# 0215Arthur/Pytorch_News_Recommender

Hardware: AMD Instinct MI355X
Metric: users/sec (train step) NRMS MIND-small hist=50 cand=5 (higher is better)
Workload: dtype f16 (MFMA inputs and saved activations; fp32 accumulate, softmax, loss, master weights and Adam); 1 GPU; configs[1] shapes: NRMS(nrms_v0) train step, 512 users/GPU, hist=50, cand=5, title_len=30, d=300, h=10, q=200, V=45800, dropout=0.2, Adam(lr=1e-3); users_per_gpu=512, global_batch=512, parallelism=dp1, precision=fp16, resident_batches=32

## Files before the change

### include/nrms_hip.h

```cpp
#ifndef NRMS_HIP_H
#define NRMS_HIP_H

#include <stddef.h>
#include <stdint.h>

#ifdef __cplusplus
extern "C" {
#endif

#define NRMS_OK            0
#define NRMS_EINVAL       -1
#define NRMS_ELAUNCH      -2
#define NRMS_EWORKSPACE   -3

#define NRMS_PRECISION_FP32   0
#define NRMS_PRECISION_BF16X3 1
#define NRMS_PRECISION_BF16   2
#define NRMS_FP16_KP 320
#define NRMS_FP16_DP 320
#define NRMS_FP16_QP 224
#define NRMS_PRECISION_FP16   3

#define NRMS_FLAG_PAD_ROW_ZERO 1
#define NRMS_FLAG_DEFER_WQKV 2
#define NRMS_FLAG_FWD_SCRATCH_KEPT 4
#define NRMS_FLAG_FUSED_SEQ64 8

typedef struct nrms_encoder_desc {
    int32_t  n_seq;
    int32_t  seq_len;
    int32_t  d_model;
    int32_t  n_heads;
    int32_t  q_dim;
    int32_t  vocab;
    float    p_drop_embed;
    float    p_drop_ctx;
    int32_t  precision;
    int32_t  use_output_proj;
    int32_t  mask_mode;
    int32_t  flags;
    uint64_t seed;
    float    loss_scale;
    float    p_drop_attn;
    const int32_t* seq_index;
} nrms_encoder_desc;

typedef struct nrms_encoder_weights {
    const float* table;
    const float* w_qkv;
    const float* b_qkv;
    const float* w_o;
    const float* b_o;
    const float* w_add;
    const float* b_add;
    const float* q_vec;
} nrms_encoder_weights;

typedef struct nrms_encoder_grads {
    float* table;
    float* w_qkv;
    float* b_qkv;
    float* w_o;
    float* b_o;
    float* w_add;
    float* b_add;
    float* q_vec;
} nrms_encoder_grads;

typedef struct nrms_encoder_acts {
    float* x;
    float* qkv;
    float* attn;
    float* ctx;
    float* t;
    float* w;
    void*  scratch;
} nrms_encoder_acts;

size_t nrms_encoder_fwd_scratch_bytes(const nrms_encoder_desc* desc);
size_t nrms_encoder_fused_qkv_bytes(const nrms_encoder_desc* desc);
int nrms_encoder_fwd(const nrms_encoder_desc* desc, const nrms_encoder_weights* w,
                     const int64_t* ids, const float* x, const uint8_t* mask ,
                     const nrms_encoder_acts* acts, float* out, void* stream);

size_t nrms_encoder_bwd_workspace_bytes(const nrms_encoder_desc* desc);
int nrms_encoder_bwd(const nrms_encoder_desc* desc, const nrms_encoder_weights* w,
                     const int64_t* ids, const float* x, const uint8_t* mask,
                     const nrms_encoder_acts* acts, const float* dout,
                     const nrms_encoder_grads* grads, float* dx,
                     void* workspace, size_t workspace_bytes, void* stream);
int nrms_encoder_bwd_wqkv(const nrms_encoder_desc* desc, const int64_t* ids, const float* x,
                          const nrms_encoder_acts* acts, const nrms_encoder_grads* grads,
                          void* workspace, size_t workspace_bytes, void* stream);

int nrms_sanitize_ids(const int64_t* src, int64_t* dst, int64_t n, int32_t vocab, int32_t* n_bad, void* stream);
int nrms_sanitize_ids_i32(const int32_t* src, int64_t* dst, int64_t n, int32_t vocab, int32_t* n_bad, void* stream);

int nrms_title_dedup(const int64_t* ids, int64_t n_titles, int32_t seq_len, int32_t* table, int64_t table_size,
                     int32_t* inverse, int32_t* rep_rows, int32_t* n_unique, void* stream);

int nrms_click_score_fwd(int32_t B, int32_t C, int32_t d, const float* cand, const float* user,
                         const uint8_t* mask, float* scores, void* stream);
int nrms_click_score_indexed(int32_t B, int32_t C, int32_t d, const float* news_vec, int64_t n_vec, const int32_t* index,
                             const float* user, const uint8_t* mask, float* scores, void* stream);
int nrms_click_score_bwd(int32_t B, int32_t C, int32_t d, const float* cand, const float* user,
                         const uint8_t* mask, const float* dscores, float* dcand, float* duser,
                         void* stream);

int nrms_ce_loss_fwd_bwd(int32_t B, int32_t C, const float* scores, float* loss_sum,
                         float* dscores, float grad_scale, void* stream);

int nrms_adam_step(size_t n, float* param, const float* grad, float* exp_avg, float* exp_avg_sq,
                   double lr, double beta1, double beta2, double eps, int32_t step, float grad_scale,
                   void* stream);

int nrms_adam_step_guarded(size_t n, float* param, const float* grad, float* exp_avg, float* exp_avg_sq,
                           double lr, double beta1, double beta2, double eps, int32_t step, float grad_scale,
                           int32_t* n_nonfinite, void* stream);
int nrms_grad_guard(size_t n, float* grad, int32_t* n_nonfinite, void* stream);

int nrms_impression_auc(int32_t n_imp, int32_t max_c, const float* scores, const uint8_t* labels,
                        const int32_t* lens, double* auc, void* stream);

int nrms_impression_metrics(int32_t n_imp, int32_t max_c, const float* scores, const uint8_t* labels,
                            const int32_t* lens, int32_t k_a, int32_t k_b, double* auc, double* mrr, double* ndcg_a,
                            double* ndcg_b, int32_t* ranks, void* stream);

size_t nrms_topk_dot_workspace_bytes(int32_t B, int64_t N, int32_t d, int32_t k);
int nrms_topk_dot(int32_t B, int64_t N, int32_t d, int32_t k, const float* user, const float* items, const int64_t* exclude,
                  int32_t n_exclude, float* top_scores, int64_t* top_ids, void* workspace, size_t workspace_bytes, void* stream);

size_t nrms_topk_grouped_dot_workspace_bytes(int32_t B, int64_t N, int32_t d, int32_t k, int32_t G);
int nrms_topk_grouped_dot(int32_t B, int64_t N, int32_t d, int32_t k, int32_t G, const float* query, const float* items,
                          const int32_t* item_ids, const int64_t* group_ptr, const int64_t* exclude, int32_t n_exclude,
                          float* top_scores, int64_t* top_ids, void* workspace, size_t workspace_bytes, void* stream);

size_t nrms_rank_dot_workspace_bytes(int32_t B, int64_t N, int32_t d, int32_t T, int32_t n_exclude);
int nrms_rank_dot(int32_t B, int64_t N, int32_t d, int32_t T, const float* user, const float* items, const int64_t* targets,
                  const int64_t* exclude, int32_t n_exclude, int32_t* ranks, float* target_scores, void* workspace,
                  size_t workspace_bytes, void* stream);

int nrms_layernorm_fwd(int64_t n_rows, int32_t d, const float* x, const float* gamma, const float* beta, float eps,
                       float* y, float* stats, void* stream);
size_t nrms_layernorm_bwd_workspace_bytes(int32_t d);
int nrms_layernorm_bwd(int64_t n_rows, int32_t d, const float* x, const float* gamma, const float* stats, const float* dy,
                       float* dx, float* dgamma_dbeta, void* workspace, size_t workspace_bytes, void* stream);

typedef struct nrms_news_features {
    int64_t n;
    int32_t d_text;
    int32_t d_cat;
    int32_t n_cat, n_sub;
    float   p_drop;
    uint64_t seed;
    const float* title_vec;
    const float* abst_vec;
    const float* cat_table;
    const float* sub_table;
    const int64_t* categ;
    const int64_t* subcateg;
} nrms_news_features;
int nrms_news_features_fwd(const nrms_news_features* f, float* out, void* stream);
int nrms_news_features_bwd(const nrms_news_features* f, const float* dout, float* d_title_vec, float* d_abst_vec,
                           float* d_cat_table, float* d_sub_table, void* stream);

#define NRMS_SEGPOOL_ROWS_UNIQUE 1
// ... 107 lines not shown
```

### pytorch_news_recommender_amd/_lib.py

```python
from __future__ import annotations

import ctypes as C
import os

PKG = os.path.dirname(os.path.abspath(__file__))
LIB_PATH = os.environ.get("NRMS_HIP_LIB") or os.path.join(PKG, "libnrms_hip.so")

NRMS_OK, NRMS_EINVAL, NRMS_ELAUNCH, NRMS_EWORKSPACE = 0, -1, -2, -3
NRMS_FLAG_PAD_ROW_ZERO = 1
NRMS_FLAG_DEFER_WQKV = 2
NRMS_FLAG_FWD_SCRATCH_KEPT = 4
NRMS_FLAG_FUSED_SEQ64 = 8
NRMS_PRECISION_FP32 = 0
NRMS_PRECISION_BF16X3 = 1
NRMS_PRECISION_BF16 = 2
NRMS_PRECISION_FP16 = 3
NRMS_DROPOUT_FIELDS16 = 0x100
NRMS_DROPOUT_SITE_NEWSVEC = 4
NRMS_FP16_KP, NRMS_FP16_DP, NRMS_FP16_QP = 320, 320, 224
PRECISIONS = {"fp32": 0, "bf16x3": 1, "bf16": 2, "fp16": 3}


class NrmsError(RuntimeError):
    pass


class EncoderDesc(C.Structure):
    _fields_ = [("n_seq", C.c_int32), ("seq_len", C.c_int32), ("d_model", C.c_int32),
                ("n_heads", C.c_int32), ("q_dim", C.c_int32), ("vocab", C.c_int32),
                ("p_drop_embed", C.c_float), ("p_drop_ctx", C.c_float), ("precision", C.c_int32),
                ("use_output_proj", C.c_int32), ("mask_mode", C.c_int32), ("flags", C.c_int32),
                ("seed", C.c_uint64), ("loss_scale", C.c_float), ("p_drop_attn", C.c_float), ("seq_index", C.c_void_p)]


class EncoderWeights(C.Structure):
    _fields_ = [("table", C.c_void_p), ("w_qkv", C.c_void_p), ("b_qkv", C.c_void_p), ("w_o", C.c_void_p),
                ("b_o", C.c_void_p), ("w_add", C.c_void_p), ("b_add", C.c_void_p), ("q_vec", C.c_void_p)]


class EncoderGrads(C.Structure):
    _fields_ = [("table", C.c_void_p), ("w_qkv", C.c_void_p), ("b_qkv", C.c_void_p), ("w_o", C.c_void_p),
                ("b_o", C.c_void_p), ("w_add", C.c_void_p), ("b_add", C.c_void_p), ("q_vec", C.c_void_p)]


class EncoderActs(C.Structure):
    _fields_ = [("x", C.c_void_p), ("qkv", C.c_void_p), ("attn", C.c_void_p), ("ctx", C.c_void_p),
                ("t", C.c_void_p), ("w", C.c_void_p), ("scratch", C.c_void_p)]


class SegPoolDesc(C.Structure):
    _fields_ = [("n_rows", C.c_int64), ("n_seg", C.c_int64), ("nnz", C.c_int64), ("d", C.c_int32), ("q", C.c_int32),
                ("precision", C.c_int32), ("flags", C.c_int32)]


NRMS_SEGPOOL_ROWS_UNIQUE = 1


class ClickGraphDesc(C.Structure):
    _fields_ = [("n_users", C.c_int64), ("n_news", C.c_int64), ("n_edges", C.c_int64), ("user_ptr", C.c_void_p),
                ("user_news", C.c_void_p), ("news_ptr", C.c_void_p), ("news_users", C.c_void_p)]


class NewsFeatures(C.Structure):
    _fields_ = [("n", C.c_int64), ("d_text", C.c_int32), ("d_cat", C.c_int32), ("n_cat", C.c_int32), ("n_sub", C.c_int32),
                ("p_drop", C.c_float), ("seed", C.c_uint64), ("title_vec", C.c_void_p), ("abst_vec", C.c_void_p),
                ("cat_table", C.c_void_p), ("sub_table", C.c_void_p), ("categ", C.c_void_p), ("subcateg", C.c_void_p)]


class NewsvecDesc(C.Structure):
    _fields_ = [("n_slots", C.c_int64), ("n_rows", C.c_int32), ("d", C.c_int32), ("precision", C.c_int32),
                ("p_drop", C.c_float), ("seed", C.c_uint64)]


SIGNATURES = {
    "nrms_encoder_fwd": (C.c_int, [C.POINTER(EncoderDesc), C.POINTER(EncoderWeights), C.c_void_p, C.c_void_p,
                                   C.c_void_p, C.POINTER(EncoderActs), C.c_void_p, C.c_void_p]),
    "nrms_encoder_bwd_workspace_bytes": (C.c_size_t, [C.POINTER(EncoderDesc)]),
    "nrms_encoder_fwd_scratch_bytes": (C.c_size_t, [C.POINTER(EncoderDesc)]),
    "nrms_encoder_fused_qkv_bytes": (C.c_size_t, [C.POINTER(EncoderDesc)]),
    "nrms_encoder_bwd": (C.c_int, [C.POINTER(EncoderDesc), C.POINTER(EncoderWeights), C.c_void_p, C.c_void_p,
                                   C.c_void_p, C.POINTER(EncoderActs), C.c_void_p, C.POINTER(EncoderGrads), C.c_void_p,
                                   C.c_void_p, C.c_size_t, C.c_void_p]),
    "nrms_encoder_bwd_wqkv": (C.c_int, [C.POINTER(EncoderDesc), C.c_void_p, C.c_void_p, C.POINTER(EncoderActs),
                                        C.POINTER(EncoderGrads), C.c_void_p, C.c_size_t, C.c_void_p]),
    "nrms_sanitize_ids": (C.c_int, [C.c_void_p, C.c_void_p, C.c_int64, C.c_int32, C.c_void_p, C.c_void_p]),
    "nrms_sanitize_ids_i32": (C.c_int, [C.c_void_p, C.c_void_p, C.c_int64, C.c_int32, C.c_void_p, C.c_void_p]),
    "nrms_title_dedup": (C.c_int, [C.c_void_p, C.c_int64, C.c_int32, C.c_void_p, C.c_int64, C.c_void_p, C.c_void_p,
                                   C.c_void_p, C.c_void_p]),
    "nrms_click_score_indexed": (C.c_int, [C.c_int32, C.c_int32, C.c_int32, C.c_void_p, C.c_int64, C.c_void_p, C.c_void_p,
                                           C.c_void_p, C.c_void_p, C.c_void_p]),
    "nrms_click_score_fwd": (C.c_int, [C.c_int32, C.c_int32, C.c_int32, C.c_void_p, C.c_void_p, C.c_void_p,
                                       C.c_void_p, C.c_void_p]),
    "nrms_click_score_bwd": (C.c_int, [C.c_int32, C.c_int32, C.c_int32, C.c_void_p, C.c_void_p, C.c_void_p,
                                       C.c_void_p, C.c_void_p, C.c_void_p, C.c_void_p]),
    "nrms_ce_loss_fwd_bwd": (C.c_int, [C.c_int32, C.c_int32, C.c_void_p, C.c_void_p, C.c_void_p, C.c_float,
                                       C.c_void_p]),
    "nrms_adam_step": (C.c_int, [C.c_size_t, C.c_void_p, C.c_void_p, C.c_void_p, C.c_void_p, C.c_double,
                                 C.c_double, C.c_double, C.c_double, C.c_int32, C.c_float, C.c_void_p]),
    "nrms_adam_step_guarded": (C.c_int, [C.c_size_t, C.c_void_p, C.c_void_p, C.c_void_p, C.c_void_p, C.c_double,
                                         C.c_double, C.c_double, C.c_double, C.c_int32, C.c_float, C.c_void_p, C.c_void_p]),
    "nrms_grad_guard": (C.c_int, [C.c_size_t, C.c_void_p, C.c_void_p, C.c_void_p]),
    "nrms_segment_pool_workspace_bytes": (C.c_size_t, [C.POINTER(SegPoolDesc)]),
    "nrms_segment_pool_fwd": (C.c_int, [C.POINTER(SegPoolDesc)] + [C.c_void_p] * 10 + [C.c_void_p, C.c_size_t, C.c_void_p]),
    "nrms_segment_pool_bwd": (C.c_int, [C.POINTER(SegPoolDesc)] + [C.c_void_p] * 12 + [C.c_void_p, C.c_size_t, C.c_void_p]),
    "nrms_hier_tree_scratch_bytes": (C.c_size_t, [C.c_int32, C.c_int32]),
    "nrms_hier_tree_build": (C.c_int, [C.c_int32, C.c_int32] + [C.c_void_p] * 16 + [C.c_size_t, C.c_void_p]),
    "nrms_hier_add_embedding_fwd": (C.c_int, [C.c_int64, C.c_int32, C.c_int32, C.c_void_p, C.c_void_p, C.c_void_p, C.c_void_p, C.c_void_p]),
    "nrms_sequence_partition_count_ints": (C.c_size_t, [C.c_int32]),
    "nrms_sequence_partition": (C.c_int, [C.c_void_p, C.c_int32, C.c_int32, C.c_void_p, C.c_void_p, C.c_void_p]),
    "nrms_encoder_empty_workspace_bytes": (C.c_size_t, [C.POINTER(EncoderDesc)]),
    "nrms_encoder_empty_saved_bytes": (C.c_size_t, [C.POINTER(EncoderDesc)]),
    "nrms_encoder_empty_fwd": (C.c_int, [C.POINTER(EncoderDesc), C.POINTER(EncoderWeights), C.c_void_p, C.c_void_p, C.c_void_p, C.c_void_p, C.c_size_t,
                                         C.c_void_p]),
    "nrms_encoder_empty_bwd": (C.c_int, [C.POINTER(EncoderDesc), C.POINTER(EncoderWeights), C.c_void_p, C.c_void_p, C.c_void_p, C.POINTER(EncoderGrads),
                                         C.c_void_p, C.c_size_t, C.c_void_p]),
    "nrms_csr_from_padded": (C.c_int, [C.c_int64, C.c_int32, C.c_void_p, C.c_int64, C.c_void_p, C.c_void_p, C.c_void_p]),
    "nrms_graph_sample_workspace_bytes": (C.c_size_t, [C.c_int64, C.c_int32]),
    "nrms_graph_sample_neighbors": (C.c_int, [C.POINTER(ClickGraphDesc), C.c_int64, C.c_int32, C.c_void_p, C.c_uint64, C.c_void_p, C.c_void_p,
                                              C.c_void_p, C.c_size_t, C.c_void_p]),
    "nrms_graph_resolve_workspace_bytes": (C.c_size_t, [C.c_int64]),
    "nrms_graph_resolve_rows": (C.c_int, [C.c_int64, C.c_int32, C.c_int64, C.c_void_p, C.c_void_p, C.c_int32] + [C.c_void_p] * 4
                                + [C.c_void_p, C.c_size_t, C.c_void_p]),
    "nrms_hier_add_embedding_bwd_workspace_bytes": (C.c_size_t, [C.c_int64, C.c_int32, C.c_int32]),
    "nrms_hier_add_embedding_bwd": (C.c_int, [C.c_int64, C.c_int32, C.c_int32, C.c_void_p, C.c_void_p, C.c_void_p, C.c_void_p, C.c_void_p,
                                              C.c_size_t, C.c_void_p]),
    "nrms_hier_match": (C.c_int, [C.c_int32, C.c_int32, C.c_int32] + [C.c_void_p] * 11 + [C.c_void_p]),
    "nrms_hier_score_fwd": (C.c_int, [C.c_int32, C.c_int32, C.c_int32] + [C.c_void_p] * 9 + [C.c_float, C.c_float, C.c_void_p, C.c_void_p]),
    "nrms_hier_score_bwd": (C.c_int, [C.c_int32, C.c_int32, C.c_int32] + [C.c_void_p] * 9 + [C.c_float, C.c_float] + [C.c_void_p] * 5 + [C.c_void_p]),
    "nrms_impression_auc": (C.c_int, [C.c_int32, C.c_int32, C.c_void_p, C.c_void_p, C.c_void_p, C.c_void_p,
                                      C.c_void_p]),
    "nrms_impression_metrics": (C.c_int, [C.c_int32, C.c_int32, C.c_void_p, C.c_void_p, C.c_void_p, C.c_int32, C.c_int32]
                                + [C.c_void_p] * 5 + [C.c_void_p]),
    "nrms_topk_dot_workspace_bytes": (C.c_size_t, [C.c_int32, C.c_int64, C.c_int32, C.c_int32]),
    "nrms_topk_dot": (C.c_int, [C.c_int32, C.c_int64, C.c_int32, C.c_int32, C.c_void_p, C.c_void_p, C.c_void_p, C.c_int32,
                                C.c_void_p, C.c_void_p, C.c_void_p, C.c_size_t, C.c_void_p]),
    "nrms_topk_grouped_dot_workspace_bytes": (C.c_size_t, [C.c_int32, C.c_int64, C.c_int32, C.c_int32, C.c_int32]),
    "nrms_topk_grouped_dot": (C.c_int, [C.c_int32, C.c_int64, C.c_int32, C.c_int32, C.c_int32] + [C.c_void_p] * 5 + [C.c_int32]
                              + [C.c_void_p] * 3 + [C.c_size_t, C.c_void_p]),
    "nrms_rank_dot_workspace_bytes": (C.c_size_t, [C.c_int32, C.c_int64, C.c_int32, C.c_int32, C.c_int32]),
    "nrms_rank_dot": (C.c_int, [C.c_int32, C.c_int64, C.c_int32, C.c_int32] + [C.c_void_p] * 4 + [C.c_int32]
                      + [C.c_void_p] * 3 + [C.c_size_t, C.c_void_p]),
    "nrms_hier_query": (C.c_int, [C.c_int32] * 4 + [C.c_void_p] * 10 + [C.c_float, C.c_float, C.c_void_p, C.c_void_p]),
    "nrms_dropout_keep_mask": (C.c_int, [C.c_uint64, C.c_int32, C.c_int64, C.c_int32, C.c_float, C.c_void_p,
                                         C.c_void_p]),
    "nrms_layernorm_fwd": (C.c_int, [C.c_int64, C.c_int32, C.c_void_p, C.c_void_p, C.c_void_p, C.c_float, C.c_void_p,
                                     C.c_void_p, C.c_void_p]),
    "nrms_layernorm_bwd_workspace_bytes": (C.c_size_t, [C.c_int32]),
    "nrms_layernorm_bwd": (C.c_int, [C.c_int64, C.c_int32, C.c_void_p, C.c_void_p, C.c_void_p, C.c_void_p, C.c_void_p,
                                     C.c_void_p, C.c_void_p, C.c_size_t, C.c_void_p]),
    "nrms_news_features_fwd": (C.c_int, [C.POINTER(NewsFeatures), C.c_void_p, C.c_void_p]),
    "nrms_news_features_bwd": (C.c_int, [C.POINTER(NewsFeatures), C.c_void_p, C.c_void_p, C.c_void_p, C.c_void_p,
                                         C.c_void_p, C.c_void_p]),
    "nrms_newsvec_saved_bytes": (C.c_size_t, [C.POINTER(NewsvecDesc)]),
    "nrms_newsvec_workspace_bytes": (C.c_size_t, [C.POINTER(NewsvecDesc)]),
    "nrms_newsvec_fwd": (C.c_int, [C.POINTER(NewsvecDesc)] + [C.c_void_p] * 6 + [C.c_size_t, C.c_void_p, C.c_void_p, C.c_size_t,
                                                                                C.c_void_p]),
    "nrms_newsvec_bwd": (C.c_int, [C.POINTER(NewsvecDesc)] + [C.c_void_p] * 4 + [C.c_size_t] + [C.c_void_p] * 4
                         + [C.c_size_t, C.c_void_p]),
    "nrms_newsvec_distinct": (C.c_int, [C.POINTER(NewsvecDesc), C.c_void_p, C.c_void_p, C.c_void_p, C.c_void_p]),
    "nrms_newsvec_rows_workspace_bytes": (C.c_size_t, [C.c_int64, C.c_int32, C.c_int32]),
    "nrms_newsvec_rows_fwd": (C.c_int, [C.c_int64, C.c_int32, C.c_int32] + [C.c_void_p] * 5 + [C.c_size_t, C.c_void_p]),
    "nrms_timing_enable": (None, [C.c_int]),
# ... 36 lines not shown
```

### pytorch_news_recommender_amd/csrc/capi.hip

```cpp
#include <stdarg.h>

#include <algorithm>

#include <mutex>
#include <vector>

#include "gemm.h"

namespace nrms {

int launch_attention(bool bwd, int n_seq, int S, int d, int h, const float* qkv, float* ctx, const Dropout& drop,
                     const float* dctx, float* dqkv, const uint8_t* mask, const int64_t* ids, const float* bias_hm,
                     const int* pos, float* padsum, float* dbias, hipStream_t stream, const Dropout* pdrop = nullptr,
                     bool split = false);
size_t attention_padsum_floats();
int launch_addattn_fwd(int n_seq, int S, int d, int q, const float* ctx, const float* w_add, const float* b_add,
                       const float* q_vec, float* T, float* wout, float* out, const uint8_t* mask, int npass,
                       void* wplanes, hipStream_t stream);
int addattn_bwd_rows_waves(int n_seq);
int launch_addattn_bwd_rows(int n_seq, int S, int d, int q, const float* ctx, const float* dout, const float* w,
                            const float* T, float* ds, float* dq_partial, float* dq, const uint8_t* mask,
                            hipStream_t stream);

int launch_attention_wide(bool bwd, int n_seq, int S, int d, int h, const float* qkv, float* ctx, const Dropout& pdrop,
// ... 165 lines not shown
    w.wadd_t = take(q * dm);
    w.wo_t = take(d->use_output_proj ? dm * dm : 0);
    const size_t p1 = gemm_tn_workspace_floats((int)M, (int)(3 * dm), (int)dm, nullptr);
    const size_t p2 = gemm_tn_workspace_floats((int)M, (int)q, (int)dm, nullptr);
    const size_t p3 = d->use_output_proj ? gemm_tn_workspace_floats((int)M, (int)dm, (int)dm, nullptr) : 0;
    w.tn_partial = take(p1 > p2 ? (p1 > p3 ? p1 : p3) : (p2 > p3 ? p2 : p3));
    const bool fused64 = (d->flags & NRMS_FLAG_FUSED_SEQ64) != 0;
    w.dq_partial = take(std::max((size_t)(wide_additive(d) ? d->n_seq : addattn_bwd_rows_waves(d->n_seq)) * q,
                                 fused64 ? user64_dq_partial_floats(d->n_seq) : (size_t)0));
    w.wplanes = take(wplane_bytes(d) / sizeof(float));
    const bool pz = d->vocab > 0 && (d->flags & NRMS_FLAG_PAD_ROW_ZERO) != 0;
    w.live = take(d->vocab > 0 ? M : 0);
    w.pos = take(pz ? M : 0);
    w.n_live = take(d->vocab > 0 ? 64 : 0);
    w.cscr = take(d->vocab > 0 ? compact_scratch_ints((long)M) : 0);
    w.padsum = take(pz ? attention_padsum_floats() : 0);
    w.sscr = take(d->vocab > 0 ? scatter_grouped_scratch_ints((long)M, d->vocab) : 0);
    w.u64planes = take(fused64 ? user64_bwd_planes_bytes(d->n_heads) / sizeof(float) + 1 : 0);
    w.total = off;
    return w;
}

}

using namespace nrms;

struct FwdScratch { size_t wq, bq, planes, live, n_live, cscr, total; };
static bool skip_pad_rows(const nrms_encoder_desc* d) { return d->vocab > 0 && (d->flags & NRMS_FLAG_PAD_ROW_ZERO) != 0; }
static FwdScratch fwd_scratch(const nrms_encoder_desc* d) {
    FwdScratch f;
    const size_t dm = (size_t)d->d_model;
    f.wq = 0;
    f.bq = align_up(3 * dm * dm * sizeof(float), 256);
    f.planes = f.bq + align_up(3 * dm * sizeof(float), 256);
    f.live = f.planes + wplane_bytes(d);
    f.n_live = f.live + (skip_pad_rows(d) ? align_up((size_t)d->n_seq * d->seq_len * sizeof(int), 256) : 0);
    f.cscr = f.n_live + (skip_pad_rows(d) ? 256 : 0);
    f.total = f.cscr + (skip_pad_rows(d) ? align_up(compact_scratch_ints((long)d->n_seq * d->seq_len) * sizeof(int), 256) : 0);
    if (d->flags & NRMS_FLAG_FUSED_SEQ64) f.total = std::max(f.total, align_up(user64_fwd_planes_bytes(d->n_heads), 256));
    return f;
}

struct Fwd16Scratch { size_t planes, live, pos, n_live, cscr, order, order_cnt, total; };
static Fwd16Scratch fwd16_scratch(const nrms_encoder_desc* d) {
    Fwd16Scratch f;
    const size_t M = (size_t)d->n_seq * d->seq_len;
    const bool gather = d->vocab > 0;
    f.planes = 0;
    f.live = align_up(d->use_output_proj ? fused16v1_planes_bytes(d->d_model, d->n_heads, d->q_dim)
                                         : fused16_layout(d->d_model, d->n_heads, d->q_dim).total, 256);
    f.pos = f.live + (gather ? align_up(M * sizeof(int), 256) : 0);
    f.n_live = f.pos + (gather ? align_up(M * sizeof(int), 256) : 0);
    f.cscr = f.n_live + (gather ? 256 : 0);
    f.order = f.cscr + (gather ? align_up(compact_scratch_ints((long)M) * sizeof(int), 256) : 0);
    f.order_cnt = f.order + (gather ? align_up((size_t)3 * d->n_seq * sizeof(int), 256) : 0);
    f.total = f.order_cnt + (gather ? align_up(title_order_cnt_ints(d->n_seq) * sizeof(int), 256) : 0);
    return f;
}

struct KeptRec { const void* scratch; const void* ids; int n_seq, seq_len, vocab, d_model, n_heads, use_wo; };
static std::mutex g_kept_mu;
static std::vector<KeptRec> g_kept;
static void kept_forget(const void* scratch) {
    if (scratch == nullptr) return;
    std::lock_guard<std::mutex> lk(g_kept_mu);
    for (size_t i = 0; i < g_kept.size(); ++i)
        if (g_kept[i].scratch == scratch) { g_kept[i] = g_kept.back(); g_kept.pop_back(); break; }
}
static void kept_record(const nrms_encoder_desc* d, const void* scratch, const void* ids) {
    std::lock_guard<std::mutex> lk(g_kept_mu);
    if (g_kept.size() >= 64) g_kept.erase(g_kept.begin());
    g_kept.push_back(KeptRec{scratch, ids, d->n_seq, d->seq_len, d->vocab, d->d_model, d->n_heads, d->use_output_proj});
}
static bool kept_matches(const nrms_encoder_desc* d, const void* scratch, const void* ids) {
    std::lock_guard<std::mutex> lk(g_kept_mu);
    for (const KeptRec& r : g_kept)
        if (r.scratch == scratch)
            return r.ids == ids && r.n_seq == d->n_seq && r.seq_len == d->seq_len && r.vocab == d->vocab && r.d_model == d->d_model &&
                   r.n_heads == d->n_heads && r.use_wo == d->use_output_proj;
    return false;
}

static int encoder_fwd16(const nrms_encoder_desc* desc, const nrms_encoder_weights* w, const int64_t* ids, const float* x,
                         const nrms_encoder_acts* acts, float* out, hipStream_t s) {
    const bool gather = desc->vocab > 0;
    NRMS_REQUIRE(acts->x && acts->ctx && acts->scratch, "encoder_fwd(fp16): acts.x, acts.ctx and acts.scratch are required");
    const int S = desc->seq_len, d = desc->d_model, h = desc->n_heads, q = desc->q_dim;
    const long M = (long)desc->n_seq * S;
    const Fwd16Scratch fs = fwd16_scratch(desc);
    const Fused16Layout L = fused16_layout(d, h, q);
    char* base = (char*)acts->scratch;
    const bool v1 = desc->use_output_proj != 0;
    NRMS_REQUIRE(!v1 || (w->w_o && w->b_o && acts->attn), "encoder_fwd(fp16): use_output_proj needs w_o, b_o and acts.attn");
    SideSet* ss = (gather && skip_pad_rows(desc)) ? side_streams_for(s) : nullptr;
    hipStream_t s_prep = ss != nullptr ? ss->s[1] : s;
    int rc = fused_bwd16_join(s);
    if (rc) return rc;
    if (ss != nullptr) {
        rc = side_order(ss, 5, s, s_prep, "encoder_fwd(fp16)");
        if (rc) return rc;
    }
    bool forked = ss != nullptr;
    auto join_prep = [&]() -> int {
        if (!forked) return NRMS_OK;
        forked = false;
        if (hipEventRecord(ss->ev[4], s_prep) != hipSuccess || hipStreamWaitEvent(s, ss->ev[4], 0) != hipSuccess) {
            set_error("encoder_fwd(fp16): joining the helper stream failed");
            return NRMS_ELAUNCH;
        }
        return NRMS_OK;
    };
    rc = v1 ? launch_prep16v1(d, h, q, w->w_qkv, w->b_qkv, w->w_o, w->b_o, w->w_add, w->b_add, w->q_vec, base + fs.planes, s_prep)
            : launch_prep16(d, h, q, w->w_qkv, w->b_qkv, w->w_add, w->b_add, w->q_vec, base + fs.planes, s_prep);
    if (rc) { (void)join_prep(); return rc; }
    Fused16Fwd f{};
    f.n_seq = desc->n_seq; f.S = S; f.d = d; f.h = h; f.q = q;
    f.planes = base + fs.planes; f.x16 = acts->x; f.ctx16 = acts->ctx; f.t16 = acts->t; f.w = acts->w; f.out = out;
    f.drop = make_dropout(desc->seed, desc->p_drop_ctx);
    if (gather) {
        const Dropout drop_e = make_dropout(desc->seed, desc->p_drop_embed);
        if (skip_pad_rows(desc)) {
            int* live = (int*)(base + fs.live);
            int* pos = (int*)(base + fs.pos);
            int* n_live = (int*)(base + fs.n_live);
            int* order = (int*)(base + fs.order);
            int* order_cnt = (int*)(base + fs.order_cnt);
            rc = S <= 32 ? launch_title_order(desc->n_seq, S, ids, order, order_cnt, s_prep, 3) : NRMS_OK;
            if (rc) { (void)join_prep(); return rc; }
            rc = launch_compact_live_rows(M, ids, live, pos, n_live, (int*)(base + fs.cscr), s);
            if (rc == NRMS_OK) rc = launch_gather16(M, d, L.KP, ids, live, n_live, w->table, drop_e, acts->x, s);
            const int rj = join_prep();
            if (rc) return rc;
            if (rj) return rj;
            f.pos = pos;
            f.n_rows = n_live;
            f.ids = ids;
            if (S <= 32) { f.order = order; f.order_cnt = order_cnt; }
        } else {
            rc = launch_gather16(M, d, L.KP, ids, nullptr, nullptr, w->table, drop_e, acts->x, s);
            if (rc) return rc;
        }
    } else {
        rc = launch_cast16(M, d, L.KP, x, acts->x, s);
        if (rc) return rc;
    }
    rc = v1 ? launch_fused_fwd16v1(f, h, acts->attn, s) : launch_fused_fwd16(f, s);
    if (rc == NRMS_OK && gather && skip_pad_rows(desc)) kept_record(desc, acts->scratch, ids);
    return rc;
}

struct Bwd16Layout { size_t fused, live, pos, n_live, cscr, order, order_cnt, dxc, sscr, total; };
static Bwd16Layout bwd16_layout(const nrms_encoder_desc* d) {
    Bwd16Layout L;
    const size_t M = (size_t)d->n_seq * d->seq_len;
    const bool gather = d->vocab > 0;
    size_t off = 0;
    auto take = [&](size_t bytes) { size_t o = off; off = align_up(off + bytes, 256); return o; };
    L.fused = take(d->use_output_proj ? fused16v1_bwd_bytes((long)M, d->n_seq, d->n_heads) : fused16_bwd_layout((long)M, d->n_seq).total);
    L.live = take(gather ? M * sizeof(int) : 0);
    L.pos = take(gather ? M * sizeof(int) : 0);
    L.n_live = take(gather ? 256 : 0);
    L.cscr = take(gather ? compact_scratch_ints((long)M) * sizeof(int) : 0);
    L.order = take(gather ? (size_t)3 * d->n_seq * sizeof(int) : 0);
    L.order_cnt = take(gather ? title_order_cnt_ints(d->n_seq) * sizeof(int) : 0);
    L.dxc = take(gather ? M * std::max((size_t)d->d_model * sizeof(float), (size_t)NRMS_FP16_KP * 2) : 0);
    L.sscr = take(gather ? scatter_grouped_scratch_ints((long)M, d->vocab) * sizeof(int) : 0);
    L.total = off;
    return L;
}

static int encoder_bwd16(const nrms_encoder_desc* desc, const nrms_encoder_weights* w, const int64_t* ids, const float* x,
                         const nrms_encoder_acts* acts, const float* dout, const nrms_encoder_grads* grads, float* dx,
                         void* workspace, size_t workspace_bytes, hipStream_t s) {
    NRMS_REQUIRE(w && acts && dout && grads && workspace, "encoder_bwd(fp16): null argument");
    const bool v1 = desc->use_output_proj != 0;
    NRMS_REQUIRE(!v1 || (w->w_o && acts->attn && grads->w_o && grads->b_o),
                 "encoder_bwd(fp16): use_output_proj needs w_o, acts.attn, grads.w_o, grads.b_o");
    NRMS_REQUIRE(acts->x && acts->ctx && acts->t && acts->w, "encoder_bwd(fp16): acts.x, ctx, t, w are required");
    NRMS_REQUIRE(grads->w_qkv && grads->b_qkv && grads->w_add && grads->b_add && grads->q_vec, "encoder_bwd(fp16): null gradient buffer");
    const bool gather = desc->vocab > 0;
    NRMS_REQUIRE(gather ? (ids != nullptr && grads->table != nullptr) : (dx != nullptr), "encoder_bwd(fp16): %s missing",
                 gather ? "ids / grads.table" : "dx");
    const Bwd16Layout L = bwd16_layout(desc);
    if (workspace_bytes < L.total) { set_error("encoder_bwd(fp16): workspace %zu < required %zu bytes", workspace_bytes, L.total); return NRMS_EWORKSPACE; }
    NRMS_REQUIRE(((uintptr_t)workspace & 255) == 0, "encoder_bwd(fp16): workspace must be 256-byte aligned");
    if (desc->n_seq == 0) return NRMS_OK;
    const int S = desc->seq_len, d = desc->d_model;
    const long M = (long)desc->n_seq * S;
    char* base = (char*)workspace;
    Fused16Bwd f{};
    f.n_seq = desc->n_seq; f.S = S; f.d = d; f.h = desc->n_heads; f.q = desc->q_dim;
    f.workspace = base + L.fused;
    f.w_qkv = w->w_qkv; f.b_qkv = w->b_qkv; f.w_add = w->w_add; f.q_vec = w->q_vec;
    f.x16 = acts->x; f.ctx16 = acts->ctx; f.t16 = acts->t; f.w = acts->w; f.dout = dout;
    f.loss_scale = desc->loss_scale;
    f.drop = make_dropout(desc->seed, desc->p_drop_ctx);
    f.dw_qkv = grads->w_qkv; f.db_qkv = grads->b_qkv; f.dw_add = grads->w_add; f.db_add = grads->b_add; f.dq_vec = grads->q_vec;
    if (v1) { f.w_o = w->w_o; f.attn16 = acts->attn; f.dw_o = grads->w_o; f.db_o = grads->b_o; }
    int rc;
    int* live = (int*)(base + L.live);
    int* n_live = (int*)(base + L.n_live);
    if (gather) {
        const bool kept = (desc->flags & NRMS_FLAG_FWD_SCRATCH_KEPT) != 0 && skip_pad_rows(desc) && acts->scratch != nullptr &&
                          kept_matches(desc, acts->scratch, ids);
        if (kept) {
            const Fwd16Scratch fs = fwd16_scratch(desc);
            char* fb = (char*)acts->scratch;
            live = (int*)(fb + fs.live);
            n_live = (int*)(fb + fs.n_live);
            f.pos = (int*)(fb + fs.pos); f.n_rows_dev = n_live; f.ids = ids;
            if (S <= 32) { f.order = (int*)(fb + fs.order); f.order_cnt = (int*)(fb + fs.order_cnt); }
        } else {
            int* pos = (int*)(base + L.pos);
            rc = launch_compact_live_rows(M, ids, live, pos, n_live, (int*)(base + L.cscr), s);
            if (rc) return rc;
            if (skip_pad_rows(desc)) {
                int* order = (int*)(base + L.order);
                int* order_cnt = (int*)(base + L.order_cnt);
                f.pos = pos; f.n_rows_dev = n_live; f.ids = ids;
                if (S <= 32) {
                    rc = launch_title_order(desc->n_seq, S, ids, order, order_cnt, s, 3);
                    if (rc) return rc;
                    f.order = order; f.order_cnt = order_cnt;
                }
            }
        }
        f.dx = (float*)(base + L.dxc);
        f.dx_fp16 = skip_pad_rows(desc);
    } else {
        f.dx = dx;
    }
    SideSet* ss_prep = (gather && skip_pad_rows(desc)) ? side_streams_for(s) : nullptr;
    bool prepared = false;
    if (ss_prep != nullptr) {
        rc = side_order(ss_prep, 5, s, ss_prep->s[1], "encoder_bwd(fp16)");
        if (rc) return rc;
        rc = launch_scatter_prepare(M, desc->vocab, ids, live, n_live, (int*)(base + L.sscr), ss_prep->s[1]);
        if (hipEventRecord(ss_prep->ev[4], ss_prep->s[1]) != hipSuccess) { set_error("encoder_bwd(fp16): hipEventRecord failed"); return NRMS_ELAUNCH; }
        if (rc) { (void)hipStreamWaitEvent(s, ss_prep->ev[4], 0); return rc; }
        prepared = true;
    }
    auto join_prepare = [&]() -> int {
        if (!prepared) return NRMS_OK;
        if (hipStreamWaitEvent(s, ss_prep->ev[4], 0) != hipSuccess) { set_error("encoder_bwd(fp16): hipStreamWaitEvent failed"); return NRMS_ELAUNCH; }
        return NRMS_OK;
    };
    const float* sc_dev = nullptr;
    f.sc_out = &sc_dev;
    f.defer_join = (desc->flags & NRMS_FLAG_DEFER_WQKV) != 0;
    rc = v1 ? launch_fused_bwd16v1(f, s) : launch_fused_bwd16(f, s);
    {
        const int rj = join_prepare();
        if (rc) return rc;
        if (rj) return rj;
    }
    if (gather) {
        const Dropout drop_e = make_dropout(desc->seed, desc->p_drop_embed);
        if (skip_pad_rows(desc))
            rc = launch_scatter_grouped(M, desc->vocab, d, ids, live, n_live, f.dx, drop_e, grads->table, (int*)(base + L.sscr), s,
                                        f.dx_fp16, NRMS_FP16_KP, sc_dev, prepared);
        else
            rc = launch_scatter_dense_rows(M, d, ids, live, n_live, f.dx, drop_e, grads->table, s);
    }
    return rc;
}

extern "C" int nrms_encoder_fwd(const nrms_encoder_desc* desc, const nrms_encoder_weights* w, const int64_t* ids,
                                const float* x, const uint8_t* mask, const nrms_encoder_acts* acts, float* out,
                                void* stream) {
    int rc = validate_desc(desc, "encoder_fwd");
    if (rc) return rc;
    if (acts != nullptr) kept_forget(acts->scratch);
    if (desc->precision == NRMS_PRECISION_FP16) {
        NRMS_REQUIRE(w && acts && out, "encoder_fwd: null argument");
        NRMS_REQUIRE(w->w_qkv && w->b_qkv && w->w_add && w->b_add && w->q_vec, "encoder_fwd: null weight");
        NRMS_REQUIRE(desc->vocab > 0 ? (ids != nullptr && w->table != nullptr) : (x != nullptr), "encoder_fwd: input missing");
        if (desc->n_seq == 0) return NRMS_OK;
        return encoder_fwd16(desc, w, ids, x, acts, out, (hipStream_t)stream);
    }
    NRMS_REQUIRE(w && acts && out, "encoder_fwd: null argument");
    NRMS_REQUIRE(w->w_qkv && w->b_qkv && w->w_add && w->b_add && w->q_vec, "encoder_fwd: null weight");
    if (desc->flags & NRMS_FLAG_FUSED_SEQ64) {
        NRMS_REQUIRE(x != nullptr && acts->qkv != nullptr && acts->scratch != nullptr, "encoder_fwd(fused): x, acts.qkv and acts.scratch are required");
        const bool train = acts->ctx != nullptr && acts->t != nullptr && acts->w != nullptr;
        if (desc->n_seq == 0) return NRMS_OK;
        rc = fused_bwd16_join((hipStream_t)stream);
        if (rc) return rc;
        return launch_user64_fwd(desc->n_seq, desc->seq_len, desc->d_model, desc->n_heads, desc->q_dim, x, w->w_qkv, w->b_qkv, w->w_add,
                                 w->b_add, w->q_vec, acts->scratch, acts->ctx, acts->t, acts->w, acts->qkv, out, train, (hipStream_t)stream);
    }
    NRMS_REQUIRE(acts->qkv && acts->ctx, "encoder_fwd: acts.qkv / acts.ctx are required");
    const bool gather = desc->vocab > 0, wo = desc->use_output_proj != 0;
    NRMS_REQUIRE(gather ? (ids != nullptr && w->table != nullptr) : (x != nullptr),
                 "encoder_fwd: %s input missing", gather ? "ids/table" : "x");
    NRMS_REQUIRE(!wo || (w->w_o && w->b_o && acts->attn), "encoder_fwd: use_output_proj needs w_o, b_o and acts.attn");
    NRMS_REQUIRE(desc->mask_mode == 0 || mask != nullptr, "encoder_fwd: mask_mode=%d but mask is null", desc->mask_mode);
    if (desc->n_seq == 0) return NRMS_OK;
    hipStream_t s = (hipStream_t)stream;
    const int S = desc->seq_len, d = desc->d_model, q = desc->q_dim, M = desc->n_seq * S;
    const Dropout drop_e = make_dropout(desc->seed, desc->p_drop_embed);
    const Dropout drop_c = make_dropout(desc->seed, desc->p_drop_ctx);
    const Dropout no_drop = make_dropout(0, 0.f);
    const uint8_t* amask = (desc->mask_mode & 1) ? mask : nullptr;
    const uint8_t* pmask = (desc->mask_mode & 2) ? mask : nullptr;

    NRMS_REQUIRE(acts->scratch != nullptr, "encoder_fwd: acts.scratch (nrms_encoder_fwd_scratch_bytes) is required");
    const FwdScratch fs = fwd_scratch(desc);
    float* wq_hm = (float*)((char*)acts->scratch + fs.wq);
    float* bq_hm = (float*)((char*)acts->scratch + fs.bq);
    void* wplanes = (char*)acts->scratch + fs.planes;
    const HeadPerm perm{d / desc->n_heads, desc->n_heads};
    rc = launch_permute_rows(w->w_qkv, w->b_qkv, wq_hm, bq_hm, 3 * d, d, perm, s);
    if (rc) return rc;

    NTArgs g{};
    g.M = M; g.N = 3 * d; g.K = d; g.rows_per_tile = NT_BM;
    g.W = wq_hm; g.bias = bq_hm; g.C = acts->qkv; g.ldc = 3 * d;
    const float* xin = x;
    if (gather) {
        NRMS_REQUIRE(acts->x != nullptr, "encoder_fwd: acts.x (gathered embeddings) is required for the news encoder");
        if (skip_pad_rows(desc)) {
            int* live = (int*)((char*)acts->scratch + fs.live);
            int* n_live = (int*)((char*)acts->scratch + fs.n_live);
            int* cscr = (int*)((char*)acts->scratch + fs.cscr);
            rc = launch_compact_live_rows((long)M, ids, live, nullptr, n_live, cscr, s);
            if (rc) return rc;
            rc = launch_gather_dropout_compact((long)M, d, ids, live, n_live, w->table, drop_e, acts->x, s);
            if (rc) return rc;
            rc = launch_fill_pad_rows((long)desc->n_seq, S, 3 * d, ids, bq_hm, acts->qkv, amask == nullptr, s);
            if (rc) return rc;
            g.c_rows = live; g.m_dev = n_live;
        } else {
            rc = launch_gather_dropout((long)M, d, ids, w->table, drop_e, acts->x, s);
            if (rc) return rc;
        }
        xin = acts->x;
    }
    g.A = xin; g.lda = d;
    rc = nt_gemm(desc, A_PLAIN, E_STORE, g, wplanes, s, "qkv_proj_fwd");
    if (rc) return rc;
    Dropout pdrop_attn = make_dropout(desc->seed, desc->p_drop_attn);
    pdrop_attn.seq_index = desc->seq_index; pdrop_attn.seq_h = desc->n_heads;
    if (wide_attention(desc))
        rc = launch_attention_wide(false, desc->n_seq, S, d, desc->n_heads, acts->qkv, wo ? acts->attn : acts->ctx,
                                   pdrop_attn, nullptr, nullptr, amask, s);
    else
        rc = launch_attention(false, desc->n_seq, S, d, desc->n_heads, acts->qkv, wo ? acts->attn : acts->ctx,
                              wo ? no_drop : drop_c, nullptr, nullptr, amask,
                              (gather && skip_pad_rows(desc)) ? ids : nullptr, (gather && skip_pad_rows(desc)) ? bq_hm : nullptr,
                              nullptr, nullptr, nullptr, s, &pdrop_attn, desc->precision != NRMS_PRECISION_FP32);
    if (rc) return rc;
    if (wo) {
        NTArgs o{};
        o.M = M; o.N = d; o.K = d; o.rows_per_tile = NT_BM;
        o.A = acts->attn; o.lda = d; o.W = w->w_o; o.bias = w->b_o; o.C = acts->ctx; o.ldc = d; o.drop = drop_c;
        rc = nt_gemm(desc, A_PLAIN, E_STORE, o, wplanes, s, "out_proj_fwd");
        if (rc) return rc;
    }
    if (wide_additive(desc)) {
        NRMS_REQUIRE(acts->t != nullptr, "encoder_fwd: acts.t is required for q_dim > 256 or d_model > 512 (also for inference)");
        NTArgs z{};
        z.M = M; z.N = q; z.K = d; z.rows_per_tile = NT_BM;
        z.A = acts->ctx; z.lda = d; z.W = w->w_add; z.bias = w->b_add; z.C = acts->t; z.ldc = q;
        rc = nt_gemm(desc, A_PLAIN, E_STORE, z, wplanes, s, "addattn_proj_fwd");
        if (rc) return rc;
        return launch_addattn_rows_fwd_wide(desc->n_seq, S, d, q, acts->t, w->q_vec, acts->ctx, pmask, acts->w, out, s);
    }
    const int npass = desc->precision == NRMS_PRECISION_FP32 ? 0 : (desc->precision == NRMS_PRECISION_BF16X3 ? 3 : 1);
    return launch_addattn_fwd(desc->n_seq, S, d, q, acts->ctx, w->w_add, w->b_add, w->q_vec, acts->t, acts->w, out,
                              pmask, npass, wplanes, s);
}

extern "C" size_t nrms_encoder_fwd_scratch_bytes(const nrms_encoder_desc* desc) {
    if (validate_desc(desc, "encoder_fwd_scratch_bytes")) return 0;
    if (desc->precision == NRMS_PRECISION_FP16) return fwd16_scratch(desc).total;
    return fwd_scratch(desc).total;
}

extern "C" size_t nrms_encoder_fused_qkv_bytes(const nrms_encoder_desc* desc) {
    if (desc == nullptr || !(desc->flags & NRMS_FLAG_FUSED_SEQ64) || validate_desc(desc, "encoder_fused_qkv_bytes")) return 0;
    return user64_qkv_bytes(desc->n_seq, desc->n_heads);
}

extern "C" size_t nrms_encoder_bwd_workspace_bytes(const nrms_encoder_desc* desc) {
    if (validate_desc(desc, "encoder_bwd_workspace_bytes")) return 0;
    if (desc->precision == NRMS_PRECISION_FP16) return bwd16_layout(desc).total;
    return bwd_layout(desc).total;
}

namespace nrms {
struct SideEntry { int device; hipStream_t caller; SideSet* set; };
static std::mutex g_side_mu;
static std::vector<SideEntry> g_side_sets;

SideSet* side_streams_for(hipStream_t caller) {
    if (getenv("NRMS_NO_SIDE_STREAMS") != nullptr) return nullptr;
    int dev = 0;
    if (hipGetDevice(&dev) != hipSuccess) return nullptr;
    std::lock_guard<std::mutex> lk(g_side_mu);
    for (const SideEntry& e : g_side_sets)
        if (e.device == dev && e.caller == caller) return e.set;
    if (g_side_sets.size() >= 32) return nullptr;
    SideSet* ss = new SideSet();
    bool ok = true;
    for (int i = 0; i < 2 && ok; ++i) ok = hipStreamCreateWithFlags(&ss->s[i], hipStreamNonBlocking) == hipSuccess;
    for (int i = 0; i < 8 && ok; ++i) ok = hipEventCreateWithFlags(&ss->ev[i], hipEventDisableTiming) == hipSuccess;
    if (!ok) {
        for (int i = 0; i < 2; ++i) if (ss->s[i]) (void)hipStreamDestroy(ss->s[i]);
        for (int i = 0; i < 8; ++i) if (ss->ev[i]) (void)hipEventDestroy(ss->ev[i]);
        delete ss;
        ss = nullptr;
        (void)hipGetLastError();
    }
    g_side_sets.push_back(SideEntry{dev, caller, ss});
    return ss;
}

int side_order(SideSet* ss, int e, hipStream_t from, hipStream_t to, const char* what) {
    if (hipEventRecord(ss->ev[e], from) != hipSuccess || hipStreamWaitEvent(to, ss->ev[e], 0) != hipSuccess) {
        set_error("%s: ordering the helper stream failed: %s", what, hipGetErrorString(hipGetLastError()));
        return NRMS_ELAUNCH;
    }
    return NRMS_OK;
}

SideJoinGuard::~SideJoinGuard() {
    if (!armed) return;
    for (int i = 0; i < 2; ++i)
        if (hipEventRecord(ss->ev[6 + i], ss->s[i]) == hipSuccess) (void)hipStreamWaitEvent(caller, ss->ev[6 + i], 0);
}
}

static int bwd_wqkv(const nrms_encoder_desc* desc, const float* xin, const float* dqkv, const int* n_live,
                    const nrms_encoder_grads* grads, float* tn_partial, hipStream_t s) {
    const int d = desc->d_model, M = desc->n_seq * desc->seq_len;
    TNArgs t{};
    t.M = M; t.N = 3 * d; t.K = d; t.amode = A_PLAIN;
    t.A = dqkv; t.lda = 3 * d; t.B = xin; t.ldb = d;
    t.dW = grads->w_qkv; t.dbias = grads->b_qkv; t.partial = tn_partial;
    t.perm = HeadPerm{d / desc->n_heads, desc->n_heads};
    if (skip_pad_rows(desc)) t.m_dev = n_live;
    return tn_gemm(desc, t, s, "dwqkv_bwd");
}

extern "C" int nrms_encoder_bwd_wqkv(const nrms_encoder_desc* desc, const int64_t* ids, const float* x,
                                     const nrms_encoder_acts* acts, const nrms_encoder_grads* grads, void* workspace,
                                     size_t workspace_bytes, void* stream) {
    int rc = validate_desc(desc, "encoder_bwd_wqkv");
    if (rc) return rc;
    if (desc->precision == NRMS_PRECISION_FP16) return fused_bwd16_join((hipStream_t)stream);
    NRMS_REQUIRE(acts && grads && workspace, "encoder_bwd_wqkv: null argument");
    NRMS_REQUIRE(grads->w_qkv && grads->b_qkv, "encoder_bwd_wqkv: null gradient buffer");
    const bool gather = desc->vocab > 0;
    NRMS_REQUIRE(gather ? (ids != nullptr && acts->x != nullptr) : (x != nullptr), "encoder_bwd_wqkv: input missing");
    if (desc->n_seq == 0) return NRMS_OK;
    const BwdWorkspace L = bwd_layout(desc);
    if (workspace_bytes < L.total) {
        set_error("encoder_bwd_wqkv: workspace %zu < required %zu bytes", workspace_bytes, L.total);
        return NRMS_EWORKSPACE;
    }
    char* base = (char*)workspace;
    return bwd_wqkv(desc, gather ? acts->x : x, (const float*)(base + L.dqkv), (const int*)(base + L.n_live), grads,
                    (float*)(base + L.tn_partial), (hipStream_t)stream);
}

extern "C" int nrms_encoder_bwd(const nrms_encoder_desc* desc, const nrms_encoder_weights* w, const int64_t* ids,
                                const float* x, const uint8_t* mask, const nrms_encoder_acts* acts, const float* dout,
                                const nrms_encoder_grads* grads, float* dx, void* workspace, size_t workspace_bytes,
                                void* stream) {
    int rc = validate_desc(desc, "encoder_bwd");
    if (rc) return rc;
    if (desc->precision == NRMS_PRECISION_FP16)
        return encoder_bwd16(desc, w, ids, x, acts, dout, grads, dx, workspace, workspace_bytes, (hipStream_t)stream);
    NRMS_REQUIRE(w && acts && dout && grads && workspace, "encoder_bwd: null argument");
    NRMS_REQUIRE(acts->qkv && acts->ctx && acts->t && acts->w, "encoder_bwd: all saved activations are required");
    NRMS_REQUIRE(grads->w_qkv && grads->b_qkv && grads->w_add && grads->b_add && grads->q_vec,
                 "encoder_bwd: null gradient buffer");
    const bool gather = desc->vocab > 0, wo = desc->use_output_proj != 0;
    NRMS_REQUIRE(gather ? (ids != nullptr && acts->x != nullptr && grads->table != nullptr) : (x != nullptr && dx != nullptr),
                 "encoder_bwd: %s missing", gather ? "ids/acts.x/grads.table" : "x/dx");
    NRMS_REQUIRE(!wo || (w->w_o && acts->attn && grads->w_o && grads->b_o),
                 "encoder_bwd: use_output_proj needs w_o, acts.attn, grads.w_o, grads.b_o");
    NRMS_REQUIRE(desc->mask_mode == 0 || mask != nullptr, "encoder_bwd: mask_mode=%d but mask is null", desc->mask_mode);
    const BwdWorkspace L = bwd_layout(desc);
    if (workspace_bytes < L.total) {
        set_error("encoder_bwd: workspace %zu < required %zu bytes", workspace_bytes, L.total);
        return NRMS_EWORKSPACE;
    }
    NRMS_REQUIRE(((uintptr_t)workspace & 255) == 0, "encoder_bwd: workspace must be 256-byte aligned");
    if (desc->n_seq == 0) return NRMS_OK;
    hipStream_t s = (hipStream_t)stream;
    const int S = desc->seq_len, d = desc->d_model, q = desc->q_dim, M = desc->n_seq * S;
    const Dropout drop_e = make_dropout(desc->seed, desc->p_drop_embed);
    const Dropout drop_c = make_dropout(desc->seed, desc->p_drop_ctx);
    const Dropout no_drop = make_dropout(0, 0.f);
    const uint8_t* amask = (desc->mask_mode & 1) ? mask : nullptr;
    const uint8_t* pmask = (desc->mask_mode & 2) ? mask : nullptr;
    char* base = (char*)workspace;
    float* dctx = (float*)(base + L.dctx);
    float* dqkv = (float*)(base + L.dqkv);
    float* dattn = (float*)(base + L.dattn);
    float* ds = (float*)(base + L.ds);
    float* wqkv_t = (float*)(base + L.wqkv_t);
    float* wadd_t = (float*)(base + L.wadd_t);
    float* wo_t = (float*)(base + L.wo_t);
    float* tn_partial = (float*)(base + L.tn_partial);
    float* dq_partial = (float*)(base + L.dq_partial);
    void* wplanes = (void*)(base + L.wplanes);

    rc = fused_bwd16_join(s);
    if (rc) return rc;
    SideSet* ss = side_streams_for(s);
    const bool side = ss != nullptr;
    hipStream_t s2 = side ? ss->s[0] : s;
    SideJoinGuard join_guard(ss, s);
    auto fork = [&](int i) -> int {
        return side ? side_order(ss, i, s, s2, "encoder_bwd") : NRMS_OK;
    };

    const bool fused64 = (desc->flags & NRMS_FLAG_FUSED_SEQ64) != 0;
    if (fused64) {
        rc = launch_user64_bwd(desc->n_seq, S, d, desc->n_heads, q, w->w_add, w->q_vec, base + L.u64planes, dout, acts->t, acts->w,
                               acts->qkv, ds, dq_partial, grads->q_vec, dqkv, s);
        if (rc) return rc;
    } else {
        if (wide_additive(desc))
            rc = launch_addattn_rows_bwd_wide(desc->n_seq, S, d, q, acts->ctx, dout, acts->w, acts->t, ds, dq_partial, grads->q_vec,
                                              pmask, s);
        else
            rc = launch_addattn_bwd_rows(desc->n_seq, S, d, q, acts->ctx, dout, acts->w, acts->t, ds, dq_partial, grads->q_vec,
                                         pmask, s);
        if (rc) return rc;
    }
    rc = fork(0);
    if (rc) return rc;
    {
        TNArgs t{};
        t.M = M; t.N = q; t.K = d; t.amode = A_DZ;
        t.ds = ds; t.qv = w->q_vec; t.T = acts->t; t.B = acts->ctx; t.ldb = d;
        t.dW = grads->w_add; t.dbias = grads->b_add; t.partial = tn_partial;
        rc = tn_gemm(desc, t, s2, "dwadd_bwd");
        if (rc) return rc;
    }
    if (!fused64) {
        rc = launch_transpose(w->w_add, wadd_t, q, d, s);
        if (rc) return rc;
        {
            NTArgs g{};
            g.M = M; g.N = d; g.K = q; g.rows_per_tile = NT_BM;
            g.ds = ds; g.qv = w->q_vec; g.T = acts->t;
            g.W = wadd_t; g.C = dctx; g.ldc = d;
            g.wrow = acts->w; g.dout = dout; g.seq_of_row = make_row_div((uint32_t)S);
            g.drop = drop_c;
            rc = nt_gemm(desc, A_DZ, E_DCTX, g, wplanes, s, "dctx_bwd");
            if (rc) return rc;
        }
// ... 195 lines not shown
```

### pytorch_news_recommender_amd/csrc/common.h

```cpp
#pragma once
#include <hip/hip_runtime.h>
#include <stdint.h>
#include <stdio.h>
#include <string>

#include "../../include/nrms_hip.h"

namespace nrms {

typedef float f32x4 __attribute__((ext_vector_type(4)));
typedef float f32x16 __attribute__((ext_vector_type(16)));

constexpr int WAVE = 64;

__device__ __forceinline__ f32x4 mfma16(float a, float b, f32x4 c) {
    return __builtin_amdgcn_mfma_f32_16x16x4f32(a, b, c, 0, 0, 0);
}
__device__ __forceinline__ f32x16 mfma32(float a, float b, f32x16 c) {
    return __builtin_amdgcn_mfma_f32_32x32x2f32(a, b, c, 0, 0, 0);
}
__device__ __forceinline__ int crow32(int r, int hh) { return (r & 3) + 8 * (r >> 2) + 4 * hh; }

struct Keep4 { bool k[4]; };

constexpr uint32_t PHILOX_SITE_GRAPH_SAMPLE = 5u;

__host__ __device__ __forceinline__ void philox_round(uint32_t& c0, uint32_t& c1, uint32_t& c2,
                                                      uint32_t& c3, uint32_t k0, uint32_t k1) {
    const uint64_t p0 = (uint64_t)0xD2511F53u * c0;
    const uint64_t p1 = (uint64_t)0xCD9E8D57u * c2;
    const uint32_t n0 = (uint32_t)(p1 >> 32) ^ c1 ^ k0;
    const uint32_t n1 = (uint32_t)p1;
    const uint32_t n2 = (uint32_t)(p0 >> 32) ^ c3 ^ k1;
    const uint32_t n3 = (uint32_t)p0;
    c0 = n0; c1 = n1; c2 = n2; c3 = n3;
}

__host__ __device__ __forceinline__ void philox4x32_7(uint64_t seed, uint64_t group, uint32_t site,
                                                      uint32_t out[4]) {
    uint32_t c0 = (uint32_t)group, c1 = (uint32_t)(group >> 32), c2 = site, c3 = 0x9E3779B9u;
    uint32_t k0 = (uint32_t)seed, k1 = (uint32_t)(seed >> 32);
#pragma unroll
    for (int i = 0; i < 7; ++i) {
        philox_round(c0, c1, c2, c3, k0, k1);
        k0 += 0x9E3779B9u;
        k1 += 0xBB67AE85u;
    }
    out[0] = c0; out[1] = c1; out[2] = c2; out[3] = c3;
}

__host__ __device__ __forceinline__ uint32_t drop_threshold(float p) {
    double t = (double)p * 4294967296.0;
    if (t <= 0.0) return 0u;
    if (t >= 4294967295.0) return 4294967295u;
    return (uint32_t)t;
}

__device__ __forceinline__ f32x4 dropout_scale4(uint64_t seed, uint32_t site, uint64_t group,
                                                uint32_t thresh, float inv_keep) {
    uint32_t r[4];
    philox4x32_7(seed, group, site, r);
    f32x4 s;
    s[0] = r[0] >= thresh ? inv_keep : 0.f;
    s[1] = r[1] >= thresh ? inv_keep : 0.f;
    s[2] = r[2] >= thresh ? inv_keep : 0.f;
    s[3] = r[3] >= thresh ? inv_keep : 0.f;
    return s;
}
__host__ __device__ __forceinline__ uint32_t drop_threshold16(float p) {
    const double t = (double)p * 65536.0;
    return t <= 0.0 ? 0u : (t >= 65535.0 ? 65535u : (uint32_t)t);
}
__device__ __forceinline__ void dropout_scale8(uint64_t seed, uint32_t site, uint64_t group8, uint32_t thresh16, float inv_keep,
                                               float (&s)[8]) {
    uint32_t r[4];
    philox4x32_7(seed, group8, site, r);
#pragma unroll
    for (int w = 0; w < 4; ++w) {
        s[2 * w] = (r[w] & 0xFFFFu) >= thresh16 ? inv_keep : 0.f;
        s[2 * w + 1] = (r[w] >> 16) >= thresh16 ? inv_keep : 0.f;
    }
}
__device__ __forceinline__ float dropout_scale1(uint64_t seed, uint32_t site, uint64_t elem,
                                                uint32_t thresh, float inv_keep) {
    uint32_t r[4];
    philox4x32_7(seed, elem >> 2, site, r);
    return r[elem & 3] >= thresh ? inv_keep : 0.f;
}

__device__ __forceinline__ float fast_tanh(float x) {
    const float e = __expf(2.0f * x);
    const float r = 1.0f - 2.0f * __builtin_amdgcn_rcpf(e + 1.0f);
    const float x2 = x * x;
    const float p = x * (1.0f + x2 * (-0.33333333f + x2 * (0.13333333f + x2 * -0.053968254f)));
    return fabsf(x) < 0.12f ? p : r;
}

struct HeadPerm {
    int dk, h;
    __host__ __device__ __forceinline__ int src(int np) const {
        if (dk == 0) return np;
        const int head = np / (3 * dk), r = np - head * 3 * dk;
        const int which = r / dk, j = r - which * dk;
        return which * h * dk + head * dk + j;
    }
};

struct Dropout {
    uint64_t seed;
    uint32_t thresh;
    float inv_keep;
    uint32_t thresh16;
    const int* seq_index;
    int seq_h;
    __device__ __forceinline__ long unit_of(long unit) const {
        if (seq_index == nullptr) return unit;
        const long seq = unit / seq_h;
        return (long)seq_index[seq] * seq_h + (unit - seq * seq_h);
    }
};

inline Dropout make_dropout(uint64_t seed, float p) {
    Dropout d;
    d.seed = seed;
    d.thresh = drop_threshold(p);
    d.thresh16 = drop_threshold16(p);
    d.inv_keep = p > 0.f ? 1.0f / (1.0f - p) : 1.0f;
    d.seq_index = nullptr;
    d.seq_h = 1;
    return d;
}

__device__ __forceinline__ float wave_sum(float v) {
#pragma unroll
    for (int o = 32; o > 0; o >>= 1) v += __shfl_xor(v, o, 64);
    return v;
}
__device__ __forceinline__ float wave_max(float v) {
#pragma unroll
    for (int o = 32; o > 0; o >>= 1) v = fmaxf(v, __shfl_xor(v, o, 64));
    return v;
}

void set_error(const char* fmt, ...);
int check_launch(const char* what);

struct SideSet {
    hipStream_t s[2] = {nullptr, nullptr};
    hipEvent_t ev[8] = {nullptr, nullptr, nullptr, nullptr, nullptr, nullptr, nullptr, nullptr};
    bool pending = false;
};
SideSet* side_streams_for(hipStream_t caller);
int side_order(SideSet* ss, int e, hipStream_t from, hipStream_t to, const char* what);
struct SideJoinGuard {
    SideSet* ss; hipStream_t caller; bool armed;
    SideJoinGuard(SideSet* set, hipStream_t c) : ss(set), caller(c), armed(set != nullptr) {}
    void disarm() { armed = false; }
    ~SideJoinGuard();
};

struct TimingScope {
    TimingScope(const char* name, hipStream_t s);
    ~TimingScope();
    bool active;
// ... 16 lines not shown
```

### pytorch_news_recommender_amd/csrc/fused16.hip

```cpp
#include <stdlib.h>

#include "fused16.h"

namespace nrms {

struct Fwd16Args {
    int n_seq, S, d, h, dk, q;
    const _Float16* x16;
    const int* pos;
    const int* n_rows;
    const int64_t* ids;
    const int* order;
    const int* order_cnt;
    const _Float16* wtiles;
    const float* bqkv32;
    const float* badd32;
    const float* qv32;
    _Float16* ctx16;
    _Float16* t16;
    float* w;
    float* out;
    Dropout drop;
    int dbg;
};

#ifndef F16_FWD_SLOTS
#define F16_FWD_SLOTS 3
#endif
constexpr int F16_FWD_WGS = F16_FWD_SLOTS == 2 ? 3 : 2;
template <bool TRAIN, int SB>
__global__ __launch_bounds__(F16_THREADS, SB == 1 ? F16_FWD_WGS : 1) void fused_fwd16_kernel(Fwd16Args a) {
    extern __shared__ __attribute__((aligned(16))) char smem[];
    const int tid = threadIdx.x, lane = tid & 63;
    const int wave = __builtin_amdgcn_readfirstlane(tid >> 6);
    const int l32 = lane & 31, hh = lane >> 5;
    const int S = a.S;
    constexpr int KP = F16_KP, DP = F16_DP;
    const int n_head_tiles = 3 * a.h;

    int slot_id = blockIdx.x * F16_WAVES + wave;
    bool valid = slot_id < a.n_seq;
    int seq = slot_id;
    if (a.order != nullptr) {
        const int n_ne = a.order_cnt[0], n_e = a.order_cnt[1];
        const int g_ne = (n_ne + F16_WAVES - 1) / F16_WAVES;
        if ((int)blockIdx.x < g_ne) { valid = slot_id < n_ne; seq = valid ? a.order[slot_id] : 0; }
        else {
            slot_id -= g_ne * F16_WAVES;
            valid = slot_id < n_e;
            seq = valid ? a.order[a.n_seq + slot_id] : 0;
        }
    }
    if (!valid) seq = 0;
    const long tok0 = (long)seq * S;
    bool tok_ok[SB];
#pragma unroll
    for (int b = 0; b < SB; ++b) tok_ok[b] = valid && 32 * b + l32 < S;
    bool empty = false;
    if (SB == 1 && a.ids != nullptr && valid) {
        const bool is_pad = lane < S ? a.ids[tok0 + lane] == 0 : true;
        empty = __ballot(is_pad) == ~0ull;
    }
    const bool live = valid && !empty;
    const bool skip_heads = __syncthreads_and(live ? 0 : 1) != 0;
    const int n_begin = skip_heads ? n_head_tiles : 0;

    using Ring = TileRingDMA<SB == 1 ? F16_FWD_SLOTS : 3>;
    constexpr int AH = Ring::AHEAD;
    Ring ring;
    ring.smem = smem; ring.src = a.wtiles; ring.n_tiles = n_head_tiles + F16_QT; ring.wave = wave; ring.lane = lane; ring.l32 = l32; ring.hh = hh;
#pragma unroll
    for (int i = 0; i < AH; ++i) ring.load(n_begin + i);
    float* addv = reinterpret_cast<float*>(smem + (SB == 1 ? F16_FWD_SLOTS : 3) * F16_SLOT_DMA);
    for (int i = tid; i < 2 * F16_QP; i += F16_THREADS) addv[i] = i < F16_QP ? a.badd32[i] : a.qv32[i - F16_QP];

    h8 xf[SB][F16_KS];
#pragma unroll
    for (int b = 0; b < SB; ++b) {
        long row = -1;
        if (tok_ok[b] && !empty) {
            row = a.pos != nullptr ? (long)a.pos[tok0 + 32 * b + l32] : tok0 + 32 * b + l32;
            if (row < 0) row = *a.n_rows;
        }
        const _Float16* xr = a.x16 + (row < 0 ? 0 : row) * KP + 8 * hh;
#pragma unroll
        for (int s = 0; s < F16_KS; ++s) xf[b][s] = *reinterpret_cast<const h8*>(xr + 16 * s);
        if (row < 0) {
#pragma unroll
            for (int s = 0; s < F16_KS; ++s) xf[b][s] = h8{0, 0, 0, 0, 0, 0, 0, 0};
        }
    }
    __builtin_amdgcn_s_waitcnt(0x0F70);
    __asm__ volatile("s_waitcnt lgkmcnt(0)\n\ts_barrier" ::: "memory");

    int n = n_begin;
#pragma unroll 1
    for (int head = 0; head < a.h; ++head) {
        f32x16 ct[SB];
        if (!skip_heads) {
            f32x16 qt[SB], kt[SB], vv[SB];
            auto pre = [&](int g) { ring.load_group(n + AH, g); };
            if (!live) ring.load(n + AH);
#pragma unroll
            for (int b = 0; b < SB; ++b) {
                qt[b] = zero16();
                if (live) { if (b == 0) tile_mma<true>(qt[b], ring, n, xf[b], pre); else tile_mma<true>(qt[b], ring, n, xf[b]); }
            }
            ring.step_barrier(n);
            ++n;
            if (!live) ring.load(n + AH);
#pragma unroll
            for (int b = 0; b < SB; ++b) {
                kt[b] = zero16();
                if (live) { if (b == 0) tile_mma<true>(kt[b], ring, n, xf[b], pre); else tile_mma<true>(kt[b], ring, n, xf[b]); }
            }
            ring.step_barrier(n);
            ++n;
            if (!live) ring.load(n + AH);
#pragma unroll
            for (int b = 0; b < SB; ++b) {
                vv[b] = zero16();
                if (live) { if (b == 0) tile_mma<false>(vv[b], ring, n, xf[b], pre); else tile_mma<false>(vv[b], ring, n, xf[b]); }
            }
            if (live) {
#pragma unroll
                for (int ib = 0; ib < SB; ++ib) {
                    f32x16 st[SB];
                    float m = -3.0e38f;
#pragma unroll
                    for (int jb = 0; jb < SB; ++jb) {
                        st[jb] = mfma32h(acc_frag(kt[jb], 0), acc_frag(qt[ib], 0), zero16());
                        st[jb] = mfma32h(acc_frag(kt[jb], 1), acc_frag(qt[ib], 1), st[jb]);
#pragma unroll
                        for (int r = 0; r < 16; ++r) {
                            st[jb][r] = 32 * jb + crow32(r, hh) < S ? st[jb][r] : -3.0e38f;
                            m = fmaxf(m, st[jb][r]);
                        }
                    }
                    m = fmaxf(m, __shfl_xor(m, 32, 64));
                    float sum = 0.f;
#pragma unroll
                    for (int jb = 0; jb < SB; ++jb)
#pragma unroll
                        for (int r = 0; r < 16; ++r) {
                            const float p = 32 * jb + crow32(r, hh) < S ? __expf(st[jb][r] - m) : 0.f;
                            st[jb][r] = p;
                            sum += p;
                        }
                    sum += __shfl_xor(sum, 32, 64);
                    const float inv = 1.0f / sum;
                    ct[ib] = zero16();
#pragma unroll
                    for (int jb = 0; jb < SB; ++jb) {
#pragma unroll
                        for (int r = 0; r < 16; ++r) st[jb][r] *= inv;
                        ct[ib] = mfma32h(acc_frag(vv[jb], 0), acc_frag(st[jb], 0), ct[ib]);
                        ct[ib] = mfma32h(acc_frag(vv[jb], 1), acc_frag(st[jb], 1), ct[ib]);
                    }
                }
            }
        }
        if (!live) {
#pragma unroll
            for (int b = 0; b < SB; ++b) ct[b] = rows_of(a.bqkv32 + (3 * head + 2) * 32, hh);
        }
#pragma unroll
        for (int b = 0; b < SB; ++b) {
            if (a.drop.thresh != 0u) {
#pragma unroll
                for (int c = 0; c < 2; ++c) {
                    const uint64_t e0 = (uint64_t)(tok0 + 32 * b + l32) * (uint64_t)DP + (uint64_t)(head * 32 + 16 * c + 8 * hh);
                    float sc[8];
                    dropout_scale8(a.drop.seed, 1u, e0 >> 3, a.drop.thresh16, a.drop.inv_keep, sc);
#pragma unroll
                    for (int e = 0; e < 8; ++e) ct[b][8 * c + e] *= sc[e];
                }
            }
            if (valid && !F16_DBG(a.dbg, 8)) {
                const h8 z = {0, 0, 0, 0, 0, 0, 0, 0};
                _Float16* dst = a.ctx16 + frag_off((long)seq * SB + b, F16_CS, 2 * head, l32, hh);
                *reinterpret_cast<h8*>(dst) = tok_ok[b] ? acc_frag(ct[b], 0) : z;
                *reinterpret_cast<h8*>(dst + 512) = tok_ok[b] ? acc_frag(ct[b], 1) : z;
            }
        }
        if (!skip_heads) {
            ring.step_barrier(n);
            ++n;
        }
    }
#pragma unroll
    for (int b = 0; b < SB; ++b) {
        if (valid) {
            for (int head = a.h; head < F16_CS / 2; ++head) {
                _Float16* dst = a.ctx16 + frag_off((long)seq * SB + b, F16_CS, 2 * head, l32, hh);
                *reinterpret_cast<h8*>(dst) = h8{0, 0, 0, 0, 0, 0, 0, 0};
                *reinterpret_cast<h8*>(dst + 512) = h8{0, 0, 0, 0, 0, 0, 0, 0};
            }
        }
    }

    __asm__ volatile("s_waitcnt vmcnt(0)" ::: "memory");
    h8 cf[SB][F16_CS];
#pragma unroll
    for (int b = 0; b < SB; ++b) {
        const _Float16* src = a.ctx16 + frag_off((long)seq * SB + b, F16_CS, 0, l32, hh);
#pragma unroll
        for (int s = 0; s < F16_CS; ++s) cf[b][s] = *reinterpret_cast<const h8*>(src + (F16_DBG(a.dbg, 16) ? 0 : 512 * s));
    }
    float score[SB];
#pragma unroll
    for (int b = 0; b < SB; ++b) score[b] = 0.f;
#pragma unroll 1
    for (int t = 0; t < F16_QT; ++t) {
        const f32x16 ba = rows_of(addv + 32 * t, hh), qq = rows_of(addv + F16_QP + 32 * t, hh);
        __builtin_amdgcn_sched_barrier(0);
        auto pre2 = [&](int g) { ring.load_group(n + AH, g); };
        if (!valid) ring.load(n + AH);
#pragma unroll
        for (int b = 0; b < SB; ++b) {
            f32x16 tt = zero16();
            if (valid) { if (b == 0) tile_mma<true>(tt, ring, n, cf[b], pre2); else tile_mma<true>(tt, ring, n, cf[b]); }
#pragma unroll
            for (int g = 0; g < 4; ++g) {
                h4 th;
#pragma unroll
                for (int e = 0; e < 4; ++e) {
                    const float ex = __builtin_amdgcn_exp2f(fmaf(tt[4 * g + e], 2.885390082f, ba[4 * g + e]));
                    const float v = fmaf(-2.0f, __builtin_amdgcn_rcpf(ex + 1.0f), 1.0f);
                    score[b] += qq[4 * g + e] * v;
                    th[e] = (_Float16)v;
                }
                if (TRAIN && valid && !F16_DBG(a.dbg, 4)) {
                    if (!tok_ok[b]) th = h4{0, 0, 0, 0};
                    *reinterpret_cast<h4*>(a.t16 + ((((long)seq * SB + b) * (F16_QP / 16) + 2 * t + (g >> 1)) * 32 + l32) * 16 +
                                           8 * (g & 1) + 4 * hh) = th;
                }
            }
        }
        ring.step_barrier(n);
        ++n;
    }
    float mx = -3.0e38f;
#pragma unroll
    for (int b = 0; b < SB; ++b) {
        score[b] += __shfl_xor(score[b], 32, 64);
        score[b] = 32 * b + l32 < S ? score[b] : -3.0e38f;
        mx = fmaxf(mx, score[b]);
    }
#pragma unroll
    for (int o = 16; o > 0; o >>= 1) mx = fmaxf(mx, __shfl_xor(mx, o, 64));
    float es = 0.f, wgt[SB];
#pragma unroll
    for (int b = 0; b < SB; ++b) {
        wgt[b] = 32 * b + l32 < S ? __expf(score[b] - mx) : 0.f;
        es += wgt[b];
    }
#pragma unroll
    for (int o = 16; o > 0; o >>= 1) es += __shfl_xor(es, o, 64);
#pragma unroll
// ... 41 lines not shown
    for (int t = 0; t < F16_QT; ++t) {
        const f32x16 ba = rows_of(addv + 32 * t, hh), qq = rows_of(addv + F16_QP + 32 * t, hh);
        __builtin_amdgcn_sched_barrier(0);
        auto pre2 = [&](int g) { if (n + AH < n_steps) ring.load_piece_at(n + AH, tile_at(n + AH), g); };
        if (!valid && n + AH < n_steps) ring.load_at(n + AH, tile_at(n + AH));
        f32x16 tt = zero16();
        if (valid) tile_mma<true>(tt, ring, n, cf, pre2);
#pragma unroll
        for (int g = 0; g < 4; ++g) {
            h4 th;
#pragma unroll
            for (int e = 0; e < 4; ++e) {
                const float ex = __builtin_amdgcn_exp2f(fmaf(tt[4 * g + e], 2.885390082f, ba[4 * g + e]));
                const float v = fmaf(-2.0f, __builtin_amdgcn_rcpf(ex + 1.0f), 1.0f);
                score += qq[4 * g + e] * v;
                th[e] = (_Float16)v;
            }
            if (TRAIN && valid) {
                if (!tok) th = h4{0, 0, 0, 0};
                *reinterpret_cast<h4*>(a.t16 + (((long)sq * (F16_QP / 16) + 2 * t + (g >> 1)) * 32 + l32) * 16 + 8 * (g & 1) + 4 * hh) = th;
            }
        }
        ring.step_barrier(n);
        ++n;
    }
    score += __shfl_xor(score, 32, 64);
    score = l32 < S ? score : NEG;
    float mx = score;
#pragma unroll
    for (int o = 16; o > 0; o >>= 1) mx = fmaxf(mx, __shfl_xor(mx, o, 64));
    float wgt = l32 < S ? __expf(score - mx) : 0.f;
    float es = wgt;
#pragma unroll
    for (int o = 16; o > 0; o >>= 1) es += __shfl_xor(es, o, 64);
    wgt /= es;
    if (TRAIN && a.w != nullptr && tok && hh == 0) a.w[t0 + l32] = wgt;
    if (valid) {
        h8 sel[2];
#pragma unroll
        for (int s2 = 0; s2 < 2; ++s2)
#pragma unroll
            for (int j = 0; j < 8; ++j) sel[s2][j] = (_Float16)(l32 == 16 * s2 + 8 * hh + j ? 1.0f : 0.0f);
        float wrow[16];
#pragma unroll
        for (int r = 0; r < 16; ++r) wrow[r] = __shfl(wgt, crow32(r, hh), 64);
#pragma unroll
        for (int p = 0; p < F16_CS / 2; ++p) {
            f32x16 dd = mfma32h(cf[2 * p], sel[0], zero16());
            dd = mfma32h(cf[2 * p + 1], sel[1], dd);
            float acc = 0.f;
#pragma unroll
            for (int r = 0; r < 16; ++r) acc += wrow[r] * dd[r];
            acc += __shfl_xor(acc, 32, 64);
            const int nn = l32, f = 16 * (nn >> 4) + 8 * ((nn & 7) >> 2) + 4 * ((nn >> 3) & 1) + (nn & 3);
            if (hh == 0 && f < a.dk && p < a.h) a.out[(long)sq * a.d + p * a.dk + f] = acc;
        }
    }
}

template <bool TRAIN>
__device__ __forceinline__ void fwd16p_closed(const Fwd16Args& a, char* smem, int first_slot, int n_e) {
    const int tid = threadIdx.x, lane = tid & 63;
    const int wave = __builtin_amdgcn_readfirstlane(tid >> 6);
    const int l32 = lane & 31, hh = lane >> 5;
    constexpr int DP = F16_DP;
    const int sl = first_slot + wave;
    const bool valid = sl < n_e;
    const int sq = valid ? a.order[(long)a.n_seq + sl] : 0;
    const long t0 = (long)sq * a.S;
    const bool tok = valid && l32 < a.S;

    const int first_tile = 3 * a.h;
    auto tile_at = [&](int step) { return first_tile + step; };
    using Ring = TileRingDMA<F16_FWD_SLOTS>;
    constexpr int AH = Ring::AHEAD;
    Ring ring;
    ring.smem = smem; ring.src = a.wtiles; ring.n_tiles = F16_QT; ring.wave = wave; ring.lane = lane; ring.l32 = l32; ring.hh = hh;
#pragma unroll
    for (int i = 0; i < AH; ++i) ring.load_at(i, tile_at(i));
    float* addv = reinterpret_cast<float*>(smem + F16_FWD_SLOTS * F16_SLOT_DMA);
    for (int i = tid; i < 2 * F16_QP; i += F16_THREADS) addv[i] = i < F16_QP ? a.badd32[i] : a.qv32[i - F16_QP];

    h8 cf[F16_CS];
#pragma unroll
    for (int head = 0; head < F16_CS / 2; ++head) {
#pragma unroll
        for (int c = 0; c < 2; ++c) {
            h8 fr = {0, 0, 0, 0, 0, 0, 0, 0};
            if (head < a.h && tok) {
                const float* bv = a.bqkv32 + (3 * head + 2) * 32 + 16 * c + 4 * hh;
                const f32x4 b0 = *reinterpret_cast<const f32x4*>(bv), b1 = *reinterpret_cast<const f32x4*>(bv + 8);
                float sc[8];
#pragma unroll
                for (int e = 0; e < 8; ++e) sc[e] = 1.0f;
                if (a.drop.thresh != 0u) {
                    const uint64_t e0 = (uint64_t)(t0 + l32) * (uint64_t)DP + (uint64_t)(head * 32 + 16 * c + 8 * hh);
                    dropout_scale8(a.drop.seed, 1u, e0 >> 3, a.drop.thresh16, a.drop.inv_keep, sc);
                }
#pragma unroll
                for (int e = 0; e < 8; ++e) fr[e] = closed_ctx16(e < 4 ? b0[e & 3] : b1[e & 3], sc[e]);
            }
            cf[2 * head + c] = fr;
        }
    }
    __builtin_amdgcn_s_waitcnt(0x0F70);
    __asm__ volatile("s_waitcnt lgkmcnt(0)\n\ts_barrier" ::: "memory");
    int n = 0;
    fwd16p_additive_pool<TRAIN>(a, ring, n, F16_QT, tile_at, addv, cf, valid, tok, sq, t0, l32, hh);
    if (valid) {
        _Float16* dst = a.ctx16 + frag_off((long)sq, F16_CS, 0, l32, hh);
#pragma unroll
        for (int s = 0; s < F16_CS; ++s) *reinterpret_cast<h8*>(dst + 512 * s) = cf[s];
    }
}

template <bool TRAIN>
__global__ __launch_bounds__(F16_THREADS, F16_FWD_WGS) void fused_fwd16p_kernel(Fwd16Args a) {
    extern __shared__ __attribute__((aligned(16))) char smem[];
    const int tid = threadIdx.x, lane = tid & 63;
    const int wave = __builtin_amdgcn_readfirstlane(tid >> 6);
    const int l32 = lane & 31, hh = lane >> 5;
    const int S = a.S;
    constexpr int KP = F16_KP, DP = F16_DP;
    const int n_head_tiles = 3 * a.h;
    constexpr float NEG = -3.0e38f;

    const int n_long = a.order_cnt[0], n_e = a.order_cnt[1], n_short = a.order_cnt[2];
    const int g_pair = (n_short + 2 * F16_WAVES - 1) / (2 * F16_WAVES);
    const int g_long = (n_long + F16_WAVES - 1) / F16_WAVES, g_e = (n_e + F16_WAVES - 1) / F16_WAVES;
    const int blk = blockIdx.x;
    if (blk >= g_pair + g_long + g_e) return;
    if (blk >= g_pair + g_long) {
        fwd16p_closed<TRAIN>(a, smem, (blk - g_pair - g_long) * F16_WAVES, n_e);
        return;
    }
    const bool pair = blk < g_pair;
    const int NT = pair ? 2 : 1;
    int seq[2] = {0, 0};
    bool val[2] = {false, false};
    if (pair) {
        const int p0 = 2 * (blk * F16_WAVES + wave);
#pragma unroll
        for (int i = 0; i < 2; ++i) { val[i] = p0 + i < n_short; seq[i] = val[i] ? a.order[2 * (long)a.n_seq + p0 + i] : 0; }
    } else {
        const int sl = (blk - g_pair) * F16_WAVES + wave;
        val[0] = sl < n_long; seq[0] = val[0] ? a.order[sl] : 0;
    }
    long tok0[2];
    int nlive[2];
#pragma unroll
    for (int i = 0; i < 2; ++i) {
        tok0[i] = (long)seq[i] * S;
        nlive[i] = 0;
        if (pair && val[i]) nlive[i] = __popcll(__ballot(lane < S && a.ids[tok0[i] + lane] != 0));
    }

    const int myp = pair ? (l32 >> 4) : 0, myr = pair ? (l32 & 15) : l32;
    const int myn = myp ? nlive[1] : nlive[0];
    const bool myval = myp ? val[1] : val[0];
    long xrow = -1;
    if (myval) {
        const long t0 = myp ? tok0[1] : tok0[0];
        if (pair) {
            if (myr < myn) xrow = a.pos[t0 + myr];
            else if (myr == myn && myn < S) xrow = *a.n_rows;
        } else if (myr < S) {
            xrow = a.pos[t0 + myr];
            if (xrow < 0) xrow = *a.n_rows;
        }
    }
    f32x16 kbias;
#pragma unroll
    for (int r = 0; r < 16; ++r) {
        const int j = crow32(r, hh);
        float bsv;
        if (pair) {
            const int jr = j & 15;
            const float lm = __logf((float)max(S - myn, 1));
            bsv = (j >> 4) != myp ? NEG : (jr < myn ? 0.f : ((jr == myn && myn < S) ? lm : NEG));
        } else {
            bsv = j < S ? 0.f : NEG;
        }
        kbias[r] = bsv;
    }
    int src_lane[2];
#pragma unroll
    for (int i = 0; i < 2; ++i) src_lane[i] = 4 * (16 * i + min(l32, nlive[i]) + 32 * hh);
    bool tok_ok[2];
#pragma unroll
    for (int i = 0; i < 2; ++i) tok_ok[i] = val[i] && l32 < S;

    const int n_steps = n_head_tiles + F16_QT * NT;
    auto tile_at = [&](int step) { return step < n_head_tiles ? step : n_head_tiles + (step - n_head_tiles) % F16_QT; };
    using Ring = TileRingDMA<F16_FWD_SLOTS>;
    constexpr int AH = Ring::AHEAD;
    Ring ring;
    ring.smem = smem; ring.src = a.wtiles; ring.n_tiles = n_steps; ring.wave = wave; ring.lane = lane; ring.l32 = l32; ring.hh = hh;
#pragma unroll
    for (int i = 0; i < AH; ++i) ring.load_at(i, tile_at(i));
    float* addv = reinterpret_cast<float*>(smem + F16_FWD_SLOTS * F16_SLOT_DMA);
    for (int i = tid; i < 2 * F16_QP; i += F16_THREADS) addv[i] = i < F16_QP ? a.badd32[i] : a.qv32[i - F16_QP];

    h8 xf[F16_KS];
    {
        const _Float16* xr = a.x16 + (xrow < 0 ? 0 : xrow) * KP + 8 * hh;
#pragma unroll
        for (int s = 0; s < F16_KS; ++s) xf[s] = *reinterpret_cast<const h8*>(xr + 16 * s);
        if (xrow < 0) {
#pragma unroll
            for (int s = 0; s < F16_KS; ++s) xf[s] = h8{0, 0, 0, 0, 0, 0, 0, 0};
        }
    }
    __builtin_amdgcn_s_waitcnt(0x0F70);
    __asm__ volatile("s_waitcnt lgkmcnt(0)\n\ts_barrier" ::: "memory");

    const bool any_live = val[0] || val[1];
    int n = 0;
#pragma unroll 1
    for (int head = 0; head < a.h; ++head) {
        f32x16 ct;
        f32x16 qt = zero16(), kt = zero16(), vv = zero16();
        auto pre = [&](int g) { if (n + AH < n_steps) ring.load_piece_at(n + AH, tile_at(n + AH), g); };
        if (!any_live && n + AH < n_steps) ring.load_at(n + AH, tile_at(n + AH));
        if (any_live) tile_mma<true>(qt, ring, n, xf, pre);
        ring.step_barrier(n);
        ++n;
        if (!any_live && n + AH < n_steps) ring.load_at(n + AH, tile_at(n + AH));
        if (any_live) tile_mma<true>(kt, ring, n, xf, pre);
        ring.step_barrier(n);
        ++n;
        if (!any_live && n + AH < n_steps) ring.load_at(n + AH, tile_at(n + AH));
        if (any_live) tile_mma<false>(vv, ring, n, xf, pre);
        if (any_live) {
            f32x16 st = mfma32h(acc_frag(kt, 0), acc_frag(qt, 0), zero16());
            st = mfma32h(acc_frag(kt, 1), acc_frag(qt, 1), st);
            float m = NEG;
#pragma unroll
            for (int r = 0; r < 16; ++r) { st[r] += kbias[r]; m = fmaxf(m, st[r]); }
            m = fmaxf(m, __shfl_xor(m, 32, 64));
            float sum = 0.f;
#pragma unroll
            for (int r = 0; r < 16; ++r) { st[r] = __expf(st[r] - m); sum += st[r]; }
            sum += __shfl_xor(sum, 32, 64);
            const float inv = 1.0f / sum;
#pragma unroll
            for (int r = 0; r < 16; ++r) st[r] *= inv;
            ct = mfma32h(acc_frag(vv, 0), acc_frag(st, 0), zero16());
            ct = mfma32h(acc_frag(vv, 1), acc_frag(st, 1), ct);
        } else {
            ct = zero16();
        }
#pragma unroll
        for (int i = 0; i < 2; ++i) {
            if (i < NT) {
                f32x16 cx = ct;
                if (pair) {
#pragma unroll
                    for (int r = 0; r < 16; ++r)
                        cx[r] = __int_as_float(__builtin_amdgcn_ds_bpermute(src_lane[i], __float_as_int(ct[r])));
                }
                if (a.drop.thresh != 0u) {
#pragma unroll
                    for (int c = 0; c < 2; ++c) {
                        const uint64_t e0 = (uint64_t)(tok0[i] + l32) * (uint64_t)DP + (uint64_t)(head * 32 + 16 * c + 8 * hh);
                        float sc[8];
                        dropout_scale8(a.drop.seed, 1u, e0 >> 3, a.drop.thresh16, a.drop.inv_keep, sc);
#pragma unroll
                        for (int e = 0; e < 8; ++e) cx[8 * c + e] *= sc[e];
                    }
                }
                if (val[i]) {
                    const h8 z = {0, 0, 0, 0, 0, 0, 0, 0};
                    _Float16* dst = a.ctx16 + frag_off((long)seq[i], F16_CS, 2 * head, l32, hh);
                    *reinterpret_cast<h8*>(dst) = tok_ok[i] ? acc_frag(cx, 0) : z;
                    *reinterpret_cast<h8*>(dst + 512) = tok_ok[i] ? acc_frag(cx, 1) : z;
                }
            }
        }
        ring.step_barrier(n);
        ++n;
    }
#pragma unroll
    for (int i = 0; i < 2; ++i) {
        if (i < NT && val[i]) {
            for (int head = a.h; head < F16_CS / 2; ++head) {
                _Float16* dst = a.ctx16 + frag_off((long)seq[i], F16_CS, 2 * head, l32, hh);
                *reinterpret_cast<h8*>(dst) = h8{0, 0, 0, 0, 0, 0, 0, 0};
                *reinterpret_cast<h8*>(dst + 512) = h8{0, 0, 0, 0, 0, 0, 0, 0};
            }
        }
    }

#pragma unroll 1
    for (int i = 0; i < NT; ++i) {
        const bool valid = i ? val[1] : val[0];
        const bool tok = i ? tok_ok[1] : tok_ok[0];
        const int sq = i ? seq[1] : seq[0];
        const long t0 = i ? tok0[1] : tok0[0];
        __asm__ volatile("s_waitcnt vmcnt(0)" ::: "memory");
        h8 cf[F16_CS];
        {
            const _Float16* src = a.ctx16 + frag_off((long)sq, F16_CS, 0, l32, hh);
#pragma unroll
            for (int s = 0; s < F16_CS; ++s) cf[s] = *reinterpret_cast<const h8*>(src + 512 * s);
        }
        fwd16p_additive_pool<TRAIN>(a, ring, n, n_steps, tile_at, addv, cf, valid, tok, sq, t0, l32, hh);
    }
}

struct Prep16Args {
    int d, h, dk, q, KP, DP, QP;
    const float* w_qkv;
    const float* b_qkv;
    const float* w_add;
    const float* b_add;
    const float* q_vec;
    _Float16* wqkv16;
    float* bqkv32;
    _Float16* wadd16;
    float* badd32;
    float* qv32;
};

__global__ __launch_bounds__(256) void prep16_kernel(Prep16Args a) {
    const float qscale = 1.0f / sqrtf((float)a.dk);
    const long n1 = (long)3 * a.h * 32 * a.KP, n2 = (long)a.QP * a.DP, n3 = (long)3 * a.h * 32, n4 = a.QP;
    const long total = n1 + n2 + n3 + 2 * n4;
    for (long i = (long)blockIdx.x * blockDim.x + threadIdx.x; i < total; i += (long)gridDim.x * blockDim.x) {
        if (i < n1) {
            const int k = (int)(i % a.KP);
            const long r = i / a.KP;
            const int f = (int)(r & 31), tile = (int)(r >> 5), head = tile / 3, which = tile - 3 * head;
            float v = 0.f;
            if (f < a.dk && k < a.d) v = a.w_qkv[((long)which * a.d + head * a.dk + f) * a.d + k] * (which == 0 ? qscale : 1.0f);
            if (f < a.dk && k == a.d) v = a.b_qkv[which * a.d + head * a.dk + f] * (which == 0 ? qscale : 1.0f);
            a.wqkv16[(long)tile * 32 * a.KP + dma_tile_pos(f, k)] = (_Float16)v;
        } else if (i < n1 + n2) {
            const long j = i - n1;
            const int p = (int)(j % a.DP), qq = (int)(j / a.DP);
            const int b16 = p >> 4, t = p & 15, hh = t >> 3, jj = t & 7;
            const int fpad = 16 * b16 + 8 * (jj >> 2) + 4 * hh + (jj & 3);
            const int head = fpad >> 5, f = fpad & 31;
            float v = 0.f;
            if (qq < a.q && f < a.dk) v = a.w_add[(long)qq * a.d + head * a.dk + f];
            a.wadd16[(long)(qq >> 5) * 32 * a.DP + dma_tile_pos(qq & 31, p)] = (_Float16)v;
        } else if (i < n1 + n2 + n3) {
            const long j = i - n1 - n2;
            const int f = (int)(j & 31), tile = (int)(j >> 5), head = tile / 3, which = tile - 3 * head;
            float v = 0.f;
            if (f < a.dk) v = a.b_qkv[which * a.d + head * a.dk + f] * (which == 0 ? qscale : 1.0f);
            a.bqkv32[j] = v;
        } else if (i < n1 + n2 + n3 + n4) {
// ... 122 lines not shown
#pragma unroll
            for (int e = 0; e < 4; ++e) o[e] = (_Float16)v[e];
        }
        *reinterpret_cast<h4*>(x16 + (long)i * 4) = o;
    }
}

bool fused16_supported(int S, int d, int h, int q, const char** why) {
    const int dk = d / h;
    const char* w = nullptr;
    if (S > 64) w = "seq_len <= 64";
    else if (d > F16_KP - 4) w = "d_model <= 316";
    else if (dk > 32) w = "d_k <= 32";
    else if (32 * h > F16_DP) w = "n_heads <= 10";
    else if (q > F16_QP) w = "q_dim <= 224";
    if (why) *why = w;
    return w == nullptr;
}

Fused16Layout fused16_layout(int d, int h, int q) {
    Fused16Layout L;
    L.KP = F16_KP;
    L.DP = F16_DP;
    L.QP = F16_QP;
    size_t off = 0;
    auto take = [&](size_t bytes) { size_t o = off; off = (off + bytes + 255) / 256 * 256; return o; };
    L.wqkv16 = take((size_t)3 * h * 32 * L.KP * 2 + (size_t)L.QP * L.DP * 2);
    L.wadd16 = L.wqkv16 + (size_t)3 * h * 32 * L.KP * 2;
    L.bqkv32 = take((size_t)3 * h * 32 * 4);
    L.badd32 = take((size_t)L.QP * 4);
    L.qv32 = take((size_t)L.QP * 4);
    L.total = off;
    return L;
}

int launch_prep16(int d, int h, int q, const float* w_qkv, const float* b_qkv, const float* w_add, const float* b_add,
                  const float* q_vec, void* planes, hipStream_t stream) {
    const Fused16Layout L = fused16_layout(d, h, q);
    char* base = (char*)planes;
    Prep16Args a{};
    a.d = d; a.h = h; a.dk = d / h; a.q = q; a.KP = L.KP; a.DP = L.DP; a.QP = L.QP;
    a.w_qkv = w_qkv; a.b_qkv = b_qkv; a.w_add = w_add; a.b_add = b_add; a.q_vec = q_vec;
    a.wqkv16 = (_Float16*)(base + L.wqkv16); a.wadd16 = (_Float16*)(base + L.wadd16);
    a.bqkv32 = (float*)(base + L.bqkv32); a.badd32 = (float*)(base + L.badd32); a.qv32 = (float*)(base + L.qv32);
    const long total = (long)3 * h * 32 * L.KP + (long)L.QP * L.DP + 3 * h * 32 + 2 * L.QP;
    TimingScope ts("prep16", stream);
    hipLaunchKernelGGL(prep16_kernel, dim3(cdiv(total, 256)), dim3(256), 0, stream, a);
    return check_launch("prep16");
}

int launch_gather16(long M, int d, int KP, const int64_t* ids, const int* live, const int* n_live, const float* table,
                    const Dropout& drop, void* x16, hipStream_t stream) {
    if (M <= 0) return NRMS_OK;
    if ((M + 1) * (KP / 4) >= (1L << 32)) { set_error("gather16: index overflow"); return NRMS_EINVAL; }
    int blocks = cdiv((M + 1) * (KP / 4), 256);
    if (blocks > 256 * 16) blocks = 256 * 16;
    TimingScope ts("gather_dropout", stream);
    hipLaunchKernelGGL(gather16_kernel, dim3(blocks), dim3(256), 0, stream, (unsigned)(d / 4), (unsigned)(KP / 4), M, ids, live,
                       n_live, table, drop, (_Float16*)x16);
    return check_launch("gather16");
}

int launch_cast16(long M, int d, int KP, const float* x, void* x16, hipStream_t stream) {
    if (M <= 0) return NRMS_OK;
    if (M * (KP / 4) >= (1L << 32)) { set_error("cast16: index overflow"); return NRMS_EINVAL; }
    int blocks = cdiv(M * (KP / 4), 256);
    if (blocks > 256 * 16) blocks = 256 * 16;
    TimingScope ts("cast16", stream);
    hipLaunchKernelGGL(cast16_kernel, dim3(blocks), dim3(256), 0, stream, (unsigned)(d / 4), (unsigned)(KP / 4), M, x, (_Float16*)x16);
    return check_launch("cast16");
}

int launch_fused_fwd16(const Fused16Fwd& f, hipStream_t stream) {
    if (f.n_seq <= 0) return NRMS_OK;
    const Fused16Layout L = fused16_layout(f.d, f.h, f.q);
    const char* base = (const char*)f.planes;
    Fwd16Args a{};
    a.n_seq = f.n_seq; a.S = f.S; a.d = f.d; a.h = f.h; a.dk = f.d / f.h; a.q = f.q;
    a.x16 = (const _Float16*)f.x16; a.pos = f.pos; a.n_rows = f.n_rows; a.ids = f.ids; a.order = f.order; a.order_cnt = f.order_cnt;
    a.wtiles = (const _Float16*)(base + L.wqkv16); a.bqkv32 = (const float*)(base + L.bqkv32);
    a.badd32 = (const float*)(base + L.badd32); a.qv32 = (const float*)(base + L.qv32);
    a.ctx16 = (_Float16*)f.ctx16; a.t16 = (_Float16*)f.t16; a.w = f.w; a.out = f.out; a.drop = f.drop;
    const bool train = f.t16 != nullptr, two = f.S > 32;
    const size_t lds = (size_t)(two ? 3 : F16_FWD_SLOTS) * F16_SLOT_DMA + (size_t)2 * F16_QP * 4;
    a.dbg = 0;
#ifdef NRMS_F16_EXPERIMENTS
    { const char* e = getenv("NRMS_F16_DBG"); a.dbg = e ? atoi(e) : 0; }
#endif
    const bool paired = !two && f.order != nullptr && f.pos != nullptr && f.ids != nullptr;
    if (!paired) { a.order = nullptr; a.order_cnt = nullptr; }
    const void* fn = paired ? (train ? (const void*)fused_fwd16p_kernel<true> : (const void*)fused_fwd16p_kernel<false>)
                   : two ? (train ? (const void*)fused_fwd16_kernel<true, 2> : (const void*)fused_fwd16_kernel<false, 2>)
                         : (train ? (const void*)fused_fwd16_kernel<true, 1> : (const void*)fused_fwd16_kernel<false, 1>);
    const hipError_t e = hipFuncSetAttribute(fn, hipFuncAttributeMaxDynamicSharedMemorySize, (int)lds);
    if (e != hipSuccess) { set_error("fused_fwd16: hipFuncSetAttribute: %s", hipGetErrorString(e)); return NRMS_ELAUNCH; }
    TimingScope ts(two ? "fused64_fwd16" : "fused_fwd16", stream);
    const dim3 grid(cdiv(f.n_seq, F16_WAVES) + (f.order != nullptr ? 3 : 0));
    if (paired) {
        if (train) hipLaunchKernelGGL((fused_fwd16p_kernel<true>), grid, dim3(F16_THREADS), lds, stream, a);
        else hipLaunchKernelGGL((fused_fwd16p_kernel<false>), grid, dim3(F16_THREADS), lds, stream, a);
    } else if (two) {
        if (train) hipLaunchKernelGGL((fused_fwd16_kernel<true, 2>), grid, dim3(F16_THREADS), lds, stream, a);
        else hipLaunchKernelGGL((fused_fwd16_kernel<false, 2>), grid, dim3(F16_THREADS), lds, stream, a);
    } else {
        if (train) hipLaunchKernelGGL((fused_fwd16_kernel<true, 1>), grid, dim3(F16_THREADS), lds, stream, a);
        else hipLaunchKernelGGL((fused_fwd16_kernel<false, 1>), grid, dim3(F16_THREADS), lds, stream, a);
    }
    return check_launch("fused_fwd16");
}

}
```

### pytorch_news_recommender_amd/csrc/fused16_bwd.h

```cpp
#pragma once
#include "fused16.h"

namespace nrms {

constexpr int B16_RED_QKV = 3 * 10 * 32;
constexpr int B16_RED = B16_RED_QKV + 2 * F16_QP;
constexpr int B16_DQ = 96 * 10;

struct Bwd16Args {
    int n_seq, S, d, h, dk, q;
    int n_groups;
    const _Float16* x16;
    const int* pos;
    const int* n_rows;
    const int64_t* ids;
    const int* order;
    const int* order_cnt;
    int n_cls;
    const _Float16* btiles;
    const float* bqkv32;
    const _Float16* qv16;
    const _Float16* ctx16;
    const _Float16* t16;
    const float* w;
    const _Float16* dout16;
    _Float16* dz16;
    _Float16* dctx16;
    _Float16* dqkv16;
    float* red;
    Dropout drop;
    int v1;
    int dbg;
};

__device__ __forceinline__ f32x16 transpose32(const f32x16& x, const h8 (&idf)[2]) {
    f32x16 z = mfma32h(acc_frag(x, 0), idf[0], zero16());
    return mfma32h(acc_frag(x, 1), idf[1], z);
}

__device__ __forceinline__ float regsum(const f32x16& x) {
    float s0 = 0.f, s1 = 0.f, s2 = 0.f, s3 = 0.f;
#pragma unroll
    for (int g = 0; g < 4; ++g) { s0 += x[4 * g]; s1 += x[4 * g + 1]; s2 += x[4 * g + 2]; s3 += x[4 * g + 3]; }
    return (s0 + s1) + (s2 + s3);
}

__device__ __forceinline__ f32x16 transpose_frags(const h8& x0, const h8& x1, const h8 (&idf)[2]) {
    f32x16 z = mfma32h(x0, idf[0], zero16());
    return mfma32h(x1, idf[1], z);
}

constexpr int DX_BM = 256, DX_BK = 64, DX_THREADS = 512;
constexpr int DX_SLABS = B16_DQ / DX_BK;
constexpr int DX_A_BYTES = DX_BM * DX_BK * 2;
constexpr int DX_B_BYTES = DX_BK * F16_KP * 2;
constexpr int DX_SLOT = DX_A_BYTES + DX_B_BYTES;
static_assert(B16_DQ % DX_BK == 0 && F16_KP == 320, "15 slabs of 64; 10 column tiles of 32");
struct Dx16Args {
    int M;
    const int* m_dev;
    const _Float16* a16;
    const _Float16* xtiles;
    int lda, n_slabs;
    float* c;
    int ldc, d;
    const float* sc;
};


size_t bwd16_fused_lds(bool two_blocks);
int launch_bwd16_pool(const Bwd16Args& a, int n_wg, bool two_blocks, hipStream_t stream);
int launch_dx16(const Dx16Args& g, bool out16, hipStream_t stream);
int launch_dout16(long n_seq, int d, int h, int dk, float fixed_scale, float* sc, const float* dout, _Float16* dout16, hipStream_t stream);
int launch_tn16(int geom, const _Float16* A, int lda, int N, const _Float16* B, int ldb, int K, int M, const int* m_dev,
                float* partial, int splits, const int* nmap, const int* kmap, const float* nscale, int ldw, float* dW,
                hipStream_t stream, const char* name, float* dbias = nullptr, const int* blk_list = nullptr, const int* blk_cnt = nullptr,
                int blk_stride = 0);

}
```

### pytorch_news_recommender_amd/csrc/fused16_bwd.hip

```cpp
#include <stdlib.h>

#include "fused16_bwd.h"

namespace nrms {

template <int SB>
__global__ __launch_bounds__(F16_THREADS, SB == 1 ? 8 / F16_WAVES : 1) void fused_bwd16_pool_kernel(Bwd16Args a) {
    extern __shared__ __attribute__((aligned(16))) char smem[];
    float* red = reinterpret_cast<float*>(smem + 3 * F16_SLOT);
    float* stg_t = red + B16_RED;
    float* stg_h = stg_t + F16_WAVES * SB * 2 * F16_QT * 32;
    const int tid = threadIdx.x, lane = tid & 63;
    const int wave = __builtin_amdgcn_readfirstlane(tid >> 6);
    const int l32 = lane & 31, hh = lane >> 5;
    const int S = a.S;
    constexpr int DP = F16_DP, QP = F16_QP;

    for (int i = tid; i < B16_RED; i += F16_THREADS) red[i] = 0.f;

    h8 idf[2], sel[2];
#pragma unroll
    for (int s = 0; s < 2; ++s)
#pragma unroll
        for (int j = 0; j < 8; ++j) {
            idf[s][j] = (_Float16)(l32 == 16 * s + 8 * (j >> 2) + 4 * hh + (j & 3) ? 1.0f : 0.0f);
            sel[s][j] = (_Float16)(l32 == 16 * s + 8 * hh + j ? 1.0f : 0.0f);
        }

    int n_ne = a.n_seq, n_e = 0, n_sh = 0, g_ne = a.n_groups, g_sh = 0;
    if (a.order != nullptr) {
        n_ne = a.order_cnt[0];
        n_e = a.order_cnt[1];
        g_ne = (n_ne + F16_WAVES - 1) / F16_WAVES;
        if (a.n_cls == 3) { n_sh = a.order_cnt[2]; g_sh = (n_sh + F16_WAVES - 1) / F16_WAVES; }
    }
    TileRing ring;
    ring.smem = smem; ring.src = a.btiles; ring.n_tiles = a.h; ring.tid = tid; ring.l32 = l32; ring.hh = hh; ring.dbg = 0;

#pragma unroll 1
    for (int grp = blockIdx.x; grp < a.n_groups; grp += gridDim.x) {
        int slot_id = grp * F16_WAVES + wave;
        bool valid;
        int seq;
        if (grp < g_ne) { valid = slot_id < n_ne; seq = valid ? (a.order != nullptr ? a.order[slot_id] : slot_id) : 0; }
        else if (grp < g_ne + g_sh) {
            slot_id -= g_ne * F16_WAVES;
            valid = slot_id < n_sh;
            seq = valid ? a.order[2 * (long)a.n_seq + slot_id] : 0;
        } else {
            slot_id -= (g_ne + g_sh) * F16_WAVES;
            valid = slot_id < n_e;
            seq = valid ? a.order[a.n_seq + slot_id] : 0;
        }
        const long tok0 = (long)seq * S;
        bool empty = false;
        if (SB == 1 && a.ids != nullptr && valid) {
            const bool is_pad = lane < S ? a.ids[tok0 + lane] == 0 : true;
            empty = __ballot(is_pad) == ~0ull;
        }
        const bool live = valid && !empty;
        int nshort = -1;
        h8 selT[2] = {h8{0, 0, 0, 0, 0, 0, 0, 0}, h8{0, 0, 0, 0, 0, 0, 0, 0}};
        if (SB == 1 && a.n_cls == 3 && live && grp >= g_ne) {
            nshort = __popcll(__ballot(lane < S && a.ids[tok0 + lane] != 0));
#pragma unroll
            for (int s = 0; s < 2; ++s)
#pragma unroll
                for (int j = 0; j < 8; ++j) {
                    const int tok = crow32(8 * s + j, hh);
                    const int src = tok < nshort ? tok : (tok < S ? nshort : -1);
                    selT[s][j] = (_Float16)(src == l32 ? 1.0f : 0.0f);
                }
        }
        ring.load(0);

        bool tok_ok[SB];
        float wgt[SB], dw[SB];
#pragma unroll
        for (int b = 0; b < SB; ++b) {
            tok_ok[b] = valid && 32 * b + l32 < S;
            wgt[b] = tok_ok[b] ? a.w[tok0 + 32 * b + l32] : 0.f;
        }

        float aw = 0.f;
#pragma unroll
        for (int b = 0; b < SB; ++b) {
            f32x16 acc = zero16();
            const _Float16* dsrc = a.dout16 + (long)seq * DP + 8 * hh;
            const _Float16* csrc = a.ctx16 + frag_off((long)seq * SB + b, F16_CS, 0, l32, hh);
#pragma unroll
            for (int g = 0; g < F16_CS / 4; ++g) {
                h8 da[4], cb[4];
#pragma unroll
                for (int i = 0; i < 4; ++i) {
                    da[i] = *reinterpret_cast<const h8*>(dsrc + 16 * (4 * g + i));
                    cb[i] = *reinterpret_cast<const h8*>(csrc + 512 * (4 * g + i));
                }
#pragma unroll
                for (int i = 0; i < 4; ++i) acc = mfma32h(da[i], cb[i], acc);
            }
            dw[b] = acc[0];
            aw += wgt[b] * dw[b];
        }
#pragma unroll
        for (int o = 16; o > 0; o >>= 1) aw += __shfl_xor(aw, o, 64);

        h8 zf[SB][16];
#pragma unroll
        for (int b = 0; b < SB; ++b) {
            const float ds = wgt[b] * (dw[b] - aw);
            const _Float16* tsrc = a.t16 + frag_off((long)seq * SB + b, QP / 16, 0, l32, hh);
#pragma unroll
            for (int s = 0; s < 14; ++s) zf[b][s] = *reinterpret_cast<const h8*>(tsrc + 512 * s);
#pragma unroll
            for (int t = 0; t < F16_QT; ++t) {
                f32x16 accz = zero16(), accu = zero16();
#pragma unroll
                for (int s2 = 0; s2 < 2; ++s2) {
                    const int s = 2 * t + s2;
                    const h8 qf = *reinterpret_cast<const h8*>(a.qv16 + 16 * s + 8 * hh);
                    h8 dz, u;
#pragma unroll
                    for (int j = 0; j < 8; ++j) {
                        const float tv = (float)zf[b][s][j];
                        dz[j] = (_Float16)(ds * (float)qf[j] * (1.0f - tv * tv));
                        u[j] = (_Float16)(ds * tv);
                    }
                    zf[b][s] = dz;
                    if (valid && !F16_DBG(a.dbg, 4)) *reinterpret_cast<h8*>(a.dz16 + frag_off((long)seq * SB + b, QP / 16, s, l32, hh)) = dz;
                    accz = mfma32h(dz, sel[s2], accz);
                    accu = mfma32h(u, sel[s2], accu);
                }
                float cz = valid ? regsum(accz) : 0.f, cu = valid ? regsum(accu) : 0.f;
                cz += __shfl_xor(cz, 32, 64);
                cu += __shfl_xor(cu, 32, 64);
                if (hh == 0) {
                    float* row = stg_t + ((wave * SB + b) * 2 * F16_QT + 2 * t) * 32 + l32;
                    row[0] = cz;
                    row[32] = cu;
                }
            }
            zf[b][14] = h8{0, 0, 0, 0, 0, 0, 0, 0};
            zf[b][15] = h8{0, 0, 0, 0, 0, 0, 0, 0};
        }
        ring.store(0);
        ring.load(1);
        ring.store(1);
        const bool any_closed = __syncthreads_or((!live && valid) ? 1 : 0) != 0;
        for (int i = tid; i < 2 * F16_QT * 32; i += F16_THREADS) {
            float sum = 0.f;
#pragma unroll
            for (int w = 0; w < F16_WAVES; ++w)
#pragma unroll
                for (int b = 0; b < SB; ++b) sum += stg_t[((w * SB + b) * 2 * F16_QT) * 32 + i];
            const int r = i >> 5, c = i & 31;
            red[B16_RED_QKV + (r & 1) * QP + 32 * (r >> 1) + c] += sum;
        }

        int n = 0;
#pragma unroll 1
        for (int head = 0; head < a.h; ++head) {
            ring.load(n + 2);
            const h8 d0 = *reinterpret_cast<const h8*>(a.dout16 + (long)seq * DP + head * 32 + 8 * hh);
            const h8 d1 = *reinterpret_cast<const h8*>(a.dout16 + (long)seq * DP + head * 32 + 16 + 8 * hh);
            float closed = 0.f;
#pragma unroll
            for (int b = 0; b < SB; ++b) {
                f32x16 dct = zero16();
                if (!F16_DBG(a.dbg, 8)) tile_mma<true>(dct, ring, n, zf[b]);
#pragma unroll
                for (int r = 0; r < 8; ++r) {
                    dct[r] += wgt[b] * (float)d0[r];
                    dct[8 + r] += wgt[b] * (float)d1[r];
                }
                if (a.drop.thresh != 0u) {
#pragma unroll
                    for (int c = 0; c < 2; ++c) {
                        const uint64_t e0 = (uint64_t)(tok0 + 32 * b + l32) * (uint64_t)DP + (uint64_t)(head * 32 + 16 * c + 8 * hh);
                        float sc[8];
                        dropout_scale8(a.drop.seed, 1u, e0 >> 3, a.drop.thresh16, a.drop.inv_keep, sc);
#pragma unroll
                        for (int e = 0; e < 8; ++e) dct[8 * c + e] *= sc[e];
                    }
                }
                if (a.v1 && live && nshort >= 0 && l32 >= 16) {
                    _Float16* dcrow = a.dctx16 + frag_off((long)seq * SB + b, F16_CS, 2 * head, l32, hh);
                    *reinterpret_cast<h8*>(dcrow) = h8{0, 0, 0, 0, 0, 0, 0, 0};
                    *reinterpret_cast<h8*>(dcrow + 512) = h8{0, 0, 0, 0, 0, 0, 0, 0};
                }
                if (live && !F16_DBG(a.dbg, 4)) {
                    _Float16* dcrow = a.dctx16 + frag_off((long)seq * SB + b, F16_CS, 2 * head, l32, hh);
                    if (SB == 1 && nshort >= 0) {
                        const f32x16 xt = transpose32(dct, idf);
                        f32x16 dcp = mfma32h(acc_frag(xt, 0), selT[0], zero16());
                        dcp = mfma32h(acc_frag(xt, 1), selT[1], dcp);
                        if (l32 < 16) {
                            *reinterpret_cast<h8*>(dcrow) = acc_frag(dcp, 0);
                            *reinterpret_cast<h8*>(dcrow + 512) = acc_frag(dcp, 1);
                        }
                    } else {
                        *reinterpret_cast<h8*>(dcrow) = acc_frag(dct, 0);
                        *reinterpret_cast<h8*>(dcrow + 512) = acc_frag(dct, 1);
                    }
                }
                if (!live && valid) {
                    closed += regsum(transpose32(dct, idf));
                }
            }
            if (any_closed) {
                closed += __shfl_xor(closed, 32, 64);
                if (hh == 0) stg_h[((head & 1) * F16_WAVES + wave) * 32 + l32] = closed;
            }
            ring.store(n + 2);
            __syncthreads();
            if (any_closed && tid < 32) {
                float sum = 0.f;
#pragma unroll
                for (int w = 0; w < F16_WAVES; ++w) sum += stg_h[((head & 1) * F16_WAVES + w) * 32 + tid];
                red[(3 * head + 2) * 32 + tid] += sum;
            }
            ++n;
        }
        __syncthreads();
    }
    __syncthreads();
    float* out = a.red + (long)blockIdx.x * B16_RED;
    for (int i = tid; i < B16_RED; i += F16_THREADS) out[i] = red[i];
}

template <int SB>
__global__ __launch_bounds__(F16_THREADS, SB == 1 ? 8 / F16_WAVES : 1) void fused_bwd16_attn_kernel(Bwd16Args a) {
    extern __shared__ __attribute__((aligned(16))) char smem[];
    float* red = reinterpret_cast<float*>(smem + 3 * F16_SLOT);
    float* stg = red + B16_RED;
    const int tid = threadIdx.x, lane = tid & 63;
    const int wave = __builtin_amdgcn_readfirstlane(tid >> 6);
    const int l32 = lane & 31, hh = lane >> 5;
    const int S = a.S;
    constexpr int KP = F16_KP;
    constexpr float NEG = -3.0e38f;
    for (int i = tid; i < B16_RED; i += F16_THREADS) red[i] = 0.f;
    h8 idf[2];
#pragma unroll
    for (int s = 0; s < 2; ++s)
#pragma unroll
        for (int j = 0; j < 8; ++j) idf[s][j] = (_Float16)(l32 == 16 * s + 8 * (j >> 2) + 4 * hh + (j & 3) ? 1.0f : 0.0f);
    int n_ne = a.n_seq, g_ne = a.n_groups, n_sh = 0, g_pair = 0;
    if (a.order != nullptr) {
        n_ne = a.order_cnt[0];
        g_ne = (n_ne + F16_WAVES - 1) / F16_WAVES;
        if (SB == 1 && a.n_cls == 3) { n_sh = a.order_cnt[2]; g_pair = (n_sh + 2 * F16_WAVES - 1) / (2 * F16_WAVES); }
    }
    TileRing ring;
    ring.smem = smem; ring.src = a.btiles + (long)a.h * 32 * KP; ring.n_tiles = 3 * a.h; ring.tid = tid; ring.l32 = l32; ring.hh = hh; ring.dbg = 0;
    const h8 z8 = {0, 0, 0, 0, 0, 0, 0, 0};
    __syncthreads();
#pragma unroll 1
    for (int grp = blockIdx.x; grp < g_pair + g_ne; grp += gridDim.x) {
// ... 681 lines not shown
                              int* kmap_x, int* nmap_add, float* nscale_add, int* kmap_ctx) {
    const float inv_scale = sc[1];
    const int i = blockIdx.x * blockDim.x + threadIdx.x;
    if (i < B16_DQ) {
        const int head = i / 96, rem = i - head * 96, which = rem >> 5, p = rem & 31;
        const int s = p >> 4, t = p & 15, hh = t >> 3, jj = t & 7;
        const int f = 16 * s + 8 * (jj >> 2) + 4 * hh + (jj & 3);
        nmap_qkv[i] = (head < h && f < dk) ? which * d + head * dk + f : -1;
        nscale_qkv[i] = inv_scale * (which == 0 ? qscale : 1.0f);
    }
    if (i < F16_KP) kmap_x[i] = i < d ? i : -1;
    if (i < F16_QP) { nmap_add[i] = i < q ? i : -1; nscale_add[i] = inv_scale; }
    if (i < F16_DP) {
        const int b16 = i >> 4, t = i & 15, hh = t >> 3, jj = t & 7;
        const int fpad = 16 * b16 + 8 * (jj >> 2) + 4 * hh + (jj & 3);
        const int head = fpad >> 5, f = fpad & 31;
        kmap_ctx[i] = (head < h && f < dk) ? head * dk + f : -1;
    }
}

static size_t up256(size_t x) { return (x + 255) / 256 * 256; }


Fused16BwdLayout fused16_bwd_layout(long M, int n_seq) {
    Fused16BwdLayout L;
    const long Mp = (long)n_seq * (M > (long)n_seq * 32 ? 64 : 32);
    size_t off = 0;
    auto take = [&](size_t bytes) { size_t o = off; off = up256(off + bytes); return o; };
    L.n_wg = 512;
    L.btiles = take((size_t)40 * 32 * F16_KP * 2);
    L.xtiles = take((size_t)DX_SLABS * DX_B_BYTES);
    L.qv16 = take((size_t)F16_QP * 2);
    L.bqkv32 = take((size_t)30 * 32 * 4);
    L.dout16 = take((size_t)n_seq * F16_DP * 2);
    L.dz16 = take((size_t)Mp * F16_QP * 2);
    L.dctx16 = take((size_t)Mp * F16_DP * 2);
    L.dqkv16 = take((size_t)(M + 32) * B16_DQ * 2);
    L.red = take((size_t)2 * L.n_wg * B16_RED * 4);
    L.maps = take((size_t)(B16_DQ * 2 + F16_KP + F16_QP * 2 + F16_DP) * 4);
    L.scale = take(256);
    L.tn_splits_qkv = 40;
    L.tn_splits_add = 192;
    if (const char* e = getenv("NRMS_TN_SPLITS_QKV")) L.tn_splits_qkv = atoi(e);
    if (const char* e = getenv("NRMS_TN_SPLITS_ADD")) L.tn_splits_add = atoi(e);
    const size_t p1 = (size_t)L.tn_splits_qkv * B16_DQ * F16_KP * 4, p2 = (size_t)L.tn_splits_add * F16_QP * F16_DP * 4;
    L.partial = take(up256(p1) + p2);
    L.total = off;
    return L;
}

int launch_tn16(int geom, const _Float16* A, int lda, int N, const _Float16* B, int ldb, int K, int M, const int* m_dev,
                float* partial, int splits, const int* nmap, const int* kmap, const float* nscale, int ldw, float* dW,
                hipStream_t stream, const char* name, float* dbias, const int* blk_list, const int* blk_cnt, int blk_stride) {
    Tn16Args t{};
    t.M = M; t.m_dev = m_dev; t.A = A; t.lda = lda; t.N = N; t.B = B; t.ldb = ldb; t.K = K; t.partial = partial;
    t.blk_list = geom != 0 ? blk_list : nullptr; t.blk_cnt = blk_cnt; t.blk_stride = blk_stride;
    typedef void (*Kern)(Tn16Args);
    const Kern fn = geom == 1 ? (Kern)gemm16_tn_kernel<true, 2, 7, 4, 5> : geom == 2 ? (Kern)gemm16_tn_kernel<true, 4, 5, 2, 5>
                                                                                     : (Kern)gemm16_tn_kernel<false, 4, 5, 2, 5>;
    const int aw = geom == 1 ? Tn16Add::AW : Tn16Qkv::AW, bw = geom == 1 ? Tn16Add::BW : Tn16Qkv::BW;
    t.splits = splits; t.n_blk = cdiv(N, aw); t.k_blk = cdiv(K, bw);
    const size_t lds = 2 * (size_t)(geom == 1 ? Tn16Add::STAGE : Tn16Qkv::STAGE);
    const hipError_t e = hipFuncSetAttribute((const void*)fn, hipFuncAttributeMaxDynamicSharedMemorySize, (int)lds);
    if (e != hipSuccess) { set_error("%s: hipFuncSetAttribute: %s", name, hipGetErrorString(e)); return NRMS_ELAUNCH; }
    {
        TimingScope ts(name, stream);
        hipLaunchKernelGGL(fn, dim3(splits * t.n_blk * t.k_blk), dim3(T16_THREADS), lds, stream, t);
    }
    int rc = check_launch(name);
    if (rc) return rc;
    TimingScope ts("tn_reduce", stream);
    hipLaunchKernelGGL(tn16_reduce_kernel, dim3(cdiv((long)N * K, 256)), dim3(256), 0, stream, partial, splits, N, K, nmap, kmap,
                       nscale, ldw, dW, dbias);
    return check_launch("tn16_reduce");
}

size_t bwd16_fused_lds(bool two) {
    static_assert(F16_WAVES * 2 * F16_QT * 32 + 2 * F16_WAVES * 32 >= 2 * F16_WAVES * 3 * 32, "the attention kernel's staging fits the same size");
    return (size_t)3 * F16_SLOT + (size_t)B16_RED * 4 + (size_t)(F16_WAVES * (two ? 2 : 1) * 2 * F16_QT * 32 + 2 * F16_WAVES * 32) * 4;
}

int launch_bwd16_pool(const Bwd16Args& a, int n_wg, bool two, hipStream_t stream) {
    const size_t lds = bwd16_fused_lds(two);
    const void* fp = two ? (const void*)fused_bwd16_pool_kernel<2> : (const void*)fused_bwd16_pool_kernel<1>;
    const hipError_t e = hipFuncSetAttribute(fp, hipFuncAttributeMaxDynamicSharedMemorySize, (int)lds);
    if (e != hipSuccess) { set_error("fused_bwd16: hipFuncSetAttribute: %s", hipGetErrorString(e)); return NRMS_ELAUNCH; }
    TimingScope ts(two ? "fused64_bwd16_pool" : "fused_bwd16_pool", stream);
    if (two) hipLaunchKernelGGL(fused_bwd16_pool_kernel<2>, dim3(n_wg), dim3(F16_THREADS), lds, stream, a);
    else hipLaunchKernelGGL(fused_bwd16_pool_kernel<1>, dim3(n_wg), dim3(F16_THREADS), lds, stream, a);
    return check_launch("fused_bwd16_pool");
}

int launch_dx16(const Dx16Args& g, bool out16, hipStream_t stream) {
    if ((g.d & 3) != 0 || ((uintptr_t)g.c & 15) != 0) { set_error("gemm16_dx: dx must be 16-byte aligned, d %% 4 == 0"); return NRMS_EINVAL; }
    const size_t lds = (size_t)2 * DX_SLOT;
    const void* fn = out16 ? (const void*)gemm16_dx_kernel<true> : (const void*)gemm16_dx_kernel<false>;
    const hipError_t e = hipFuncSetAttribute(fn, hipFuncAttributeMaxDynamicSharedMemorySize, (int)lds);
    if (e != hipSuccess) { set_error("gemm16_dx: hipFuncSetAttribute: %s", hipGetErrorString(e)); return NRMS_ELAUNCH; }
    TimingScope ts("dx_bwd", stream);
    if (out16) hipLaunchKernelGGL(gemm16_dx_kernel<true>, dim3(cdiv(g.M, DX_BM)), dim3(DX_THREADS), lds, stream, g);
    else hipLaunchKernelGGL(gemm16_dx_kernel<false>, dim3(cdiv(g.M, DX_BM)), dim3(DX_THREADS), lds, stream, g);
    return check_launch("gemm16_dx");
}

int launch_dout16(long n_seq, int d, int h, int dk, float fixed_scale, float* sc, const float* dout, _Float16* dout16, hipStream_t stream) {
    unsigned* max_bits = (unsigned*)(sc + 2);
    if (hipMemsetAsync(max_bits, 0, sizeof(unsigned), stream) != hipSuccess) { set_error("fused_bwd16: memset failed"); return NRMS_ELAUNCH; }
    const long nd = n_seq * d;
    if (!(fixed_scale > 0.f))
        hipLaunchKernelGGL(absmax_kernel, dim3(nd > 512L * 1024 ? 512 : (int)cdiv(nd, 1024)), dim3(256), 0, stream, nd, dout, max_bits);
    hipLaunchKernelGGL(dout16_kernel, dim3(cdiv(n_seq * F16_DP, 256) > 4096 ? 4096 : cdiv(n_seq * F16_DP, 256)),
                       dim3(256), 0, stream, n_seq, d, h, dk, fixed_scale, max_bits, sc, dout, dout16);
    return check_launch("dout16");
}

int launch_fused_bwd16(const Fused16Bwd& f, hipStream_t stream) {
    if (f.n_seq <= 0) return NRMS_OK;
    const long M = (long)f.n_seq * f.S;
    const Fused16BwdLayout L = fused16_bwd_layout(M, f.n_seq);
    char* base = (char*)f.workspace;
    const int dk = f.d / f.h;
    const float qscale = 1.0f / sqrtf((float)dk);
    _Float16* btiles = (_Float16*)(base + L.btiles);
    _Float16* xtiles = (_Float16*)(base + L.xtiles);
    _Float16* qv16 = (_Float16*)(base + L.qv16);
    float* bqkv32 = (float*)(base + L.bqkv32);
    _Float16* dout16 = (_Float16*)(base + L.dout16);
    _Float16* dz16 = (_Float16*)(base + L.dz16);
    _Float16* dctx16 = (_Float16*)(base + L.dctx16);
    _Float16* dqkv16 = (_Float16*)(base + L.dqkv16);
    float* red = (float*)(base + L.red);
    int* nmap_qkv = (int*)(base + L.maps);
    float* nscale_qkv = (float*)(nmap_qkv + B16_DQ);
    int* kmap_x = (int*)(nscale_qkv + B16_DQ);
    int* nmap_add = kmap_x + F16_KP;
    float* nscale_add = (float*)(nmap_add + F16_QP);
    int* kmap_ctx = (int*)(nscale_add + F16_QP);
    float* sc = (float*)(base + L.scale);
    if (f.sc_out != nullptr) *f.sc_out = sc;
    float* partial_qkv = (float*)(base + L.partial);
    float* partial_add = (float*)(base + L.partial + up256((size_t)L.tn_splits_qkv * B16_DQ * F16_KP * 4));
    { const int jr = fused_bwd16_join(stream); if (jr) return jr; }
    SideSet* ss = side_streams_for(stream);
    const bool side = ss != nullptr;
    hipStream_t s_add = side ? ss->s[0] : stream, s_qkv = side ? ss->s[1] : stream;
    SideJoinGuard join_guard(ss, stream);
    const int Mp = f.n_seq * 32 * (f.S > 32 ? 2 : 1);
    {
        Prep16bArgs p{};
        p.d = f.d; p.h = f.h; p.dk = dk; p.q = f.q; p.w_qkv = f.w_qkv; p.b_qkv = f.b_qkv; p.w_add = f.w_add; p.q_vec = f.q_vec;
        p.btiles = btiles; p.xtiles = xtiles; p.qv16 = qv16; p.bqkv32 = bqkv32;
        TimingScope ts("prep16", stream);
        hipLaunchKernelGGL(prep16b_kernel, dim3(2048), dim3(256), 0, stream, p);
        int rc0 = launch_dout16((long)f.n_seq, f.d, f.h, dk, f.loss_scale, sc, f.dout, dout16, stream);
        if (rc0) return rc0;
        hipLaunchKernelGGL(maps16_kernel, dim3(cdiv(B16_DQ, 256)), dim3(256), 0, stream, f.d, f.h, dk, f.q, sc, qscale,
                           nmap_qkv, nscale_qkv, kmap_x, nmap_add, nscale_add, kmap_ctx);
        int rc = check_launch("prep16b");
        if (rc) return rc;
    }
    Bwd16Args a{};
    a.n_seq = f.n_seq; a.S = f.S; a.d = f.d; a.h = f.h; a.dk = dk; a.q = f.q;
    const bool lists = f.order != nullptr && f.S <= 32;
    a.n_groups = cdiv(f.n_seq, F16_WAVES) + (lists ? 2 : 0);
    a.n_cls = lists ? 3 : 2;
    a.x16 = (const _Float16*)f.x16; a.pos = f.pos; a.n_rows = f.n_rows_dev; a.ids = f.ids;
    a.order = lists ? f.order : nullptr; a.order_cnt = lists ? f.order_cnt : nullptr;
    a.btiles = btiles; a.bqkv32 = bqkv32; a.qv16 = qv16;
    a.ctx16 = (const _Float16*)f.ctx16; a.t16 = (const _Float16*)f.t16; a.w = f.w; a.dout16 = dout16;
    a.dz16 = dz16; a.dctx16 = dctx16; a.dqkv16 = dqkv16; a.red = red; a.drop = f.drop;
    a.dbg = 0;
#ifdef NRMS_F16_EXPERIMENTS
    { const char* e = getenv("NRMS_F16_DBG"); a.dbg = e ? atoi(e) : 0; }
#endif
    const int n_wg = a.n_groups < L.n_wg ? a.n_groups : L.n_wg;
    {
        const bool two = f.S > 32;
        const size_t lds = bwd16_fused_lds(two);
        const void* fa = two ? (const void*)fused_bwd16_attn_kernel<2> : (const void*)fused_bwd16_attn_kernel<1>;
        const hipError_t e = hipFuncSetAttribute(fa, hipFuncAttributeMaxDynamicSharedMemorySize, (int)lds);
        if (e != hipSuccess) { set_error("fused_bwd16: hipFuncSetAttribute: %s", hipGetErrorString(e)); return NRMS_ELAUNCH; }
        {
            const int rcp = launch_bwd16_pool(a, n_wg, two, stream);
            if (rcp) return rcp;
        }
        if (side) {
            int rc = side_order(ss, 0, stream, s_add, "fused_bwd16");
            if (rc) return rc;
            rc = launch_tn16(1, dz16, F16_QP, F16_QP, (const _Float16*)f.ctx16, F16_DP, F16_DP, Mp, nullptr, partial_add,
                             L.tn_splits_add, nmap_add, kmap_ctx, nscale_add, f.d, f.dw_add, s_add, "dwadd_bwd");
            if (rc) return rc;
            if (hipEventRecord(ss->ev[2], s_add) != hipSuccess) { set_error("fused_bwd16: hipEventRecord failed"); return NRMS_ELAUNCH; }
        }
        Bwd16Args b = a;
        b.red = red + (long)n_wg * B16_RED;
        {
            TimingScope ts(two ? "fused64_bwd16_attn" : "fused_bwd16_attn", stream);
            if (two) hipLaunchKernelGGL(fused_bwd16_attn_kernel<2>, dim3(n_wg), dim3(F16_THREADS), lds, stream, b);
            else hipLaunchKernelGGL(fused_bwd16_attn_kernel<1>, dim3(n_wg), dim3(F16_THREADS), lds, stream, b);
        }
        int rc = check_launch("fused_bwd16");
        if (rc) return rc;
    }
    {
        TimingScope ts("red16", stream);
        hipLaunchKernelGGL(red16_kernel, dim3(cdiv(B16_RED, 32)), dim3(1024), 0, stream, red, 2 * n_wg, f.h, dk, f.d, f.q, sc,
                           qscale, f.db_qkv, f.db_add, f.dq_vec);
        int rc = check_launch("red16");
        if (rc) return rc;
    }
    int rc = NRMS_OK;
    if (!side) {
        rc = launch_tn16(1, dz16, F16_QP, F16_QP, (const _Float16*)f.ctx16, F16_DP, F16_DP, Mp, nullptr, partial_add,
                         L.tn_splits_add, nmap_add, kmap_ctx, nscale_add, f.d, f.dw_add, stream, "dwadd_bwd");
        if (rc) return rc;
    }
    if (side) {
        rc = side_order(ss, 1, stream, s_qkv, "fused_bwd16");
        if (rc) return rc;
    }
    rc = launch_tn16(0, dqkv16, B16_DQ, B16_DQ, (const _Float16*)f.x16, F16_KP, F16_KP, (int)M, f.n_rows_dev, partial_qkv,
                     L.tn_splits_qkv, nmap_qkv, kmap_x, nscale_qkv, f.d, f.dw_qkv, s_qkv, "dwqkv_bwd");
    if (rc) return rc;
    if (side && hipEventRecord(ss->ev[3], s_qkv) != hipSuccess) { set_error("fused_bwd16: hipEventRecord failed"); return NRMS_ELAUNCH; }
    {
        Dx16Args g{};
        g.M = (int)M; g.m_dev = f.n_rows_dev; g.a16 = dqkv16; g.xtiles = xtiles; g.c = f.dx; g.ldc = f.d; g.d = f.d;
        g.sc = sc; g.lda = B16_DQ; g.n_slabs = DX_SLABS;
        rc = launch_dx16(g, f.dx_fp16, stream);
    }
    if (side && rc == NRMS_OK) {
        if (f.defer_join) ss->pending = true;
        else if (hipStreamWaitEvent(stream, ss->ev[2], 0) != hipSuccess || hipStreamWaitEvent(stream, ss->ev[3], 0) != hipSuccess) {
            set_error("fused_bwd16: hipStreamWaitEvent failed");
            return NRMS_ELAUNCH;
        }
        join_guard.disarm();
    }
    return rc;
}

int fused_bwd16_join(hipStream_t stream) {
    SideSet* ss = side_streams_for(stream);
    if (ss == nullptr || !ss->pending) return NRMS_OK;
    ss->pending = false;
    if (hipStreamWaitEvent(stream, ss->ev[2], 0) != hipSuccess || hipStreamWaitEvent(stream, ss->ev[3], 0) != hipSuccess) {
        set_error("fused_bwd16_join: hipStreamWaitEvent failed");
        return NRMS_ELAUNCH;
    }
    return NRMS_OK;
}

}
// ... 1 lines not shown
```

### pytorch_news_recommender_amd/csrc/gemm.h

```cpp
#pragma once
#include "common.h"
#include "rowdiv.h"

namespace nrms {

constexpr int NT_BM = 128;
constexpr int NT_BK = 16;
constexpr int NT_STAGE_A = NT_BM * NT_BK;

enum { A_PLAIN = 0, A_DZ = 2 };
enum { E_STORE = 0, E_DCTX = 1 };

struct NTArgs {
    int M, N, K;
    int rows_per_tile;
    const float* A; int lda;
    const float* ds;
    const float* qv;
    const float* T;
    const float* W;
    const float* bias;
    float* C; int ldc;
    const float* wrow;
    const float* dout;
// ... 181 lines not shown
                    int sr, c4, rl, n;
                    if (!rem_pos(idx, rbase, sr, c4, rl, n)) continue;
                    const long gr = (long)row0 + rl;
                    f32x4 v = *reinterpret_cast<const f32x4*>(wave_lds + sr * S + 4 * c4);
                    if (!dropped) {
                        f32x4 b4 = {0.f, 0.f, 0.f, 0.f};
                        if (EMODE == E_STORE && g.bias != nullptr) b4 = *reinterpret_cast<const f32x4*>(g.bias + n);
                        v = fix(v, gr, n, b4);
                    }
                    *reinterpret_cast<f32x4*>(g.C + (g.c_rows != nullptr ? (long)g.c_rows[gr] : gr) * g.ldc + n) = v;
                }
            }
            __builtin_amdgcn_fence(__ATOMIC_RELEASE, "wavefront");
            __builtin_amdgcn_wave_barrier();
            __builtin_amdgcn_fence(__ATOMIC_ACQUIRE, "wavefront");
        }
    }
}

int launch_gemm_nt(int amode, int emode, const NTArgs& a, hipStream_t stream, const char* name);

struct TNArgs {
    int M, N, K;
    int amode;
    const float* A; int lda;
    const float* ds;
    const float* qv;
    const float* T;
    const float* B; int ldb;
    float* dW;
    float* dbias;
    float* partial;
    int splits;
    int rows_per_split;
    HeadPerm perm;
    const int* m_dev;
};
size_t gemm_tn_workspace_floats(int M, int N, int K, int* splits_out);
int launch_gemm_tn(const TNArgs& a, hipStream_t stream, const char* name);

int launch_transpose(const float* in, float* out, int rows, int cols, hipStream_t stream, HeadPerm perm = HeadPerm{0, 0});
int launch_permute_rows(const float* w, const float* b, float* w2, float* b2, int rows, int cols, HeadPerm perm,
                        hipStream_t stream);

int launch_gemm_nt_bf16(int amode, int emode, int npass, const NTArgs& a, void* wplanes, hipStream_t stream,
                        const char* name);
size_t gemm_nt_bf16_wplane_bytes(int N, int K);
int launch_gemm_tn_bf16(int npass, const TNArgs& a, hipStream_t stream, const char* name);

struct AddFwdArgs {
    NTArgs g;
    const float* qv;
    float* T;
    float* wout;
    float* out;
    int S, d;
    const uint8_t* mask;
};
int launch_addattn_fwd_bf16(int npass, const AddFwdArgs& a, void* wplanes, hipStream_t stream);
int launch_colsum_add(const float* partial, int rows, int cols, float* out, hipStream_t stream);

struct Fused16Layout { int KP, DP, QP; size_t wqkv16, wadd16, bqkv32, badd32, qv32, total; };
Fused16Layout fused16_layout(int d, int h, int q);
bool fused16_supported(int S, int d, int h, int q, const char** why);
int launch_prep16(int d, int h, int q, const float* w_qkv, const float* b_qkv, const float* w_add, const float* b_add,
                  const float* q_vec, void* planes, hipStream_t stream);
int launch_gather16(long M, int d, int KP, const int64_t* ids, const int* live, const int* n_live, const float* table,
                    const Dropout& drop, void* x16, hipStream_t stream);
int launch_cast16(long M, int d, int KP, const float* x, void* x16, hipStream_t stream);
struct Fused16Fwd {
    int n_seq, S, d, h, q;
    const void* planes;
    const void* x16;
    const int* pos;
    const int* n_rows;
    const int64_t* ids;
    const int* order;
    const int* order_cnt;
    void* ctx16;
    void* t16;
    float* w;
    float* out;
    Dropout drop;
};
int launch_fused_fwd16(const Fused16Fwd& f, hipStream_t stream);
bool fused16v1_supported(int S, int d, int h, int q, const char** why);
size_t fused16v1_planes_bytes(int d, int h, int q);
int launch_prep16v1(int d, int h, int q, const float* w_qkv, const float* b_qkv, const float* w_o, const float* b_o,
                    const float* w_add, const float* b_add, const float* q_vec, void* planes, hipStream_t stream);
int launch_fused_fwd16v1(const Fused16Fwd& f, int h, void* attn16, hipStream_t stream);
size_t title_order_cnt_ints(int n_seq);
int launch_title_order(int n_seq, int S, const int64_t* ids, int* order, int* cnt, hipStream_t stream, int n_classes = 2);

struct Fused16BwdLayout { int n_wg, tn_splits_qkv, tn_splits_add; size_t btiles, xtiles, qv16, bqkv32, dout16, dz16, dctx16, dqkv16, red, maps, scale, partial, total; };
Fused16BwdLayout fused16_bwd_layout(long M, int n_seq);
struct Fused16Bwd {
    int n_seq, S, d, h, q;
    void* workspace;
    const float* w_qkv; const float* b_qkv; const float* w_add; const float* q_vec;
    const void* x16;
    const int* pos;
    const int* n_rows_dev;
    const int64_t* ids;
    const int* order; const int* order_cnt;
    const void* ctx16; const void* t16; const float* w;
    const float* dout;
    float loss_scale;
    Dropout drop;
    float* dw_qkv; float* db_qkv; float* dw_add; float* db_add; float* dq_vec;
    float* dx;
    bool dx_fp16;
    const float** sc_out;
    bool defer_join;
    const float* w_o; const void* attn16; float* dw_o; float* db_o;
};
int launch_fused_bwd16(const Fused16Bwd& f, hipStream_t stream);
size_t fused16v1_bwd_bytes(long M, int n_seq, int h);
int launch_fused_bwd16v1(const Fused16Bwd& f, hipStream_t stream);
int fused_bwd16_join(hipStream_t stream);

bool user64_supported(int S, int d, int h, int q, const char** why);
size_t user64_qkv_bytes(int n_seq, int h);
size_t user64_fwd_planes_bytes(int h);
size_t user64_bwd_planes_bytes(int h);
size_t user64_dq_partial_floats(int n_seq);
int launch_user64_fwd(int n_seq, int S, int d, int h, int q, const float* x, const float* w_qkv, const float* b_qkv,
                      const float* w_add, const float* b_add, const float* q_vec, void* planes, float* ctx, float* t, float* w,
                      void* qkv, float* out, bool train, hipStream_t stream);
int launch_user64_bwd(int n_seq, int S, int d, int h, int q, const float* w_add, const float* q_vec, void* planes, const float* dout,
                      const float* t, const float* w, const void* qkv, float* ds, float* dq_partial, float* dq_vec, float* dqkv,
                      hipStream_t stream);

int launch_sanitize_ids(long n, const void* src, bool src_is_int32, int64_t* dst, int vocab, int* n_bad, hipStream_t stream);
int launch_title_dedup(long n, int L, const int64_t* ids, int* table, long table_size, int* inverse, int* rep_rows,
                       int* n_unique, hipStream_t stream);
int launch_gather_dropout(long M, int d, const int64_t* ids, const float* table, const Dropout& drop, float* x,
                          hipStream_t stream);
int launch_gather_dropout_compact(long M, int d, const int64_t* ids, const int* live, const int* n_live,
                                  const float* table, const Dropout& drop, float* x, hipStream_t stream);
int launch_fill_pad_rows(long n_seq, int S, int n, const int64_t* ids, const float* row, float* out, bool skip_all_pad,
                         hipStream_t stream);
size_t compact_scratch_ints(long M);
int launch_compact_live_rows(long M, const int64_t* ids, int* live, int* pos, int* n_live, int* scratch,
                             hipStream_t stream);
size_t scatter_grouped_scratch_ints(long M, int V);
int launch_scatter_grouped(long M, int V, int d, const int64_t* ids, const int* live, const int* n_live, const void* dx,
                           const Dropout& drop, float* dtable, int* scratch, hipStream_t stream, bool dx_fp16 = false, int ldx = 0,
                           const float* sc = nullptr, bool prepared = false);
int launch_scatter_prepare(long M, int V, const int64_t* ids, const int* live, const int* n_live, int* scratch, hipStream_t stream);
int launch_scatter_dense_rows(long M, int d, const int64_t* ids, const int* live, const int* n_live, const float* dx,
                              const Dropout& drop, float* dtable, hipStream_t stream);
int launch_scatter_dropout_compact(long M, int d, const int64_t* ids, const int* live, const int* n_live, const float* dx,
                                   const Dropout& drop, float* dtable, hipStream_t stream);

}
```

### pytorch_news_recommender_amd/engine.py

```python
from __future__ import annotations

import ctypes as C
import math
from dataclasses import dataclass

import torch

from . import _lib
from .synth import ENCODERS


@dataclass(frozen=True)
class ModelDims:
    n_words: int
    word_embed_size: int
    num_attention_heads: int
    query_vector_dim: int
    news_heads: int = 0
    output_proj: bool = False
    style: str = "v0"

    def heads(self, enc):
        return self.news_heads if (enc == "news_encoder" and self.news_heads) else self.num_attention_heads

# ... 137 lines not shown
                and d.word_embed_size // h <= L["d_k"] and d.query_vector_dim <= L["q_dim"]
                and not d.output_proj and not mask_mode and (not training or self.fp16_backward))

    def set_precision(self, precision):
        if precision not in _lib.PRECISIONS:
            raise ValueError("precision must be one of %s" % sorted(_lib.PRECISIONS))
        self.precision = precision
        self.pad_row_zero = False

    def _buf(self, key, numel, dtype=torch.float32):
        t = self._bufs.get(key)
        if t is None or t.numel() < numel or t.dtype != dtype:
            t = torch.empty(max(int(numel), 1), dtype=dtype, device=self.device)
            self._bufs[key] = t
        return t

    def _desc(self, enc, n_seq, seq_len, p_embed=0.0, p_ctx=0.0, seed=0, mask_mode=0, training=False):
        d = self.dims
        prec = self.precision
        if prec == "fp16" and not self._fp16_ok(enc, seq_len, mask_mode, training):
            prec = "bf16x3"
        flags = _lib.NRMS_FLAG_PAD_ROW_ZERO if (self.pad_row_zero and enc == "news_encoder") else 0
        h = d.heads(enc)
        if (enc == "user_encoder" and self.fused_user_encoder and prec == "bf16x3" and not d.output_proj and not mask_mode
                and 32 < seq_len <= 64 and d.word_embed_size <= 300 and d.word_embed_size % h == 0
                and (d.word_embed_size // h) <= 32 and (d.word_embed_size // h) % 2 == 0 and h <= 10 and d.query_vector_dim <= 224):
            flags |= _lib.NRMS_FLAG_FUSED_SEQ64
        return _lib.EncoderDesc(n_seq=n_seq, seq_len=seq_len, d_model=d.word_embed_size, n_heads=h,
                                q_dim=d.query_vector_dim, vocab=d.n_words if enc == "news_encoder" else 0,
                                p_drop_embed=float(p_embed), p_drop_ctx=float(p_ctx),
                                precision=_lib.PRECISIONS[prec], use_output_proj=int(d.output_proj),
                                mask_mode=int(mask_mode),
                                flags=flags,
                                seed=int(seed), loss_scale=float(self.loss_scale), p_drop_attn=0.0)

    def _ptrs(self, cls, flat, enc):
        b = self.layout.blocks[enc]
        base = flat.data_ptr()
        p = lambda role: (base + 4 * b[role]) if role in b else None
        return cls(table=p("table"), w_qkv=p("wq"), b_qkv=p("bq"), w_o=p("wo"), b_o=p("bo"), w_add=p("wa"),
                   b_add=p("ba"), q_vec=p("qv"))

    def _weights(self, flat, enc):
        return self._ptrs(_lib.EncoderWeights, flat, enc)

    def _grads(self, gflat, enc):
        return self._ptrs(_lib.EncoderGrads, gflat, enc)

    def _acts(self, tag, M, need_bwd, gather=False, desc=None):
        d, q = self.dims.word_embed_size, self.dims.query_vector_dim
        if desc is not None and desc.precision == _lib.NRMS_PRECISION_FP16:
            KP, DP, QP = _lib.NRMS_FP16_KP, _lib.NRMS_FP16_DP, _lib.NRMS_FP16_QP
            h = torch.float16
            x = self._buf(tag + ".x16", (M + 1) * KP, h)
            Mp = desc.n_seq * (32 if desc.seq_len <= 32 else 64)
            ctx = self._buf(tag + ".ctx16", Mp * DP, h)
            t = self._buf(tag + ".t16", Mp * QP, h) if need_bwd else None
            w = self._buf(tag + ".w", M) if need_bwd else None
            nbytes = int(self.lib.nrms_encoder_fwd_scratch_bytes(C.byref(desc)))
            scratch = self._buf(tag + ".scratch16", (nbytes + 3) // 4)
            attn = self._buf(tag + ".attn16", Mp * DP, h) if desc.use_output_proj else None
            dp = lambda z: None if z is None else z.data_ptr()
            return _lib.EncoderActs(x=dp(x), qkv=None, attn=dp(attn), ctx=dp(ctx), t=dp(t), w=dp(w), scratch=dp(scratch))
        x = self._buf(tag + ".x", M * d) if gather else None
        if desc is not None and desc.flags & _lib.NRMS_FLAG_FUSED_SEQ64:
            nb = int(self.lib.nrms_encoder_fused_qkv_bytes(C.byref(desc)))
            qkv = self._buf(tag + ".qkvf", (nb + 3) // 4)
            ctx = self._buf(tag + ".ctx", M * d) if need_bwd else None
            t = self._buf(tag + ".t", M * q) if need_bwd else None
            w = self._buf(tag + ".w", M) if need_bwd else None
            ns = int(self.lib.nrms_encoder_fwd_scratch_bytes(C.byref(desc)))
            scratch = self._buf("fwd_scratch64", (ns + 3) // 4)
            dp = lambda z: None if z is None else z.data_ptr()
            return _lib.EncoderActs(x=None, qkv=dp(qkv), attn=None, ctx=dp(ctx), t=dp(t), w=dp(w), scratch=dp(scratch))
        qkv = self._buf(tag + ".qkv", M * 3 * d)
        attn = self._buf(tag + ".attn", M * d) if self.dims.output_proj else None
        ctx = self._buf(tag + ".ctx", M * d)
        t = self._buf(tag + ".t", M * q) if need_bwd else None
        w = self._buf(tag + ".w", M) if need_bwd else None
        scratch = self._buf("fwd_scratch", 3 * d * d + 3 * d + 256 + (3 * d + 32) * (d + 32) + (M + M // 1024 + 512 if gather else 0))
        dp = lambda z: None if z is None else z.data_ptr()
        return _lib.EncoderActs(x=dp(x), qkv=dp(qkv), attn=dp(attn), ctx=dp(ctx), t=dp(t), w=dp(w), scratch=dp(scratch))

    def sanitize_ids(self, src, dst):
        n = src.numel()
        if n == 0:
            return dst
        fn = self.lib.nrms_sanitize_ids_i32 if src.dtype == torch.int32 else self.lib.nrms_sanitize_ids
        rc = fn(_lib.ptr(src), _lib.ptr(dst), C.c_int64(n), int(self.dims.n_words), _lib.ptr(self._bad_ids), _stream())
        _lib.check(rc, "nrms_sanitize_ids")
        self._bad_host.copy_(self._bad_ids, non_blocking=True)
        ev = torch.cuda.Event()
        ev.record()
        self._bad_event = ev
        return dst

    def note_bad_ids(self):
        self._bad_host.copy_(self._bad_ids, non_blocking=True)
        ev = torch.cuda.Event()
        ev.record()
        self._bad_event = ev

    def _raise_bad_ids(self):
        n = int(self._bad_host.item())
        if n:
            self._bad_ids.zero_()
            self._bad_host.zero_()
            raise _lib.NrmsError("%d word id(s) outside [0, %d) reached the embedding gather (treated as the padding "
                                 "id on the device; the vocabulary and the embedding table disagree)" % (n, self.dims.n_words))

    def poll_ids(self):
        if self._bad_event is not None and self._bad_event.query():
            self._bad_event = None
            self._raise_bad_ids()

    def check_ids(self):
        if self._bad_event is not None:
            self._bad_event.synchronize()
            self._bad_event = None
        self._raise_bad_ids()

    def encode_titles(self, flat, ids, out=None, p_embed=0.0, p_ctx=0.0, seed=0, save=False, tag=None,
                      chunk_titles=32768, mask=None, mask_mode=0, trusted_ids=False):
        N, L = ids.shape
        d = self.dims.word_embed_size
        if tag is None:
            tag = "news" if save else "news_eval"
        if out is None:
            out = torch.empty(N, d, dtype=torch.float32, device=self.device)
        if trusted_ids:
            ids = ids.contiguous()
        else:
            self.poll_ids()
            ids = self.sanitize_ids(ids.contiguous(), self._buf(tag + ".ids", N * L, torch.int64)[:N * L].view(N, L))
        if mask is not None:
            mask = mask.contiguous()
        w = self._weights(flat, "news_encoder")
        step = N if save else min(N, chunk_titles)
        for s0 in range(0, N, max(step, 1)):
            n = min(step, N - s0)
            desc = self._desc("news_encoder", n, L, p_embed, p_ctx, seed, mask_mode if mask is not None else 0, training=save)
            acts = self._acts(tag, n * L, save, gather=True, desc=desc)
            mp = None if mask is None else C.c_void_p(mask[s0:].data_ptr())
            rc = self.lib.nrms_encoder_fwd(C.byref(desc), C.byref(w), C.c_void_p(ids[s0:].data_ptr()), None, mp,
                                           C.byref(acts), C.c_void_p(out[s0:].data_ptr()), _stream())
            _lib.check(rc, "nrms_encoder_fwd(news)")
        return out

    def encode_users(self, flat, news_vectors, out=None, save=False, tag=None, mask=None, mask_mode=0):
        B, H, d = news_vectors.shape
        if tag is None:
            tag = "user" if save else "user_eval"
        if out is None:
            out = torch.empty(B, d, dtype=torch.float32, device=self.device)
        w = self._weights(flat, "user_encoder")
        desc = self._desc("user_encoder", B, H, mask_mode=mask_mode if mask is not None else 0, training=save)
        acts = self._acts(tag, B * H, save, desc=desc)
        rc = self.lib.nrms_encoder_fwd(C.byref(desc), C.byref(w), None, C.c_void_p(news_vectors.data_ptr()),
                                       _lib.ptr(None if mask is None else mask.contiguous()), C.byref(acts),
                                       C.c_void_p(out.data_ptr()), _stream())
        _lib.check(rc, "nrms_encoder_fwd(user)")
        return out

    def click_scores(self, cand_vec, user_vec, cand_mask=None, out=None):
        B, Cn, d = cand_vec.shape
        if out is None:
            out = torch.empty(B, Cn, dtype=torch.float32, device=self.device)
        rc = self.lib.nrms_click_score_fwd(B, Cn, d, _lib.ptr(cand_vec), _lib.ptr(user_vec), _lib.ptr(cand_mask),
                                           _lib.ptr(out), _stream())
        _lib.check(rc, "nrms_click_score_fwd")
        return out

    def forward(self, flat, hist_ids, cand_ids, cand_mask, training, p_drop=0.0, seed=0, user_mask=None,
                user_mask_mode=0):
        B, H, L = hist_ids.shape
        Cn = cand_ids.shape[1]
        d = self.dims.word_embed_size
        N = B * (H + Cn)
        sfx = "" if training else "_eval"
        self.poll_ids()
        ids = self._buf("ids" + sfx, N * L, torch.int64)[:N * L].view(N, L)
        self.sanitize_ids(hist_ids.reshape(B * H, L).contiguous(), ids[:B * H])
        self.sanitize_ids(cand_ids.reshape(B * Cn, L).contiguous(), ids[B * H:])
        nv = self._buf("news_vec" + sfx, N * d)[:N * d].view(N, d)
        p = float(p_drop)
        p_embed = 0.0 if self.dims.style == "v1" else p
        self.encode_titles(flat, ids, out=nv, p_embed=p_embed, p_ctx=p, seed=seed, save=training, tag="news" + sfx,
                           trusted_ids=True)
        hist = nv[:B * H].view(B, H, d)
        cand = nv[B * H:].view(B, Cn, d)
        user = self._buf("user_vec" + sfx, B * d)[:B * d].view(B, d)
        self.encode_users(flat, hist, out=user, save=training, tag="user" + sfx, mask=user_mask, mask_mode=user_mask_mode)
        if cand_mask is not None:
            cand_mask = cand_mask.contiguous()
        scores = torch.empty(B, Cn, dtype=torch.float32, device=self.device)
        self.click_scores(cand, user, cand_mask, out=scores)
        if training:
            self._gen += 1
            self._saved = dict(B=B, H=H, C=Cn, L=L, ids=ids, nv=nv, user=user, mask=cand_mask, p=p, p_embed=p_embed,
                               seed=seed, user_mask=user_mask, user_mask_mode=user_mask_mode if user_mask is not None else 0,
                               gen=self._gen)
        return scores

    def ce_loss(self, scores, grad_scale=None, want_grad=True):
        B, Cn = scores.shape
        loss_sum = torch.zeros(1, dtype=torch.float32, device=self.device)
        dscores = torch.empty_like(scores) if want_grad else None
        gs = (1.0 / B) if grad_scale is None else grad_scale
        rc = self.lib.nrms_ce_loss_fwd_bwd(B, Cn, _lib.ptr(scores), _lib.ptr(loss_sum), _lib.ptr(dscores),
                                           C.c_float(gs), _stream())
        _lib.check(rc, "nrms_ce_loss_fwd_bwd")
        return loss_sum, dscores

    def _bwd_workspace(self, *descs):
        nbytes = max(self.lib.nrms_encoder_bwd_workspace_bytes(C.byref(d)) for d in descs)
        return self._buf("bwd_ws", (nbytes + 3) // 4)

    def encode_users_backward(self, flat, gflat, news_vectors, dout, dx=None, tag="user", mask=None, mask_mode=0):
        B, H, d = news_vectors.shape
        if dx is None:
            dx = torch.empty(B * H, d, dtype=torch.float32, device=self.device)
        desc = self._desc("user_encoder", B, H, mask_mode=mask_mode if mask is not None else 0, training=True)
        ws = self._bwd_workspace(desc)
        w, g = self._weights(flat, "user_encoder"), self._grads(gflat, "user_encoder")
        acts = self._acts(tag, B * H, True, desc=desc)
        rc = self.lib.nrms_encoder_bwd(C.byref(desc), C.byref(w), None, _lib.ptr(news_vectors),
                                       _lib.ptr(None if mask is None else mask.contiguous()), C.byref(acts),
                                       _lib.ptr(dout.contiguous()), C.byref(g), _lib.ptr(dx), _lib.ptr(ws),
                                       C.c_size_t(ws.numel() * 4), _stream())
        _lib.check(rc, "nrms_encoder_bwd(user)")
        return dx[:B * H].view(B, H, d)

    def backward(self, flat, gflat, dscores, table_grad_ready=None, gen=None):
        sv = self._saved
        if sv is None:
            raise _lib.NrmsError("backward() without a training forward()")
        if gen is not None and gen != sv["gen"]:
            raise _lib.NrmsError("backward() for training forward #%d, but the saved activations belong to forward #%d: "
                                 "a later training forward replaced them (one forward/backward pair at a time)" % (gen, sv["gen"]))
        B, H, Cn, L = sv["B"], sv["H"], sv["C"], sv["L"]
        d = self.dims.word_embed_size
        N = B * (H + Cn)
        self.poll_grad_overflow()
        self.loss_scale = float(getattr(self, "loss_scale_override", None) or -float(self.loss_scale_backoff))
        nv, user = sv["nv"], sv["user"]
        hist = nv[:B * H]
        cand = nv[B * H:]
        dnv = self._buf("d_news_vec", N * d)[:N * d].view(N, d)
        duser = self._buf("d_user_vec", B * d)[:B * d].view(B, d)
        dscores = dscores.contiguous()
        rc = self.lib.nrms_click_score_bwd(B, Cn, d, _lib.ptr(cand), _lib.ptr(user), _lib.ptr(sv["mask"]),
                                           _lib.ptr(dscores), C.c_void_p(dnv[B * H:].data_ptr()), _lib.ptr(duser),
                                           _stream())
        _lib.check(rc, "nrms_click_score_bwd")
        desc_u = self._desc("user_encoder", B, H, mask_mode=sv["user_mask_mode"], training=True)
        desc_n = self._desc("news_encoder", N, L, sv["p_embed"], sv["p"], sv["seed"], training=True)
        ws = self._bwd_workspace(desc_u, desc_n)
        self.encode_users_backward(flat, gflat, hist.view(B, H, d), duser, dx=dnv, tag="user", mask=sv["user_mask"],
                                   mask_mode=sv["user_mask_mode"])
        wn, gn = self._weights(flat, "news_encoder"), self._grads(gflat, "news_encoder")
        acts_n = self._acts("news", N * L, True, gather=True, desc=desc_n)
        if desc_n.precision == _lib.NRMS_PRECISION_FP16:
            desc_n.flags |= _lib.NRMS_FLAG_FWD_SCRATCH_KEPT
        if table_grad_ready is not None:
            desc_n.flags |= _lib.NRMS_FLAG_DEFER_WQKV
        rc = self.lib.nrms_encoder_bwd(C.byref(desc_n), C.byref(wn), _lib.ptr(sv["ids"]), None, None, C.byref(acts_n),
                                       _lib.ptr(dnv), C.byref(gn), None, _lib.ptr(ws),
                                       C.c_size_t(ws.numel() * 4), _stream())
        _lib.check(rc, "nrms_encoder_bwd(news)")
        if table_grad_ready is not None:
            table_grad_ready()
            rc = self.lib.nrms_encoder_bwd_wqkv(C.byref(desc_n), _lib.ptr(sv["ids"]), None, C.byref(acts_n), C.byref(gn),
                                                _lib.ptr(ws), C.c_size_t(ws.numel() * 4), _stream())
            _lib.check(rc, "nrms_encoder_bwd_wqkv(news)")

    def adam_step(self, flat, gflat, exp_avg, exp_avg_sq, step, lr=1e-3, betas=(0.9, 0.999), eps=1e-8,
                  grad_scale=1.0, guard=None):
        if guard is None:
            guard = self.precision == "fp16"
        if guard:
            rc = self.lib.nrms_adam_step_guarded(C.c_size_t(flat.numel()), _lib.ptr(flat), _lib.ptr(gflat), _lib.ptr(exp_avg),
                                                 _lib.ptr(exp_avg_sq), C.c_double(lr), C.c_double(betas[0]), C.c_double(betas[1]),
                                                 C.c_double(eps), int(step), C.c_float(grad_scale), _lib.ptr(self._grad_bad), _stream())
            _lib.check(rc, "nrms_adam_step_guarded")
            return
        rc = self.lib.nrms_adam_step(C.c_size_t(flat.numel()), _lib.ptr(flat), _lib.ptr(gflat), _lib.ptr(exp_avg),
                                     _lib.ptr(exp_avg_sq), C.c_double(lr), C.c_double(betas[0]), C.c_double(betas[1]),
                                     C.c_double(eps), int(step), C.c_float(grad_scale), _stream())
        _lib.check(rc, "nrms_adam_step")

    def grad_guard(self, gflat):
        rc = self.lib.nrms_grad_guard(C.c_size_t(gflat.numel()), _lib.ptr(gflat), _lib.ptr(self._grad_bad), _stream())
        _lib.check(rc, "nrms_grad_guard")

    def note_grad_check(self):
        if self._grad_bad_event is not None and not self._grad_bad_event.query():
            return
        self._grad_bad_host.copy_(self._grad_bad, non_blocking=True)
        ev = torch.cuda.Event()
        ev.record()
        self._grad_bad_event = ev

    def poll_grad_overflow(self, block=False):
        ev = self._grad_bad_event
        if ev is None:
            return self.loss_scale_backoff
        if block:
            ev.synchronize()
        elif not ev.query():
            return self.loss_scale_backoff
        self._grad_bad_event = None
        n = int(self._grad_bad_host.item())
        if n:
            self._grad_bad.zero_()
            self._grad_bad_host.zero_()
            self.grad_overflow_steps += 1
            self._clean_polls = 0
            if self.loss_scale_backoff < 24:
                self.loss_scale_backoff = min(24, self.loss_scale_backoff + 2)
            import warnings
            warnings.warn("NRMS fp16 backward: %d non-finite gradient element(s) were skipped by the optimizer (an fp16 overflow of "
                          "the loss-scaled gradient tensors, or an inf / nan loss); loss-scale head room raised to 2^%d below the "
                          "default" % (n, self.loss_scale_backoff), RuntimeWarning, stacklevel=2)
        else:
            self._clean_polls += 1
            if self._clean_polls >= 2000 and self.loss_scale_backoff > 0:
                self.loss_scale_backoff -= 1
                self._clean_polls = 0
        return self.loss_scale_backoff

    def impression_auc(self, scores, labels, lens):
        n, cmax = scores.shape
        auc = torch.empty(n, dtype=torch.float64, device=self.device)
        rc = self.lib.nrms_impression_auc(n, cmax, _lib.ptr(scores.contiguous()), _lib.ptr(labels.contiguous()),
                                          _lib.ptr(lens.contiguous()), _lib.ptr(auc), _stream())
        _lib.check(rc, "nrms_impression_auc")
        return auc

    def impression_metrics(self, scores, labels, lens, ks=(5, 10), ranks=False):
        return impression_metrics(self.lib, self.device, scores, labels, lens, ks, ranks)

    def top_k(self, user_vec, items, k, exclude=None):
        k = int(k)
        dev = self.device if self.device.index is not None else torch.device("cuda", torch.cuda.current_device())
        for name, t, dt in (("user_vec", user_vec, torch.float32), ("items", items, torch.float32)):
            if t.dim() != 2 or t.dtype != dt or t.device != dev or not t.is_contiguous():
                raise _lib.NrmsError("top_k: %s must be a contiguous 2-D %s tensor on %s (got %s %s on %s%s)"
                                     % (name, dt, self.device, tuple(t.shape), t.dtype, t.device,
                                        "" if t.is_contiguous() else ", not contiguous"))
        B, d = user_vec.shape
        N = items.shape[0]
# ... 261 lines not shown
```

Baseline: 170,400 users/s.

## Save context-dropout keep bits in forward and reuse them in backward

The fp16 news-encoder forward now packs the per-element context dropout keep mask into 16-bit words per lane and head, and writes them to a small buffer. The backward pool kernel gains a KEEP specialization that reads these bits instead of regenerating Philox random numbers. This removes the RNG recomputation from the backward pass for 32-token sequences. The cost is extra global writes and reads of the mask, a small buffer, and one more kernel template instantiation.

```diff
diff --git a/include/nrms_hip.h b/include/nrms_hip.h
--- a/include/nrms_hip.h
+++ b/include/nrms_hip.h
@@ -82,6 +82,16 @@
 int nrms_encoder_fwd(const nrms_encoder_desc* desc, const nrms_encoder_weights* w,
                      const int64_t* ids, const float* x, const uint8_t* mask ,
                      const nrms_encoder_acts* acts, float* out, void* stream);
+
+size_t nrms_encoder_keep_bits_bytes(const nrms_encoder_desc* desc);
+int nrms_encoder_fwd_keep(const nrms_encoder_desc* desc, const nrms_encoder_weights* w,
+                          const int64_t* ids, const float* x, const uint8_t* mask,
+                          const nrms_encoder_acts* acts, void* keep, float* out, void* stream);
+int nrms_encoder_bwd_keep(const nrms_encoder_desc* desc, const nrms_encoder_weights* w,
+                          const int64_t* ids, const float* x, const uint8_t* mask,
+                          const nrms_encoder_acts* acts, const void* keep, const float* dout,
+                          const nrms_encoder_grads* grads, float* dx,
+                          void* workspace, size_t workspace_bytes, void* stream);
 
 size_t nrms_encoder_bwd_workspace_bytes(const nrms_encoder_desc* desc);
 int nrms_encoder_bwd(const nrms_encoder_desc* desc, const nrms_encoder_weights* w,
diff --git a/pytorch_news_recommender_amd/_lib.py b/pytorch_news_recommender_amd/_lib.py
--- a/pytorch_news_recommender_amd/_lib.py
+++ b/pytorch_news_recommender_amd/_lib.py
@@ -78,6 +78,12 @@
     "nrms_encoder_bwd_workspace_bytes": (C.c_size_t, [C.POINTER(EncoderDesc)]),
     "nrms_encoder_fwd_scratch_bytes": (C.c_size_t, [C.POINTER(EncoderDesc)]),
     "nrms_encoder_fused_qkv_bytes": (C.c_size_t, [C.POINTER(EncoderDesc)]),
+    "nrms_encoder_keep_bits_bytes": (C.c_size_t, [C.POINTER(EncoderDesc)]),
+    "nrms_encoder_fwd_keep": (C.c_int, [C.POINTER(EncoderDesc), C.POINTER(EncoderWeights), C.c_void_p, C.c_void_p,
+                                        C.c_void_p, C.POINTER(EncoderActs), C.c_void_p, C.c_void_p, C.c_void_p]),
+    "nrms_encoder_bwd_keep": (C.c_int, [C.POINTER(EncoderDesc), C.POINTER(EncoderWeights), C.c_void_p, C.c_void_p,
+                                        C.c_void_p, C.POINTER(EncoderActs), C.c_void_p, C.c_void_p, C.POINTER(EncoderGrads),
+                                        C.c_void_p, C.c_void_p, C.c_size_t, C.c_void_p]),
     "nrms_encoder_bwd": (C.c_int, [C.POINTER(EncoderDesc), C.POINTER(EncoderWeights), C.c_void_p, C.c_void_p,
                                    C.c_void_p, C.POINTER(EncoderActs), C.c_void_p, C.POINTER(EncoderGrads), C.c_void_p,
                                    C.c_void_p, C.c_size_t, C.c_void_p]),
diff --git a/pytorch_news_recommender_amd/csrc/capi.hip b/pytorch_news_recommender_amd/csrc/capi.hip
--- a/pytorch_news_recommender_amd/csrc/capi.hip
+++ b/pytorch_news_recommender_amd/csrc/capi.hip
@@ -271,7 +271,7 @@
 }
 
 static int encoder_fwd16(const nrms_encoder_desc* desc, const nrms_encoder_weights* w, const int64_t* ids, const float* x,
-                         const nrms_encoder_acts* acts, float* out, hipStream_t s) {
+                         const nrms_encoder_acts* acts, void* keep, float* out, hipStream_t s) {
     const bool gather = desc->vocab > 0;
     NRMS_REQUIRE(acts->x && acts->ctx && acts->scratch, "encoder_fwd(fp16): acts.x, acts.ctx and acts.scratch are required");
     const int S = desc->seq_len, d = desc->d_model, h = desc->n_heads, q = desc->q_dim;
@@ -306,6 +306,7 @@
     f.n_seq = desc->n_seq; f.S = S; f.d = d; f.h = h; f.q = q;
     f.planes = base + fs.planes; f.x16 = acts->x; f.ctx16 = acts->ctx; f.t16 = acts->t; f.w = acts->w; f.out = out;
     f.drop = make_dropout(desc->seed, desc->p_drop_ctx);
+    f.keep = v1 ? nullptr : keep;
     if (gather) {
         const Dropout drop_e = make_dropout(desc->seed, desc->p_drop_embed);
         if (skip_pad_rows(desc)) {
@@ -359,7 +360,7 @@
 }
 
 static int encoder_bwd16(const nrms_encoder_desc* desc, const nrms_encoder_weights* w, const int64_t* ids, const float* x,
-                         const nrms_encoder_acts* acts, const float* dout, const nrms_encoder_grads* grads, float* dx,
+                         const nrms_encoder_acts* acts, const void* keep, const float* dout, const nrms_encoder_grads* grads, float* dx,
                          void* workspace, size_t workspace_bytes, hipStream_t s) {
     NRMS_REQUIRE(w && acts && dout && grads && workspace, "encoder_bwd(fp16): null argument");
     const bool v1 = desc->use_output_proj != 0;
@@ -384,6 +385,7 @@
     f.x16 = acts->x; f.ctx16 = acts->ctx; f.t16 = acts->t; f.w = acts->w; f.dout = dout;
     f.loss_scale = desc->loss_scale;
     f.drop = make_dropout(desc->seed, desc->p_drop_ctx);
+    f.keep = v1 ? nullptr : keep;
     f.dw_qkv = grads->w_qkv; f.db_qkv = grads->b_qkv; f.dw_add = grads->w_add; f.db_add = grads->b_add; f.dq_vec = grads->q_vec;
     if (v1) { f.w_o = w->w_o; f.attn16 = acts->attn; f.dw_o = grads->w_o; f.db_o = grads->b_o; }
     int rc;
@@ -454,9 +456,9 @@
     return rc;
 }
 
-extern "C" int nrms_encoder_fwd(const nrms_encoder_desc* desc, const nrms_encoder_weights* w, const int64_t* ids,
-                                const float* x, const uint8_t* mask, const nrms_encoder_acts* acts, float* out,
-                                void* stream) {
+static int encoder_fwd_any(const nrms_encoder_desc* desc, const nrms_encoder_weights* w, const int64_t* ids,
+                           const float* x, const uint8_t* mask, const nrms_encoder_acts* acts, void* keep, float* out,
+                           void* stream) {
     int rc = validate_desc(desc, "encoder_fwd");
     if (rc) return rc;
     if (acts != nullptr) kept_forget(acts->scratch);
@@ -465,7 +467,7 @@
         NRMS_REQUIRE(w->w_qkv && w->b_qkv && w->w_add && w->b_add && w->q_vec, "encoder_fwd: null weight");
         NRMS_REQUIRE(desc->vocab > 0 ? (ids != nullptr && w->table != nullptr) : (x != nullptr), "encoder_fwd: input missing");
         if (desc->n_seq == 0) return NRMS_OK;
-        return encoder_fwd16(desc, w, ids, x, acts, out, (hipStream_t)stream);
+        return encoder_fwd16(desc, w, ids, x, acts, keep, out, (hipStream_t)stream);
     }
     NRMS_REQUIRE(w && acts && out, "encoder_fwd: null argument");
     NRMS_REQUIRE(w->w_qkv && w->b_qkv && w->w_add && w->b_add && w->q_vec, "encoder_fwd: null weight");
@@ -560,6 +562,17 @@
                               pmask, npass, wplanes, s);
 }
 
+extern "C" int nrms_encoder_fwd(const nrms_encoder_desc* desc, const nrms_encoder_weights* w, const int64_t* ids,
+                                const float* x, const uint8_t* mask, const nrms_encoder_acts* acts, float* out,
+                                void* stream) {
+    return encoder_fwd_any(desc, w, ids, x, mask, acts, nullptr, out, stream);
+}
+extern "C" int nrms_encoder_fwd_keep(const nrms_encoder_desc* desc, const nrms_encoder_weights* w, const int64_t* ids,
+                                     const float* x, const uint8_t* mask, const nrms_encoder_acts* acts, void* keep, float* out,
+                                     void* stream) {
+    return encoder_fwd_any(desc, w, ids, x, mask, acts, keep, out, stream);
+}
+
 extern "C" size_t nrms_encoder_fwd_scratch_bytes(const nrms_encoder_desc* desc) {
     if (validate_desc(desc, "encoder_fwd_scratch_bytes")) return 0;
     if (desc->precision == NRMS_PRECISION_FP16) return fwd16_scratch(desc).total;
@@ -569,6 +582,12 @@
 extern "C" size_t nrms_encoder_fused_qkv_bytes(const nrms_encoder_desc* desc) {
     if (desc == nullptr || !(desc->flags & NRMS_FLAG_FUSED_SEQ64) || validate_desc(desc, "encoder_fused_qkv_bytes")) return 0;
     return user64_qkv_bytes(desc->n_seq, desc->n_heads);
+}
+
+extern "C" size_t nrms_encoder_keep_bits_bytes(const nrms_encoder_desc* desc) {
+    if (desc == nullptr || desc->precision != NRMS_PRECISION_FP16 || validate_desc(desc, "encoder_keep_bits_bytes")) return 0;
+    const size_t blocks = (size_t)desc->n_seq * (desc->seq_len <= 32 ? 1 : 2);
+    return blocks * (size_t)desc->n_heads * 64 * sizeof(uint16_t);
 }
 
 extern "C" size_t nrms_encoder_bwd_workspace_bytes(const nrms_encoder_desc* desc) {
@@ -653,14 +672,28 @@
                     (float*)(base + L.tn_partial), (hipStream_t)stream);
 }
 
+static int encoder_bwd_any(const nrms_encoder_desc* desc, const nrms_encoder_weights* w, const int64_t* ids, const float* x,
+                           const uint8_t* mask, const nrms_encoder_acts* acts, const void* keep, const float* dout,
+                           const nrms_encoder_grads* grads, float* dx, void* workspace, size_t workspace_bytes, void* stream);
 extern "C" int nrms_encoder_bwd(const nrms_encoder_desc* desc, const nrms_encoder_weights* w, const int64_t* ids,
                                 const float* x, const uint8_t* mask, const nrms_encoder_acts* acts, const float* dout,
                                 const nrms_encoder_grads* grads, float* dx, void* workspace, size_t workspace_bytes,
                                 void* stream) {
+    return encoder_bwd_any(desc, w, ids, x, mask, acts, nullptr, dout, grads, dx, workspace, workspace_bytes, stream);
+}
+extern "C" int nrms_encoder_bwd_keep(const nrms_encoder_desc* desc, const nrms_encoder_weights* w, const int64_t* ids,
+                                     const float* x, const uint8_t* mask, const nrms_encoder_acts* acts, const void* keep,
+                                     const float* dout, const nrms_encoder_grads* grads, float* dx, void* workspace,
+                                     size_t workspace_bytes, void* stream) {
+    return encoder_bwd_any(desc, w, ids, x, mask, acts, keep, dout, grads, dx, workspace, workspace_bytes, stream);
+}
+static int encoder_bwd_any(const nrms_encoder_desc* desc, const nrms_encoder_weights* w, const int64_t* ids, const float* x,
+                           const uint8_t* mask, const nrms_encoder_acts* acts, const void* keep, const float* dout,
+                           const nrms_encoder_grads* grads, float* dx, void* workspace, size_t workspace_bytes, void* stream) {
     int rc = validate_desc(desc, "encoder_bwd");
     if (rc) return rc;
     if (desc->precision == NRMS_PRECISION_FP16)
-        return encoder_bwd16(desc, w, ids, x, acts, dout, grads, dx, workspace, workspace_bytes, (hipStream_t)stream);
+        return encoder_bwd16(desc, w, ids, x, acts, keep, dout, grads, dx, workspace, workspace_bytes, (hipStream_t)stream);
     NRMS_REQUIRE(w && acts && dout && grads && workspace, "encoder_bwd: null argument");
     NRMS_REQUIRE(acts->qkv && acts->ctx && acts->t && acts->w, "encoder_bwd: all saved activations are required");
     NRMS_REQUIRE(grads->w_qkv && grads->b_qkv && grads->w_add && grads->b_add && grads->q_vec,
diff --git a/pytorch_news_recommender_amd/csrc/common.h b/pytorch_news_recommender_amd/csrc/common.h
--- a/pytorch_news_recommender_amd/csrc/common.h
+++ b/pytorch_news_recommender_amd/csrc/common.h
@@ -80,6 +80,23 @@
         s[2 * w] = (r[w] & 0xFFFFu) >= thresh16 ? inv_keep : 0.f;
         s[2 * w + 1] = (r[w] >> 16) >= thresh16 ? inv_keep : 0.f;
     }
+}
+__device__ __forceinline__ uint32_t dropout_scale8_bits(uint64_t seed, uint32_t site, uint64_t group8, uint32_t thresh16, float inv_keep,
+                                                        float (&s)[8]) {
+    uint32_t r[4];
+    philox4x32_7(seed, group8, site, r);
+    uint32_t bits = 0u;
+#pragma unroll
+    for (int w = 0; w < 4; ++w) {
+        const bool k0 = (r[w] & 0xFFFFu) >= thresh16, k1 = (r[w] >> 16) >= thresh16;
+        s[2 * w] = k0 ? inv_keep : 0.f;
+        s[2 * w + 1] = k1 ? inv_keep : 0.f;
+        bits |= (k0 ? 1u : 0u) << (2 * w) | (k1 ? 1u : 0u) << (2 * w + 1);
+    }
+    return bits;
+}
+__device__ __forceinline__ float keep_bit_scale(uint32_t bits, int k, float inv_keep) {
+    return __uint_as_float((uint32_t)(-(int32_t)((bits >> k) & 1u)) & __float_as_uint(inv_keep));
 }
 __device__ __forceinline__ float dropout_scale1(uint64_t seed, uint32_t site, uint64_t elem,
                                                 uint32_t thresh, float inv_keep) {
diff --git a/pytorch_news_recommender_amd/csrc/fused16.hip b/pytorch_news_recommender_amd/csrc/fused16.hip
--- a/pytorch_news_recommender_amd/csrc/fused16.hip
+++ b/pytorch_news_recommender_amd/csrc/fused16.hip
@@ -21,6 +21,7 @@
     float* w;
     float* out;
     Dropout drop;
+    uint16_t* keep;
     int dbg;
 };
 
@@ -167,14 +168,17 @@
 #pragma unroll
         for (int b = 0; b < SB; ++b) {
             if (a.drop.thresh != 0u) {
+                uint32_t kb = 0u;
 #pragma unroll
                 for (int c = 0; c < 2; ++c) {
                     const uint64_t e0 = (uint64_t)(tok0 + 32 * b + l32) * (uint64_t)DP + (uint64_t)(head * 32 + 16 * c + 8 * hh);
                     float sc[8];
-                    dropout_scale8(a.drop.seed, 1u, e0 >> 3, a.drop.thresh16, a.drop.inv_keep, sc);
+                    if (TRAIN && SB == 1) kb |= dropout_scale8_bits(a.drop.seed, 1u, e0 >> 3, a.drop.thresh16, a.drop.inv_keep, sc) << (8 * c);
+                    else dropout_scale8(a.drop.seed, 1u, e0 >> 3, a.drop.thresh16, a.drop.inv_keep, sc);
 #pragma unroll
                     for (int e = 0; e < 8; ++e) ct[b][8 * c + e] *= sc[e];
                 }
+                if (TRAIN && SB == 1 && a.keep != nullptr && valid) a.keep[((long)seq * a.h + head) * 64 + lane] = (uint16_t)kb;
             }
             if (valid && !F16_DBG(a.dbg, 8)) {
                 const h8 z = {0, 0, 0, 0, 0, 0, 0, 0};
@@ -382,6 +386,9 @@
     for (int i = tid; i < 2 * F16_QP; i += F16_THREADS) addv[i] = i < F16_QP ? a.badd32[i] : a.qv32[i - F16_QP];
 
     h8 cf[F16_CS];
+    uint32_t kbits[F16_CS / 4];
+#pragma unroll
+    for (int i = 0; i < F16_CS / 4; ++i) kbits[i] = 0u;
 #pragma unroll
     for (int head = 0; head < F16_CS / 2; ++head) {
 #pragma unroll
@@ -395,7 +402,9 @@
                 for (int e = 0; e < 8; ++e) sc[e] = 1.0f;
                 if (a.drop.thresh != 0u) {
                     const uint64_t e0 = (uint64_t)(t0 + l32) * (uint64_t)DP + (uint64_t)(head * 32 + 16 * c + 8 * hh);
-                    dropout_scale8(a.drop.seed, 1u, e0 >> 3, a.drop.thresh16, a.drop.inv_keep, sc);
+                    if (TRAIN) kbits[head >> 1] |= dropout_scale8_bits(a.drop.seed, 1u, e0 >> 3, a.drop.thresh16, a.drop.inv_keep, sc)
+                                                   << (16 * (head & 1) + 8 * c);
+                    else dropout_scale8(a.drop.seed, 1u, e0 >> 3, a.drop.thresh16, a.drop.inv_keep, sc);
                 }
 #pragma unroll
                 for (int e = 0; e < 8; ++e) fr[e] = closed_ctx16(e < 4 ? b0[e & 3] : b1[e & 3], sc[e]);
@@ -411,6 +420,11 @@
         _Float16* dst = a.ctx16 + frag_off((long)sq, F16_CS, 0, l32, hh);
 #pragma unroll
         for (int s = 0; s < F16_CS; ++s) *reinterpret_cast<h8*>(dst + 512 * s) = cf[s];
+        if (TRAIN && a.keep != nullptr && a.drop.thresh != 0u) {
+#pragma unroll
+            for (int head = 0; head < F16_CS / 2; ++head)
+                if (head < a.h) a.keep[((long)sq * a.h + head) * 64 + lane] = (uint16_t)(kbits[head >> 1] >> (16 * (head & 1)));
+        }
     }
 }
 
@@ -560,14 +574,17 @@
                         cx[r] = __int_as_float(__builtin_amdgcn_ds_bpermute(src_lane[i], __float_as_int(ct[r])));
                 }
                 if (a.drop.thresh != 0u) {
+                    uint32_t kb = 0u;
 #pragma unroll
                     for (int c = 0; c < 2; ++c) {
                         const uint64_t e0 = (uint64_t)(tok0[i] + l32) * (uint64_t)DP + (uint64_t)(head * 32 + 16 * c + 8 * hh);
                         float sc[8];
-                        dropout_scale8(a.drop.seed, 1u, e0 >> 3, a.drop.thresh16, a.drop.inv_keep, sc);
+                        if (TRAIN) kb |= dropout_scale8_bits(a.drop.seed, 1u, e0 >> 3, a.drop.thresh16, a.drop.inv_keep, sc) << (8 * c);
+                        else dropout_scale8(a.drop.seed, 1u, e0 >> 3, a.drop.thresh16, a.drop.inv_keep, sc);
 #pragma unroll
                         for (int e = 0; e < 8; ++e) cx[8 * c + e] *= sc[e];
                     }
+                    if (TRAIN && a.keep != nullptr && val[i]) a.keep[((long)seq[i] * a.h + head) * 64 + lane] = (uint16_t)kb;
                 }
                 if (val[i]) {
                     const h8 z = {0, 0, 0, 0, 0, 0, 0, 0};
@@ -856,6 +873,7 @@
     a.badd32 = (const float*)(base + L.badd32); a.qv32 = (const float*)(base + L.qv32);
     a.ctx16 = (_Float16*)f.ctx16; a.t16 = (_Float16*)f.t16; a.w = f.w; a.out = f.out; a.drop = f.drop;
     const bool train = f.t16 != nullptr, two = f.S > 32;
+    a.keep = (train && !two && f.drop.thresh != 0u) ? (uint16_t*)f.keep : nullptr;
     const size_t lds = (size_t)(two ? 3 : F16_FWD_SLOTS) * F16_SLOT_DMA + (size_t)2 * F16_QP * 4;
     a.dbg = 0;
 #ifdef NRMS_F16_EXPERIMENTS
diff --git a/pytorch_news_recommender_amd/csrc/fused16_bwd.h b/pytorch_news_recommender_amd/csrc/fused16_bwd.h
--- a/pytorch_news_recommender_amd/csrc/fused16_bwd.h
+++ b/pytorch_news_recommender_amd/csrc/fused16_bwd.h
@@ -29,6 +29,7 @@
     _Float16* dqkv16;
     float* red;
     Dropout drop;
+    const uint16_t* keep;
     int v1;
     int dbg;
 };
diff --git a/pytorch_news_recommender_amd/csrc/fused16_bwd.hip b/pytorch_news_recommender_amd/csrc/fused16_bwd.hip
--- a/pytorch_news_recommender_amd/csrc/fused16_bwd.hip
+++ b/pytorch_news_recommender_amd/csrc/fused16_bwd.hip
@@ -4,8 +4,9 @@
 
 namespace nrms {
 
-template <int SB>
+template <int SB, bool KEEP = false>
 __global__ __launch_bounds__(F16_THREADS, SB == 1 ? 8 / F16_WAVES : 1) void fused_bwd16_pool_kernel(Bwd16Args a) {
+    static_assert(!KEEP || SB == 1, "keep bits: 32-row kernels only");
     extern __shared__ __attribute__((aligned(16))) char smem[];
     float* red = reinterpret_cast<float*>(smem + 3 * F16_SLOT);
     float* stg_t = red + B16_RED;
@@ -163,6 +164,8 @@
             ring.load(n + 2);
             const h8 d0 = *reinterpret_cast<const h8*>(a.dout16 + (long)seq * DP + head * 32 + 8 * hh);
             const h8 d1 = *reinterpret_cast<const h8*>(a.dout16 + (long)seq * DP + head * 32 + 16 + 8 * hh);
+            uint32_t kw = 0u;
+            if (KEEP) kw = a.keep[((long)seq * a.h + head) * 64 + lane];
             float closed = 0.f;
 #pragma unroll
             for (int b = 0; b < SB; ++b) {
@@ -173,7 +176,10 @@
                     dct[r] += wgt[b] * (float)d0[r];
                     dct[8 + r] += wgt[b] * (float)d1[r];
                 }
-                if (a.drop.thresh != 0u) {
+                if (KEEP) {
+#pragma unroll
+                    for (int e = 0; e < 16; ++e) dct[e] *= keep_bit_scale(kw, e, a.drop.inv_keep);
+                } else if (a.drop.thresh != 0u) {
 #pragma unroll
                     for (int c = 0; c < 2; ++c) {
                         const uint64_t e0 = (uint64_t)(tok0 + 32 * b + l32) * (uint64_t)DP + (uint64_t)(head * 32 + 16 * c + 8 * hh);
@@ -1021,11 +1027,13 @@
 
 int launch_bwd16_pool(const Bwd16Args& a, int n_wg, bool two, hipStream_t stream) {
     const size_t lds = bwd16_fused_lds(two);
-    const void* fp = two ? (const void*)fused_bwd16_pool_kernel<2> : (const void*)fused_bwd16_pool_kernel<1>;
+    const bool keep = !two && a.keep != nullptr;
+    const void* fp = two ? (const void*)fused_bwd16_pool_kernel<2> : keep ? (const void*)fused_bwd16_pool_kernel<1, true> : (const void*)fused_bwd16_pool_kernel<1>;
     const hipError_t e = hipFuncSetAttribute(fp, hipFuncAttributeMaxDynamicSharedMemorySize, (int)lds);
     if (e != hipSuccess) { set_error("fused_bwd16: hipFuncSetAttribute: %s", hipGetErrorString(e)); return NRMS_ELAUNCH; }
     TimingScope ts(two ? "fused64_bwd16_pool" : "fused_bwd16_pool", stream);
     if (two) hipLaunchKernelGGL(fused_bwd16_pool_kernel<2>, dim3(n_wg), dim3(F16_THREADS), lds, stream, a);
+    else if (keep) hipLaunchKernelGGL((fused_bwd16_pool_kernel<1, true>), dim3(n_wg), dim3(F16_THREADS), lds, stream, a);
     else hipLaunchKernelGGL(fused_bwd16_pool_kernel<1>, dim3(n_wg), dim3(F16_THREADS), lds, stream, a);
     return check_launch("fused_bwd16_pool");
 }
@@ -1108,6 +1116,7 @@
     a.btiles = btiles; a.bqkv32 = bqkv32; a.qv16 = qv16;
     a.ctx16 = (const _Float16*)f.ctx16; a.t16 = (const _Float16*)f.t16; a.w = f.w; a.dout16 = dout16;
     a.dz16 = dz16; a.dctx16 = dctx16; a.dqkv16 = dqkv16; a.red = red; a.drop = f.drop;
+    a.keep = (f.S <= 32 && f.drop.thresh != 0u) ? (const uint16_t*)f.keep : nullptr;
     a.dbg = 0;
 #ifdef NRMS_F16_EXPERIMENTS
     { const char* e = getenv("NRMS_F16_DBG"); a.dbg = e ? atoi(e) : 0; }
diff --git a/pytorch_news_recommender_amd/csrc/gemm.h b/pytorch_news_recommender_amd/csrc/gemm.h
--- a/pytorch_news_recommender_amd/csrc/gemm.h
+++ b/pytorch_news_recommender_amd/csrc/gemm.h
@@ -287,6 +287,7 @@
     float* w;
     float* out;
     Dropout drop;
+    void* keep;
 };
 int launch_fused_fwd16(const Fused16Fwd& f, hipStream_t stream);
 bool fused16v1_supported(int S, int d, int h, int q, const char** why);
@@ -312,6 +313,7 @@
     const float* dout;
     float loss_scale;
     Dropout drop;
+    const void* keep;
     float* dw_qkv; float* db_qkv; float* dw_add; float* db_add; float* dq_vec;
     float* dx;
     bool dx_fp16;
diff --git a/pytorch_news_recommender_amd/engine.py b/pytorch_news_recommender_amd/engine.py
--- a/pytorch_news_recommender_amd/engine.py
+++ b/pytorch_news_recommender_amd/engine.py
@@ -243,6 +243,12 @@
         dp = lambda z: None if z is None else z.data_ptr()
         return _lib.EncoderActs(x=dp(x), qkv=dp(qkv), attn=dp(attn), ctx=dp(ctx), t=dp(t), w=dp(w), scratch=dp(scratch))
 
+    def _keep_bits(self, tag, desc):
+        if desc.precision != _lib.NRMS_PRECISION_FP16:
+            return None
+        kb = int(self.lib.nrms_encoder_keep_bits_bytes(C.byref(desc)))
+        return C.c_void_p(self._buf(tag + ".keep16", (kb + 3) // 4).data_ptr()) if kb else None
+
     def sanitize_ids(self, src, dst):
         n = src.numel()
         if n == 0:
@@ -303,8 +309,9 @@
             desc = self._desc("news_encoder", n, L, p_embed, p_ctx, seed, mask_mode if mask is not None else 0, training=save)
             acts = self._acts(tag, n * L, save, gather=True, desc=desc)
             mp = None if mask is None else C.c_void_p(mask[s0:].data_ptr())
-            rc = self.lib.nrms_encoder_fwd(C.byref(desc), C.byref(w), C.c_void_p(ids[s0:].data_ptr()), None, mp,
-                                           C.byref(acts), C.c_void_p(out[s0:].data_ptr()), _stream())
+            keep = self._keep_bits(tag, desc) if save else None
+            rc = self.lib.nrms_encoder_fwd_keep(C.byref(desc), C.byref(w), C.c_void_p(ids[s0:].data_ptr()), None, mp,
+                                                C.byref(acts), keep, C.c_void_p(out[s0:].data_ptr()), _stream())
             _lib.check(rc, "nrms_encoder_fwd(news)")
         return out
 
@@ -425,9 +432,9 @@
             desc_n.flags |= _lib.NRMS_FLAG_FWD_SCRATCH_KEPT
         if table_grad_ready is not None:
             desc_n.flags |= _lib.NRMS_FLAG_DEFER_WQKV
-        rc = self.lib.nrms_encoder_bwd(C.byref(desc_n), C.byref(wn), _lib.ptr(sv["ids"]), None, None, C.byref(acts_n),
-                                       _lib.ptr(dnv), C.byref(gn), None, _lib.ptr(ws),
-                                       C.c_size_t(ws.numel() * 4), _stream())
+        rc = self.lib.nrms_encoder_bwd_keep(C.byref(desc_n), C.byref(wn), _lib.ptr(sv["ids"]), None, None, C.byref(acts_n),
+                                            self._keep_bits("news", desc_n), _lib.ptr(dnv), C.byref(gn), None, _lib.ptr(ws),
+                                            C.c_size_t(ws.numel() * 4), _stream())
         _lib.check(rc, "nrms_encoder_bwd(news)")
         if table_grad_ready is not None:
             table_grad_ready()
```

New measurement: 170,200 users/s. Within noise of the previous version (-0.1%).
